# DecodeGenetics/Ratatosk

Measured on AMD Instinct MI355X. Metric: corrected long-read bases/sec, higher is better.
Workload: dtype u64

## Files before the change

### include/ratatosk_hip.h

```cpp
#ifndef RATATOSK_HIP_H
#define RATATOSK_HIP_H

#include <stdint.h>

#ifdef __cplusplus
extern "C" {
#endif

#define RTK_OK 0
#define RTK_ERR_IO (-1)
#define RTK_ERR_FORMAT (-2)
#define RTK_ERR_ARG (-3)
#define RTK_ERR_NO_DEVICE (-4)
#define RTK_ERR_DEVICE (-5)
#define RTK_ERR_UNSUPPORTED (-6)

typedef struct rtk_graph rtk_graph;
typedef struct rtk_batch rtk_batch;

typedef struct rtk_opts {
    uint64_t insert_sz;
    uint64_t min_cov_vertices;
    uint64_t max_len_weak_region1;
    uint64_t max_km_cov;
    double weak_region_len_factor;
    double large_k_factor;
    double min_score;
    int32_t max_qual;
    int32_t out_qual;
    double min_confidence_snp_corr;
    int32_t long_read_correct;
    int32_t force_unres_snp_corr;
    uint64_t max_len_weak_region2;
    int32_t a2_exclusive;
    int32_t a3_strand_order;
    int32_t d1_desc;
    uint32_t struct_size;
} rtk_opts;

typedef struct rtk_graph_info {
    uint64_t n_unitigs, n_kmers, n_bases, n_colour_ids, n_global_sets;
    uint64_t table_slots, hbm_bytes;
    uint64_t max_km_cov_top;
    int32_t k, device;
} rtk_graph_info;

typedef struct rtk_stats {
    double ms_total, ms_lookup_exact, ms_mask, ms_lookup_inexact, ms_seeds, ms_regions, ms_correct, ms_stitch;
    uint64_t n_windows, n_probes_exact, n_probes_inexact, n_hits_inexact, n_regions, n_region_items, n_arena_overflow;
    uint64_t n_expand, n_colour_elem, n_path_base, n_align, n_align_cells;
    uint64_t in_bases, out_bases;
    uint64_t cyc_colour, cyc_paths, cyc_consensus, cyc_total, cyc_myers, cyc_sets , cyc_tostring, cyc_pathqual;
    uint64_t n_slots_exact, n_slots_inexact;
    uint64_t cyc_walk, n_moves;
    double ms_lanes;
    uint64_t n_lane_regions, n_lane_handed;
    double ms_phase;
    uint64_t n_phase_skipped;
    uint64_t n_trim_stored, n_trim_column, n_trim_fallback, n_consensus_resumed, n_consensus_swept;
    uint64_t n_fa_linked_run, n_fa_linked_skipped, n_fa_linked_entries;
    uint64_t n_strand2_run, n_strand2_skipped, n_strand2_audit_mismatch;
    uint64_t n_park_walked, n_park_deferred;
    uint64_t n_colours_small, n_colours_wide, n_colours_bits, n_colours_general, n_colours_audit_mismatch;
    uint64_t n_colours_declined_fit;
} rtk_stats;

int rtk_graph_load(const char* unitig_fasta_gz, const char* rtsk, int k, int n_threads, rtk_graph** out);
#define RTK_LOAD_DEVICE_TABLES 1u
int rtk_graph_load2(const char* unitig_fasta_gz, const char* rtsk, int k, int n_threads, uint32_t flags, rtk_graph** out);

int rtk_graph_upload(rtk_graph* g, int device);

int rtk_graph_shell(int k, rtk_graph** out);
int rtk_graph_n_buffers(const rtk_graph* g);
int rtk_graph_buffer(rtk_graph* g, int idx, void** dev_ptr, uint64_t* bytes);
int rtk_graph_alloc_buffers(rtk_graph* g, int device, const uint64_t* bytes, int n, const rtk_graph_info* info);
int rtk_graph_adopt_device(rtk_graph* g);
int rtk_graph_attach_buffers(rtk_graph* g, int device, void* const* dev_ptrs, const uint64_t* bytes, int n, const rtk_graph_info* info);
int rtk_graph_buffer_bytes(const rtk_graph* g, uint64_t* bytes, int n);
int rtk_graph_move_buffer(rtk_graph* g, int idx, void* dev_ptr, uint64_t bytes);
int rtk_graph_host_buffer(const rtk_graph* g, int idx, const void** p, uint64_t* bytes);
int rtk_graph_download_buffer(const rtk_graph* g, int idx, void* host_dst, uint64_t bytes);

int rtk_n_devices(void);
int rtk_device_memory(int device, uint64_t* free_bytes, uint64_t* total_bytes);
int rtk_graph_clone_to_device(const rtk_graph* src, int device, rtk_graph** out);

int rtk_graph_get_info(const rtk_graph* g, rtk_graph_info* info);
void rtk_graph_free(rtk_graph* g);
long long rtk_graph_strip_annotations(rtk_graph* g);

int rtk_reserve_scratch(int device, uint32_t max_read_len);
int rtk_reserve_second_pass(int device, uint32_t n_tickets, uint64_t phase_bytes, uint64_t region_bytes);
int rtk_graph_reserve_batches(rtk_graph* g, uint32_t n_batches, uint64_t bases_per_batch, uint32_t reads_per_batch, int with_qualities, uint64_t raw_bases_per_batch);

int rtk_opts_default(const rtk_graph* g, rtk_opts* opts);

int rtk_correct_batch(rtk_graph* g, const rtk_opts* opts, uint32_t n, const char* const* seq, const char* const* qual,
                      const uint32_t* len, char** out_seq, char** out_qual, uint32_t* out_len);
int rtk_coalesce_stats(rtk_graph* g, uint64_t* n_groups, uint64_t* n_tickets);

int rtk_batch_create(rtk_graph* g, uint32_t n, const char* const* seq, const char* const* qual, const uint32_t* len, rtk_batch** out);
int rtk_batch_create2(rtk_graph* g, uint32_t n, const char* const* seq, const char* const* qual, const uint32_t* len,
                      const char* const* raw, const uint32_t* raw_len, rtk_batch** out);
int rtk_batch_run(rtk_batch* b, const rtk_opts* opts);
int rtk_batch_run_seeds(rtk_batch* b, const rtk_opts* opts);
int rtk_batch_run_regions(rtk_batch* b, const rtk_opts* opts);
int rtk_batch_fetch(rtk_batch* b, char** out_seq, char** out_qual, uint32_t* out_len);
int rtk_batch_fetch_view(rtk_batch* b, const char** pool, const uint64_t** off, const uint32_t** len);
int rtk_batch_get_stats(const rtk_batch* b, rtk_stats* stats);
void rtk_batch_free(rtk_batch* b);


int rtk_lookup_exact(rtk_graph* g, const char* seq, uint32_t len, int64_t* hits);

int rtk_fix_snps(rtk_graph* g, const char* seq, uint32_t len, char* out);

int rtk_seeds(rtk_graph* g, const rtk_opts* opts, const char* seq, uint32_t len,
              uint64_t* n_solid, int64_t* solid, uint64_t* n_weak, int64_t* weak, uint64_t cap);

int rtk_batch_fetch_seeds(rtk_batch* b, uint32_t read, uint64_t* n_solid, int64_t* solid, uint64_t* n_weak, int64_t* weak, uint64_t cap);

int rtk_myers_batch(uint32_t n, const char* const* query, const uint32_t* qlen, const char* const* target, const uint32_t* tlen,
                    const int32_t* k, const int32_t* mode, int want_path, int use_iupac,
                    int32_t* dist, int32_t* n_loc, int32_t* end_locs, uint32_t cap_locs, char* cigar, uint32_t cap_cigar);

int rtk_myers_batch_waves(uint32_t n, const char* const* query, const uint32_t* qlen, const char* const* target, const uint32_t* tlen,
                          const int32_t* k, const int32_t* mode, int want_path, int use_iupac,
                          int32_t* dist, int32_t* n_loc, int32_t* end_locs, uint32_t cap_locs, char* cigar, uint32_t cap_cigar, int waves);

#define RTK_MYERS_MODE_SHW_BY_COLUMN 3
#define RTK_MYERS_MODE_NW_PREFIX 4
#define RTK_MYERS_MODE_NW_PREFIX_LAST 5
void rtk_myers_column_last_routes(uint64_t* column_route, uint64_t* fallback);

int rtk_myers_batch_lanes(uint32_t n, const char* const* query, const uint32_t* qlen, const char* const* target, const uint32_t* tlen,
                          const int32_t* k, const int32_t* mode, int want_path, int use_iupac,
                          int32_t* dist, int32_t* n_loc, int32_t* end_locs, uint32_t cap_locs, char* cigar, uint32_t cap_cigar);
void rtk_myers_lanes_last_routes(uint64_t* lane_route, uint64_t* wave_route);

int rtk_index_count_kmers(int device, int k, const char* const* files, int n_files, uint32_t min_count, int n_threads, uint64_t** solid, uint64_t* n_solid);
int rtk_index_unitigs(int device, int k, const uint64_t* solid, uint64_t n_solid, char** seq_pool, uint64_t** seq_off, uint64_t** seeds, uint64_t* n_unitigs,
                      uint64_t** left, uint64_t* n_left);

int rtk_index_colour_begin(int device, int k, const char* seq_pool, const uint64_t* seq_off, uint64_t n_unitigs, void** job);
int rtk_index_colour_chunk(void* job, const char* chars, uint64_t n_chars, const uint64_t* starts, const uint32_t* ids, uint32_t n_reads);
int rtk_index_colour_end(void* job, uint64_t** events, uint64_t* n_events, uint64_t** cov);
int rtk_index_colour_chunk_q(void* job, const char* chars, const unsigned char* quals, unsigned char q_min, uint64_t n_chars, const uint64_t* starts, const uint32_t* ids,
                             uint32_t n_reads);
int rtk_index_colour_cov(void* job, uint64_t** cov);
int rtk_index_colour_end_subsampled(void* job, const uint8_t* bin_of_unitig, const uint8_t* forced_candidate, const uint8_t* bin_is_sampled, uint32_t n_bins, uint32_t mcv,
                                    double rate, uint64_t seed, uint64_t** events, uint64_t* n_events, uint64_t* n_events_before, uint64_t* n_ids_before, uint64_t* n_ids_after);
int rtk_index_subsample_events(int device, const uint64_t* events, uint64_t n_events, uint32_t n_unitigs, const uint8_t* bin_of_unitig, const uint8_t* forced_candidate,
                               const uint8_t* bin_is_sampled, uint32_t n_bins, uint32_t mcv, double rate, uint64_t seed, uint64_t* events_out, uint64_t* n_out,
                               uint64_t* n_ids_before, uint64_t* n_ids_after);
int rtk_index_colour_merge(void* job, uint64_t* n_events_before, uint64_t* n_events_after, uint64_t* n_ids_before, uint64_t* n_ids_after);
int rtk_index_colour_merge_classes(void* job, uint64_t* classes_above_one, uint64_t* largest);
int rtk_index_merge_events(int device, const uint64_t* events, uint64_t n_events, uint32_t n_unitigs, uint64_t* events_out, uint64_t* n_out, uint64_t* n_ids_before,
                           uint64_t* n_ids_after);

#define RTK_SNP_FIRST_PER_SITE 1u
int rtk_index_snp_candidates(int device, int k, const char* seq_pool, const uint64_t* seq_off, uint64_t n_unitigs, const uint8_t* searched, uint32_t flags,
                             uint64_t** cand, uint64_t* n_cand);
int rtk_index_snp_plan(int device, int k, const uint64_t* seq_off, uint64_t n_unitigs, const uint8_t* searched, uint64_t room, uint32_t* passes,
                       uint64_t* need_one_pass, uint64_t* need_min);

int rtk_index_cover_begin(int device, int k, const char* seq_pool, const uint64_t* seq_off, uint64_t n_unitigs, const uint8_t* low_bits, void** job);
int rtk_index_cover_chunk(void* job, const char* chars, uint64_t n_chars, const uint64_t* starts, const uint32_t* seq_numbers, const uint64_t* first_positions, uint32_t n_seqs);
int rtk_index_cover_end(void* job, uint64_t** crossings, uint64_t* n);

int rtk_rescue_begin(int device, int k, const uint64_t* lr, uint64_t n_lr, const uint64_t* sr, uint64_t n_sr, uint32_t min_positions, void** job);
int rtk_rescue_chunk(void* job, const char* chars, uint64_t n_chars, const uint64_t* starts, uint32_t n_reads, unsigned char* keep);
int rtk_rescue_end(void* job, uint64_t* n_positions_probed, uint64_t* n_hits);

#define RTK_SETS_UNION 0
#define RTK_SETS_INTER 1
#define RTK_SETS_DIFF 2
#define RTK_SETS_INTER_COUNT 3
#define RTK_SETS_SORT_PAIRS 4
#define RTK_SETS_RADIX_U32 5
#define RTK_SETS_RADIX_PAIRS_U32 6
#define RTK_SETS_BM_LOWEST 7
#define RTK_SETS_BM8_LOWEST 8
#define RTK_SETS_RADIX_TAGGED 9
#define RTK_SETS_COLOUR_UNIVERSE 10
#define RTK_SETS_OK 0
// ... 18 lines not shown
```

### ratatosk_amd/api.py

```python
import ctypes as C
import os

_HERE = os.path.dirname(os.path.abspath(__file__))
LIB_PATH = os.environ.get("RTK_LIB_OVERRIDE") or os.path.join(_HERE, "libratatosk_hip.so")


class RtkError(RuntimeError):
    pass


class RtkOpts(C.Structure):
    _fields_ = [("insert_sz", C.c_uint64), ("min_cov_vertices", C.c_uint64), ("max_len_weak_region1", C.c_uint64),
                ("max_km_cov", C.c_uint64), ("weak_region_len_factor", C.c_double), ("large_k_factor", C.c_double),
                ("min_score", C.c_double), ("max_qual", C.c_int32), ("out_qual", C.c_int32), ("min_confidence_snp_corr", C.c_double),
                ("long_read_correct", C.c_int32), ("force_unres_snp_corr", C.c_int32), ("max_len_weak_region2", C.c_uint64),
                ("a2_exclusive", C.c_int32), ("a3_strand_order", C.c_int32), ("d1_desc", C.c_int32), ("struct_size", C.c_uint32)]


class RtkGraphInfo(C.Structure):
    _fields_ = [("n_unitigs", C.c_uint64), ("n_kmers", C.c_uint64), ("n_bases", C.c_uint64), ("n_colour_ids", C.c_uint64),
                ("n_global_sets", C.c_uint64), ("table_slots", C.c_uint64), ("hbm_bytes", C.c_uint64), ("max_km_cov_top", C.c_uint64),
                ("k", C.c_int32), ("device", C.c_int32)]


class RtkStats(C.Structure):
    _fields_ = [(n, C.c_double) for n in ("ms_total", "ms_lookup_exact", "ms_mask", "ms_lookup_inexact", "ms_seeds", "ms_regions", "ms_correct", "ms_stitch")] + \
               [(n, C.c_uint64) for n in ("n_windows", "n_probes_exact", "n_probes_inexact", "n_hits_inexact", "n_regions", "n_region_items", "n_arena_overflow",
                                         "n_expand", "n_colour_elem", "n_path_base", "n_align", "n_align_cells", "in_bases", "out_bases",
                                         "cyc_colour", "cyc_paths", "cyc_consensus", "cyc_total", "cyc_myers", "cyc_sets", "cyc_tostring", "cyc_pathqual", "n_slots_exact", "n_slots_inexact", "cyc_walk", "n_moves")] + \
               [("ms_lanes", C.c_double), ("n_lane_regions", C.c_uint64), ("n_lane_handed", C.c_uint64), ("ms_phase", C.c_double), ("n_phase_skipped", C.c_uint64)] + \
               [(n, C.c_uint64) for n in ("n_trim_stored", "n_trim_column", "n_trim_fallback", "n_consensus_resumed", "n_consensus_swept",
                                         "n_fa_linked_run", "n_fa_linked_skipped", "n_fa_linked_entries",
                                         "n_strand2_run", "n_strand2_skipped", "n_strand2_audit_mismatch",
                                         "n_park_walked", "n_park_deferred",
                                         "n_colours_small", "n_colours_wide", "n_colours_bits", "n_colours_general", "n_colours_audit_mismatch", "n_colours_declined_fit")]

    def as_dict(self):
        return {n: getattr(self, n) for n, _ in self._fields_}


_libs = {}


os.environ.setdefault("GPU_MAX_HW_QUEUES", "16")


def load_library(path=None):
    path = path or LIB_PATH
    if path in _libs:
        return _libs[path]
    if not os.path.exists(path):
        raise RtkError("%s is missing: build it with `python -c 'import __graft_entry__ as g; g.build()'` (make -C ratatosk_amd/csrc)" % path)
    L = C.CDLL(path)
    L.rtk_last_error.restype = C.c_char_p
    L.rtk_version.restype = C.c_char_p
    L.rtk_graph_load.argtypes = [C.c_char_p, C.c_char_p, C.c_int, C.c_int, C.POINTER(C.c_void_p)]
    L.rtk_graph_load2.argtypes = [C.c_char_p, C.c_char_p, C.c_int, C.c_int, C.c_uint32, C.POINTER(C.c_void_p)]
    L.rtk_graph_move_buffer.argtypes = [C.c_void_p, C.c_int, C.c_void_p, C.c_uint64]
    L.rtk_graph_host_buffer.argtypes = [C.c_void_p, C.c_int, C.POINTER(C.c_void_p), C.POINTER(C.c_uint64)]
    L.rtk_graph_download_buffer.argtypes = [C.c_void_p, C.c_int, C.c_void_p, C.c_uint64]
    L.rtk_graph_upload.argtypes = [C.c_void_p, C.c_int]
    L.rtk_graph_shell.argtypes = [C.c_int, C.POINTER(C.c_void_p)]
    L.rtk_graph_n_buffers.argtypes = [C.c_void_p]
    L.rtk_graph_buffer.argtypes = [C.c_void_p, C.c_int, C.POINTER(C.c_void_p), C.POINTER(C.c_uint64)]
    L.rtk_graph_alloc_buffers.argtypes = [C.c_void_p, C.c_int, C.POINTER(C.c_uint64), C.c_int, C.POINTER(RtkGraphInfo)]
    L.rtk_graph_adopt_device.argtypes = [C.c_void_p]
    L.rtk_graph_buffer_bytes.argtypes = [C.c_void_p, C.POINTER(C.c_uint64), C.c_int]
    L.rtk_graph_get_info.argtypes = [C.c_void_p, C.POINTER(RtkGraphInfo)]
    L.rtk_graph_free.argtypes = [C.c_void_p]
    L.rtk_opts_default.argtypes = [C.c_void_p, C.POINTER(RtkOpts)]
    L.rtk_correct_batch.argtypes = [C.c_void_p, C.POINTER(RtkOpts), C.c_uint32, C.POINTER(C.c_char_p), C.POINTER(C.c_char_p), C.POINTER(C.c_uint32),
                                    C.POINTER(C.c_void_p), C.POINTER(C.c_void_p), C.POINTER(C.c_uint32)]
    L.rtk_batch_create.argtypes = [C.c_void_p, C.c_uint32, C.POINTER(C.c_char_p), C.POINTER(C.c_char_p), C.POINTER(C.c_uint32), C.POINTER(C.c_void_p)]
    L.rtk_batch_create2.argtypes = [C.c_void_p, C.c_uint32, C.POINTER(C.c_char_p), C.POINTER(C.c_char_p), C.POINTER(C.c_uint32),
                                    C.POINTER(C.c_char_p), C.POINTER(C.c_uint32), C.POINTER(C.c_void_p)]
    L.rtk_batch_run.argtypes = [C.c_void_p, C.POINTER(RtkOpts)]
    L.rtk_graph_strip_annotations.restype = C.c_longlong
    L.rtk_graph_strip_annotations.argtypes = [C.c_void_p]
    L.rtk_batch_run_seeds.argtypes = [C.c_void_p, C.POINTER(RtkOpts)]
    L.rtk_batch_run_regions.argtypes = [C.c_void_p, C.POINTER(RtkOpts)]
    L.rtk_batch_fetch.argtypes = [C.c_void_p, C.POINTER(C.c_void_p), C.POINTER(C.c_void_p), C.POINTER(C.c_uint32)]
    L.rtk_batch_fetch_view.argtypes = [C.c_void_p, C.POINTER(C.c_char_p), C.POINTER(C.POINTER(C.c_uint64)), C.POINTER(C.POINTER(C.c_uint32))]
    L.rtk_n_devices.restype = C.c_int
    L.rtk_device_memory.argtypes = [C.c_int, C.POINTER(C.c_uint64), C.POINTER(C.c_uint64)]
    L.rtk_graph_clone_to_device.argtypes = [C.c_void_p, C.c_int, C.POINTER(C.c_void_p)]
    L.rtk_batch_get_stats.argtypes = [C.c_void_p, C.POINTER(RtkStats)]
    L.rtk_batch_free.argtypes = [C.c_void_p]
    L.rtk_lookup_exact.argtypes = [C.c_void_p, C.c_char_p, C.c_uint32, C.POINTER(C.c_int64)]
# ... 234 lines not shown
            c = cig.raw[i * cap_cig:(i + 1) * cap_cig].split(b"\0", 1)[0].decode()
        out.append((dist[i], el, c))
    return out


def _u64_array(a):
    if hasattr(a, "ctypes"):
        import numpy as np
        arr = np.ascontiguousarray(a, dtype=np.uint64)
        return arr, arr.ctypes.data_as(C.POINTER(C.c_uint64)), int(arr.size)
    arr = (C.c_uint64 * max(1, len(a)))(*[int(x) for x in a])
    return arr, arr, len(a)


def rescue_reads(lr_kmers, sr_kmers, seqs, k=31, min_positions=31, device=0, stats=None, lib_path=None):
    L = load_library(lib_path)
    if L.rtk_api_revision() < 9:
        raise RtkError("%s is of interface revision %d: the rescue entries came with revision 9" % (L._name, L.rtk_api_revision()))
    keep_lr, p_lr, n_lr = _u64_array(lr_kmers)
    keep_sr, p_sr, n_sr = _u64_array(sr_kmers)
    job = C.c_void_p()

    def check(rc):
        if rc != 0:
            raise RtkError("rtk error %d: %s" % (rc, L.rtk_last_error().decode()))

    check(L.rtk_rescue_begin(device, k, p_lr, n_lr, p_sr, n_sr, min_positions, C.byref(job)))
    out = []
    try:
        bs = [_b(s) for s in seqs]
        i = 0
        while i < len(bs):
            j, size = i, 0
            while j < len(bs) and (j == i or (size + len(bs[j]) + 1 <= (48 << 20) and j - i < (2 << 20))):
                size += len(bs[j]) + 1; j += 1
            starts, at = (C.c_uint64 * (j - i))(), 0
            for r in range(i, j):
                starts[r - i] = at; at += len(bs[r]) + 1
            chars = b"\n".join(bs[i:j]) + b"\n"
            keep = (C.c_ubyte * (j - i))()
            check(L.rtk_rescue_chunk(job, chars, len(chars), starts, j - i, keep))
            out.extend(bool(x) for x in keep)
            i = j
    except Exception:
        L.rtk_rescue_end(job, None, None)
        raise
    probed, hits = C.c_uint64(), C.c_uint64()
    check(L.rtk_rescue_end(job, C.byref(probed), C.byref(hits)))
    if stats is not None:
        stats["n_positions_probed"], stats["n_hits"] = probed.value, hits.value
    return out


MODE_SHW_BY_COLUMN, MODE_NW_PREFIX, MODE_NW_PREFIX_LAST = 3, 4, 5


def myers_column_last_routes(lib_path=None):
    L = load_library(lib_path)
    a, b = C.c_uint64(), C.c_uint64()
    L.rtk_myers_column_last_routes.argtypes = [C.POINTER(C.c_uint64), C.POINTER(C.c_uint64)]; L.rtk_myers_column_last_routes.restype = None
    L.rtk_myers_column_last_routes(C.byref(a), C.byref(b))
    return a.value, b.value


def myers_lanes_last_routes(lib_path=None):
    L = load_library(lib_path)
    a, b = C.c_uint64(), C.c_uint64()
    L.rtk_myers_lanes_last_routes.argtypes = [C.POINTER(C.c_uint64), C.POINTER(C.c_uint64)]; L.rtk_myers_lanes_last_routes.restype = None
    L.rtk_myers_lanes_last_routes(C.byref(a), C.byref(b))
    return a.value, b.value


SETS_UNION, SETS_INTER, SETS_DIFF, SETS_INTER_COUNT, SETS_SORT_PAIRS, SETS_RADIX_U32, SETS_RADIX_PAIRS_U32, SETS_BM_LOWEST, SETS_BM8_LOWEST, SETS_RADIX_TAGGED, SETS_COLOUR_UNIVERSE = range(11)
SETS_OK, SETS_NOT_IN_BUILD, SETS_DECLINED = 0, 1, 2


def sets_batch(problems, lib_path=None):
    import numpy as np
    L = load_library(lib_path)
    if L.rtk_api_revision() < 10:
        raise RtkError("%s is of interface revision %d: rtk_sets_batch came with revision 10" % (L._name, L.rtk_api_revision()))
    n = len(problems)
    keep, off = [], [0]
    ops = (C.c_uint32 * max(1, n))(); na = (C.c_uint32 * max(1, n))(); nb = (C.c_uint32 * max(1, n))(); sc = (C.c_uint32 * max(1, n))()
    pa = (C.POINTER(C.c_uint32) * max(1, n))(); pb = (C.POINTER(C.c_uint32) * max(1, n))()
    for i, (op, a, b, scalar) in enumerate(problems):
        if op == SETS_SORT_PAIRS:
            a = np.ascontiguousarray(a, dtype="<u8"); b = np.ascontiguousarray(b, dtype="<u8")
            count_a, count_b, a, b = int(a.size), int(b.size), a.view("<u4"), b.view("<u4")
        else:
            a = np.ascontiguousarray(a, dtype=np.uint32); b = np.ascontiguousarray(b, dtype=np.uint32)
            count_a, count_b = int(a.size), int(b.size)
        keep.append((a, b))
        ops[i], na[i], nb[i], sc[i] = op, count_a, count_b, scalar
        pa[i] = a.ctypes.data_as(C.POINTER(C.c_uint32)); pb[i] = b.ctypes.data_as(C.POINTER(C.c_uint32))
        need = {SETS_UNION: count_a + count_b, SETS_INTER: count_a, SETS_DIFF: count_a, SETS_INTER_COUNT: 0, SETS_SORT_PAIRS: 4 * count_a, SETS_RADIX_U32: count_a,
                SETS_RADIX_PAIRS_U32: 2 * count_a, SETS_BM_LOWEST: min(scalar, count_b), SETS_BM8_LOWEST: min(scalar, count_b),
                SETS_RADIX_TAGGED: 2 * count_a, SETS_COLOUR_UNIVERSE: 2 + count_a + 2 * count_b * max(1, (count_a + 63) // 64)}.get(op, 0)
        off.append(off[-1] + need)
    out = np.zeros(max(1, off[-1]), dtype=np.uint32)
    offs = (C.c_uint64 * (n + 1))(*off)
    out_n = (C.c_uint32 * max(1, n))(); res = (C.c_uint32 * max(1, n))(); st = (C.c_uint32 * max(1, n))()
    rc = L.rtk_sets_batch(n, ops, pa, na, pb, nb, sc, out.ctypes.data_as(C.POINTER(C.c_uint32)), offs, out_n, res, st)
    if rc != 0:
        raise RtkError("rtk error %d: %s" % (rc, L.rtk_last_error().decode()))
    ret = []
    for i, (op, _, _, _) in enumerate(problems):
# ... 250 lines not shown
```

### ratatosk_amd/csrc/hip/rtk_device.hip

```cpp
#include <algorithm>
#include <atomic>
#include <chrono>
#include <cmath>
#include <cstdio>
#include <cstring>
#include <map>
#include <memory>
#include <condition_variable>
#include <mutex>
#include <string>
#include <thread>
#include <vector>

#include "../../../include/ratatosk_hip.h"
#include "../host/flat_graph.hpp"
#include "rtk_graph_tables.h"
#include "rtk_mem.h"
#include "rtk_myers.h"
#include "rtk_myers_lane.h"
#include "rtk_types.h"
#include "rtk_wave.h"

#ifdef RTK_SIM
thread_local int rtk_sim_block_id = 0;
// ... 404 lines not shown
            if (rtk_lane() == 0) hitmap[tile] = bal;
#endif
        }
    }
    if (n_probes_out) {
        const int tot = rtk_wave_sum(static_cast<int>(probes)), tots = rtk_wave_sum(static_cast<int>(slots));
        if (rtk_lane() == 0) { if (tot) rtk_atomic_add(reinterpret_cast<unsigned long long*>(n_probes_out), static_cast<unsigned long long>(tot)); if (tots) rtk_atomic_add(reinterpret_cast<unsigned long long*>(n_probes_out) + 11, static_cast<unsigned long long>(tots)); }
    }
}

static int default_grid() {
#ifdef RTK_SIM
    return 64;
#else
    return 256 * 16;
#endif
}

extern "C" int rtk_lookup_exact(rtk_graph* g, const char* seq, uint32_t len, int64_t* hits) {
    if (!g || !seq || !hits) return rtk_fail(RTK_ERR_ARG, "rtk_lookup_exact: null argument");
    if (!g->on_device) return rtk_fail(RTK_ERR_NO_DEVICE, "rtk_lookup_exact: graph is not resident on a device (call rtk_graph_upload)");
    try {
        rtk_set_device(g->device);
        std::string up(seq, len);
        for (size_t i = 0; i < up.size(); ++i) up[i] = static_cast<char>(toupper(static_cast<unsigned char>(up[i])));
        char* dseq = static_cast<char*>(rtk_dmalloc(len + 64));
        uint64_t* droff = static_cast<uint64_t*>(rtk_dmalloc(16));
        uint64_t* dhits = static_cast<uint64_t*>(rtk_dmalloc(8ull * (len + 1)));
        const uint64_t roff[2] = {0, len};
        rtk_h2d(dseq, up.data(), len); rtk_h2d(droff, roff, 16);
        rtk_launch(k_lookup_exact, default_grid(), 0, g->dview, static_cast<const char*>(dseq), static_cast<const uint64_t*>(droff), 1u, static_cast<uint64_t>(len), default_grid(), dhits, static_cast<uint64_t*>(nullptr), static_cast<uint64_t*>(nullptr));
        rtk_dsync();
        std::vector<uint64_t> h(len + 1);
        rtk_d2h(h.data(), dhits, 8ull * len);
        const uint32_t nw = len >= static_cast<uint32_t>(g->info.k) ? len - g->info.k + 1 : 0;
        for (uint32_t i = 0; i < nw; ++i) hits[i] = (h[i] == RTK_NO_HIT) ? -1 : static_cast<int64_t>(h[i]);
        rtk_dfree(dseq); rtk_dfree(droff); rtk_dfree(dhits);
    } catch (const std::exception& e) { return rtk_fail(RTK_ERR_DEVICE, e.what()); }
    return RTK_OK;
}

RTK_FN void rtk_myers_column_item(const MyersScratch& sc, const MyersProb& p, uint32_t i, const char* q, const char* t, int use_iupac, int32_t* dist, int32_t* n_loc, int32_t* end_locs,
                                  uint32_t cap_locs, uint8_t* moves_out, uint32_t* n_moves_out, uint32_t cap_moves, uint32_t* status) {
    const int m = static_cast<int>(p.qlen), n = static_cast<int>(p.tlen); const bool iupac = use_iupac != 0;
    uint32_t route = 2, nm = 0;
    MyersResult r;
    if (p.mode == RTK_MYERS_MODE_SHW_BY_COLUMN) {
        if (rtk_myers_shw_by_column(sc, t, n, q, m, iupac, 0, 0, &r, nullptr)) route = 1;
        else r = rtk_myers_distance(sc, q, m, t, n, -1, RTK_MODE_SHW, iupac);
        if (cap_locs > 0) end_locs[static_cast<uint64_t>(i) * cap_locs] = r.first;
        if (r.nloc > 1 && static_cast<uint32_t>(r.nloc) <= cap_locs) end_locs[static_cast<uint64_t>(i) * cap_locs + (r.nloc - 1)] = r.last;
        n_loc[i] = r.nloc;
    } else {
        const int k = p.k; const bool last_only = p.mode == RTK_MYERS_MODE_NW_PREFIX_LAST;
        int at = 0, last = -1;
        if (k > 0 && rtk_myers_shw_by_column(sc, q, m, t, n, iupac, 1, k, &r, &at)) {
            const long long W = (k + 63) >> 6;
            if (static_cast<uint32_t>(k) <= sc.r_cap && static_cast<uint32_t>(k + n) <= sc.mv_cap && (2LL * 8 + 4) * W * n + 8LL * n < 1024 * 1024) {
                if (last_only) last = rtk_myers_last_move(sc, k, n, n, at);
                else rtk_myers_walk(sc, k, n, n, at, &nm);
                r.dist = at; route = 1;
            }
        }
        if (route != 1) {
            if (k > 0 && n > 0) r = rtk_myers_path(sc, q, k, t, n, RTK_MODE_NW, iupac, &nm);
            else r = rtk_myers_distance(sc, q, k, t, n, -1, RTK_MODE_NW, iupac);
            if (last_only) { rtk_sync(); last = nm ? static_cast<int>(rtk_ld(sc.moves.get() + (nm - 1u))) : -1; nm = 0; }
        }
        if (cap_locs > 0) end_locs[static_cast<uint64_t>(i) * cap_locs] = last_only ? last : n - 1;
        n_loc[i] = 1;
    }
    dist[i] = r.dist;
    if (nm <= cap_moves) rtk_wcopy(moves_out + static_cast<uint64_t>(i) * cap_moves, sc.moves, nm);
    n_moves_out[i] = nm;
    status[i] = *sc.overflow | (route << 16);
}

RTK_FN void rtk_myers_batch_item(const MyersScratch& sc, const MyersProb& p, uint32_t i, const char* pool, int want_path, int use_iupac, int32_t* dist, int32_t* n_loc, int32_t* end_locs, uint32_t cap_locs,
                                 uint8_t* moves_out, uint32_t* n_moves_out, uint32_t cap_moves, uint32_t* status) {
    *sc.overflow = 0;
    const char* q = pool + p.q_off; const char* t = pool + p.t_off;
    if (p.mode >= RTK_MYERS_MODE_SHW_BY_COLUMN) { rtk_myers_column_item(sc, p, i, q, t, use_iupac, dist, n_loc, end_locs, cap_locs, moves_out, n_moves_out, cap_moves, status); return; }
    const MyersResult r = rtk_myers_distance(sc, q, static_cast<int>(p.qlen), t, static_cast<int>(p.tlen), p.k, p.mode, use_iupac != 0, cap_locs ? end_locs + static_cast<uint64_t>(i) * cap_locs : nullptr, static_cast<int>(cap_locs));
    dist[i] = r.dist; n_loc[i] = r.nloc;
    uint32_t nm = 0;
    if (want_path && r.dist >= 0 && p.qlen > 0 && p.tlen > 0) {
        if (p.k < 0 && p.mode != RTK_MODE_HW) {
            const MyersResult r2 = rtk_myers_path(sc, q, static_cast<int>(p.qlen), t, static_cast<int>(p.tlen), p.mode, use_iupac != 0, &nm);
            if (r2.dist != r.dist || r2.first != r.first) *sc.overflow = 3;
        } else
        rtk_myers_alignment(sc, q, static_cast<int>(p.qlen), t, r.first + 1, r.dist, use_iupac != 0, &nm);
        if (nm <= cap_moves) rtk_wcopy(moves_out + static_cast<uint64_t>(i) * cap_moves, sc.moves, nm);
    }
    n_moves_out[i] = nm;
    status[i] = *sc.overflow;
}

RTK_GLOBAL void k_myers_batch(const MyersProb* probs, uint32_t n, const char* pool, int want_path, int use_iupac, char* scratch, uint64_t scratch_stride, ScratchCfg cfg,
                              int grid, int32_t* dist, int32_t* n_loc, int32_t* end_locs, uint32_t cap_locs, uint8_t* moves_out, uint32_t* n_moves_out, uint32_t cap_moves, uint32_t* status, unsigned long long* prof) {
#ifdef RTK_SIM
    const MyersScratch sc = scratch_carve(scratch + static_cast<uint64_t>(RTK_BLOCK_ID) * scratch_stride, cfg);
#else
    __shared__ MyersScratch sc;
    sc = scratch_carve(scratch + static_cast<uint64_t>(RTK_BLOCK_ID) * scratch_stride, cfg);
    __syncthreads();
#endif
    for (uint32_t i = static_cast<uint32_t>(RTK_BLOCK_ID); i < n; i += static_cast<uint32_t>(grid))
        rtk_myers_batch_item(sc, probs[i], i, pool, want_path, use_iupac, dist, n_loc, end_locs, cap_locs, moves_out, n_moves_out, cap_moves, status);
    if (prof && rtk_lane() == 0) { rtk_atomic_add(prof + 0, sc.hb_total.get()); rtk_atomic_add(prof + 1, sc.hb_pass.get()); rtk_atomic_add(prof + 2, sc.hb_split.get()); rtk_atomic_add(prof + 3, sc.hb_leaf.get()); rtk_atomic_add(prof + 4, sc.walk_cycles.get()); }
}

#ifndef RTK_SIM
void rtk_launch_myers_batch_waves(int grid, int waves, const MyersProb* probs, uint32_t n, const char* pool, int want_path, int use_iupac, char* scratch, uint64_t scratch_stride, const ScratchCfg& cfg,
                                  int32_t* dist, int32_t* n_loc, int32_t* end_locs, uint32_t cap_locs, uint8_t* moves_out, uint32_t* n_moves_out, uint32_t cap_moves, uint32_t* status, unsigned long long* prof);
#endif
static thread_local uint64_t g_col_routes[2] = {0, 0};
extern "C" void rtk_myers_column_last_routes(uint64_t* column_route, uint64_t* fallback) { if (column_route) *column_route = g_col_routes[0]; if (fallback) *fallback = g_col_routes[1]; }
extern "C" int rtk_myers_batch(uint32_t n, const char* const* query, const uint32_t* qlen, const char* const* target, const uint32_t* tlen,
                               const int32_t* k, const int32_t* mode, int want_path, int use_iupac,
                               int32_t* dist, int32_t* n_loc, int32_t* end_locs, uint32_t cap_locs, char* cigar, uint32_t cap_cigar) {
    return rtk_myers_batch_waves(n, query, qlen, target, tlen, k, mode, want_path, use_iupac, dist, n_loc, end_locs, cap_locs, cigar, cap_cigar, 1);
}
extern "C" int rtk_myers_batch_waves(uint32_t n, const char* const* query, const uint32_t* qlen, const char* const* target, const uint32_t* tlen,
                                     const int32_t* k, const int32_t* mode, int want_path, int use_iupac,
                                     int32_t* dist, int32_t* n_loc, int32_t* end_locs, uint32_t cap_locs, char* cigar, uint32_t cap_cigar, int waves) {
    if (waves > 16) return rtk_fail(RTK_ERR_ARG, "rtk_myers_batch_waves: at most 16 waves per workgroup");
    if (!query || !qlen || !target || !tlen || !k || !mode || !dist || !n_loc || (!end_locs && cap_locs)) return rtk_fail(RTK_ERR_ARG, "rtk_myers_batch: null argument");
    if (rtk_device_count() <= 0) return rtk_fail(RTK_ERR_NO_DEVICE, "rtk_myers_batch: no HIP device visible (no CPU fallback)");
    if (n == 0) return RTK_OK;
    try {
        std::vector<MyersProb> probs(n);
        std::string pool;
        uint32_t max_q = 1, max_t = 1;
        for (uint32_t i = 0; i < n; ++i) {
            probs[i].q_off = pool.size(); pool.append(query[i], qlen[i]);
            probs[i].t_off = pool.size(); pool.append(target[i], tlen[i]);
            probs[i].qlen = qlen[i]; probs[i].tlen = tlen[i]; probs[i].k = k[i]; probs[i].mode = mode[i];
            if (mode[i] == RTK_MODE_HW && want_path) return rtk_fail(RTK_ERR_UNSUPPORTED, "rtk_myers_batch: HW path alignment is not on the hot path");
            if (mode[i] < 0 || mode[i] > RTK_MYERS_MODE_NW_PREFIX_LAST || (mode[i] > RTK_MODE_HW && waves > 1)) return rtk_fail(RTK_ERR_ARG, "rtk_myers_batch: unknown mode (the test-only modes 3 to 5 run on one wave)");
            if ((mode[i] == RTK_MYERS_MODE_SHW_BY_COLUMN && k[i] >= 0) || (mode[i] >= RTK_MYERS_MODE_NW_PREFIX && (k[i] < 0 || static_cast<uint32_t>(k[i]) > qlen[i])))
                return rtk_fail(RTK_ERR_ARG, "rtk_myers_batch: mode 3 takes k < 0, modes 4 and 5 a query row 0 <= k <= qlen");
            max_q = std::max(max_q, qlen[i]); max_t = std::max(max_t, tlen[i]);
        }
        for (uint32_t i = 0; i < n; ++i) if (mode[i] > RTK_MODE_HW) { max_q = max_t = std::max(max_q, max_t); break; }
        ScratchCfg cfg;
        cfg.w_cap = (max_q + 63) / 64 + 1; cfg.t_cap = max_t + 64; cfg.r_cap = max_q + 64; cfg.mv_cap = max_q + max_t + 64;
        cfg.tb_cap_words = std::max<uint64_t>(4ull * 52429 + 64, 4ull * cfg.w_cap + 64);
        const int grid = static_cast<int>(std::min<uint32_t>(n, static_cast<uint32_t>(default_grid() / 4 > 0 ? default_grid() / 4 : 1)));
        const uint64_t stride = scratch_bytes(cfg) + (waves > 1 ? static_cast<uint64_t>((waves < RTK_LEAF_WAVES ? waves : RTK_LEAF_WAVES) - 1) * scratch_bytes(rtk_leaf_cfg()) : 0ull);
        const uint32_t cap_moves = want_path ? (max_q + max_t + 8) : 1;
        struct Held { std::vector<void*> v; void* get(uint64_t bytes) { v.push_back(nullptr); v.back() = rtk_dmalloc(bytes); return v.back(); } void release() { for (void* p : v) if (p) rtk_dfree(p); v.clear(); } ~Held() { release(); } } held;
        char* dpool = static_cast<char*>(held.get(pool.size() + 64));
        MyersProb* dprobs = static_cast<MyersProb*>(held.get(sizeof(MyersProb) * n));
        char* dscr = static_cast<char*>(held.get(stride * grid));
        int32_t* ddist = static_cast<int32_t*>(held.get(4ull * n)); int32_t* dnloc = static_cast<int32_t*>(held.get(4ull * n));
        int32_t* dlocs = static_cast<int32_t*>(held.get(4ull * n * cap_locs + 8)); uint32_t* dst = static_cast<uint32_t*>(held.get(4ull * n));
        uint8_t* dmoves = static_cast<uint8_t*>(held.get(static_cast<uint64_t>(n) * cap_moves + 8)); uint32_t* dnm = static_cast<uint32_t*>(held.get(4ull * n));
        rtk_h2d(dpool, pool.data(), pool.size()); rtk_h2d(dprobs, probs.data(), sizeof(MyersProb) * n);
        unsigned long long* dprof = nullptr;
        if (rtk_knob_myers_prof()) { dprof = static_cast<unsigned long long*>(rtk_dmalloc(64)); const unsigned long long z[8] = {0, 0, 0, 0, 0, 0, 0, 0}; rtk_h2d(dprof, z, 64); }
#ifndef RTK_SIM
        if (waves > 1) rtk_launch_myers_batch_waves(grid, waves, static_cast<const MyersProb*>(dprobs), n, static_cast<const char*>(dpool), want_path, use_iupac, dscr, stride, cfg, ddist, dnloc, dlocs, cap_locs, dmoves, dnm, cap_moves, dst, dprof);
        else
#endif
        { RtkTimer tk; const bool timed = rtk_knob_myers_time() && waves <= 1; if (timed) tk.start(0);
          rtk_launch(k_myers_batch, grid, 0, static_cast<const MyersProb*>(dprobs), n, static_cast<const char*>(dpool), want_path, use_iupac, dscr, stride, cfg, grid, ddist, dnloc, dlocs, cap_locs, dmoves, dnm, cap_moves, dst, dprof);
          if (timed) { tk.stop(0); rtk_dsync(); fprintf(stderr, "[rtk myers time] one wave per problem: %u problems, %d waves, kernel %.3f ms\n", n, grid, tk.elapsed()); } }
        if (dprof) { rtk_dsync(); unsigned long long pc[8]; rtk_d2h(pc, dprof, 64); rtk_dfree(dprof);
            fprintf(stderr, "[rtk myers prof] waves %d: Hirschberg driver %.3g cycles (half passes %.3g, columns + split %.3g, leaf tracebacks %.3g of which walks %.3g)\n", waves, double(pc[0]), double(pc[1]), double(pc[2]), double(pc[3]), double(pc[4])); }
        rtk_dsync();
        std::vector<uint32_t> st(n), nm(n);
        rtk_d2h(dist, ddist, 4ull * n); rtk_d2h(n_loc, dnloc, 4ull * n); if (cap_locs) rtk_d2h(end_locs, dlocs, 4ull * n * cap_locs);
        rtk_d2h(st.data(), dst, 4ull * n); rtk_d2h(nm.data(), dnm, 4ull * n);
        int rc = RTK_OK;
        g_col_routes[0] = 0; g_col_routes[1] = 0;
        for (uint32_t i = 0; i < n; ++i) {
            if (st[i] & 0xFFFFu) rc = rtk_fail(RTK_ERR_DEVICE, "rtk_myers_batch: scratch capacity exceeded on device");
            if (mode[i] > RTK_MODE_HW) ++g_col_routes[(st[i] >> 16) == 1u ? 0 : 1];
        }
        if (want_path && cigar && rc == RTK_OK) {
            std::vector<uint8_t> mv(static_cast<size_t>(n) * cap_moves);
            rtk_d2h(mv.data(), dmoves, mv.size());
            static const char code[4] = {'M', 'I', 'D', 'M'};
            for (uint32_t i = 0; i < n; ++i) {
                std::string c;
                const uint8_t* a = &mv[static_cast<size_t>(i) * cap_moves];
                for (uint32_t x = 0; x < nm[i];) { uint32_t y = x; while (y < nm[i] && code[a[y]] == code[a[x]]) ++y; c += std::to_string(y - x); c.push_back(code[a[x]]); x = y; }
                if (c.size() + 1 > cap_cigar) { rc = rtk_fail(RTK_ERR_ARG, "rtk_myers_batch: cigar buffer too small"); break; }
                memcpy(cigar + static_cast<size_t>(i) * cap_cigar, c.c_str(), c.size() + 1);
            }
        }
        held.release();
        return rc;
    } catch (const std::exception& e) { return rtk_fail(RTK_ERR_DEVICE, e.what()); }
// ... 278 lines not shown
```

### ratatosk_amd/csrc/hip/rtk_knobs.h

```cpp
#ifndef RTK_KNOBS_H
#define RTK_KNOBS_H

#include <stdint.h>
#include <stdlib.h>
#include <string.h>
#include <algorithm>

inline bool rtk_env_set(const char* name) { return getenv(name) != nullptr; }
inline bool rtk_env_is1(const char* name) { const char* e = getenv(name); return e && e[0] == '1'; }
inline int rtk_env_int(const char* name, int dflt) { const char* e = getenv(name); return e ? atoi(e) : dflt; }
inline int rtk_env_pos_int(const char* name, int dflt) { const int v = rtk_env_int(name, 0); return v > 0 ? v : dflt; }
inline uint64_t rtk_env_u64(const char* name, uint64_t dflt) { const char* e = getenv(name); return e ? strtoull(e, nullptr, 10) : dflt; }
inline bool rtk_env_eq(const char* name, const char* value) { const char* e = getenv(name); return e && !strcmp(e, value); }

inline bool rtk_knob_trace() { return rtk_env_set("RTK_TRACE"); }
inline int rtk_knob_trace_class(int dflt) { return rtk_env_int("RTK_TRACE_CLASS", dflt); }
inline bool rtk_knob_lane_cost() { return rtk_env_set("RTK_LANE_COST"); }
inline bool rtk_knob_myers_prof() { return rtk_env_set("RTK_MYERS_PROF"); }
inline bool rtk_knob_myers_time() { return rtk_env_set("RTK_MYERS_TIME"); }
inline bool rtk_knob_index_trace() { return rtk_env_set("RTK_INDEX_TRACE"); }
inline bool rtk_knob_load_trace() { return rtk_env_set("RTK_LOAD_TRACE"); }

inline uint32_t rtk_knob_mask_seg() { return static_cast<uint32_t>(rtk_env_u64("RTK_MASK_SEG", 8192)); }
inline int rtk_knob_seed_waves() { return rtk_env_pos_int("RTK_SEED_WAVES", 4096); }
inline bool rtk_knob_inexact_enum() { return rtk_env_is1("RTK_INEXACT_ENUM"); }
inline bool rtk_knob_test_tiny_scratch() { return rtk_env_set("RTK_TEST_TINY_SCRATCH"); }
inline int rtk_knob_a2_exclusive() { return rtk_env_eq("RTK_A2_XOR", "union") ? 0 : (rtk_env_eq("RTK_A2_XOR", "exclusive-ids") ? 2 : 1); }
inline int rtk_knob_a3_strand_order() { return rtk_env_eq("RTK_A3_ORDER", "strand") ? 1 : 0; }
inline int rtk_knob_d1_desc() { return rtk_env_eq("RTK_D1_ORDER", "desc") ? 1 : 0; }

inline bool rtk_knob_phase_align_all() { return rtk_env_is1("RTK_PHASE_ALIGN_ALL"); }
inline uint32_t rtk_knob_phase_long() { return static_cast<uint32_t>(rtk_env_u64("RTK_PHASE_LONG", 24576)); }
inline int rtk_knob_phase_lwaves() { return std::max(1, std::min(16, rtk_env_int("RTK_PHASE_LWAVES", 4))); }
inline int rtk_knob_phase_pgrid() { return rtk_env_int("RTK_PHASE_PGRID", 1024); }
inline int rtk_knob_phase_lgrid() { return rtk_env_int("RTK_PHASE_LGRID", 192); }
inline int rtk_knob_phase_mgrid() { return rtk_env_int("RTK_PHASE_MGRID", 768); }

inline bool rtk_knob_lane_max_gap_set() { return rtk_env_set("RTK_LANE_MAX_GAP"); }
inline uint32_t rtk_knob_lane_max_gap() { return static_cast<uint32_t>(rtk_env_u64("RTK_LANE_MAX_GAP", 0)); }
inline int rtk_knob_lane_waves() { return rtk_env_pos_int("RTK_LANE_WAVES", 1024); }
inline bool rtk_knob_lane_serial() { return rtk_env_is1("RTK_LANE_SERIAL"); }
inline int rtk_knob_lane_round() { return rtk_env_int("RTK_LANE_ROUND", 64); }
inline bool rtk_knob_compact() { return rtk_env_is1("RTK_COMPACT"); }
inline int rtk_knob_region_waves() { return rtk_env_pos_int("RTK_REGION_WAVES", 4096); }
inline int rtk_knob_p2_rgrid() { return rtk_env_int("RTK_P2_RGRID", 512); }
inline bool rtk_knob_fa_linked_always() { return rtk_env_is1("RTK_FA_LINKED_ALWAYS"); }
inline bool rtk_knob_strand2_always() { return rtk_env_is1("RTK_STRAND2_ALWAYS"); }
inline bool rtk_knob_strand2_audit() { return rtk_env_is1("RTK_STRAND2_AUDIT"); }
inline uint32_t rtk_knob_colours_route() { return rtk_env_eq("RTK_COLOURS_ROUTE", "bits") ? 1u : (rtk_env_eq("RTK_COLOURS_ROUTE", "general") ? 2u : 0u); }
inline uint32_t rtk_knob_colours_audit() { return rtk_env_is1("RTK_COLOURS_AUDIT") ? (rtk_env_is1("RTK_TEST_COLOURS_FAULT") ? 3u : 1u) : 0u; }
inline bool rtk_knob_park_eager() { return rtk_env_is1("RTK_PARK_EAGER"); }
inline bool rtk_knob_test_coalesce_fail() { return rtk_env_set("RTK_TEST_COALESCE_FAIL"); }

inline uint64_t rtk_knob_lane_auto_bases() { static const uint64_t v = rtk_env_u64("RTK_LANE_AUTO_BASES", 512ull << 20); return v; }
inline uint64_t rtk_knob_half_slab_bases() { static const uint64_t v = rtk_env_u64("RTK_HALF_SLAB_BASES", 8ull << 20); return v; }
inline int rtk_knob_half_waves() { static const int v = std::min(rtk_env_pos_int("RTK_HALF_WAVES", 2048), 2048); return v; }
inline uint64_t rtk_knob_coalesce_bases() { static const uint64_t v = rtk_env_u64("RTK_COALESCE_BASES", 16ull << 20); return v; }
inline long rtk_knob_coalesce_wait_us() { static const long v = [] { const char* e = getenv("RTK_COALESCE_WAIT_US"); return e ? atol(e) : 1500L; }(); return v; }
inline uint32_t rtk_knob_coalesce_split() { static const uint32_t v = static_cast<uint32_t>(rtk_env_pos_int("RTK_COALESCE_SPLIT", 2)); return v; }

inline uint64_t rtk_knob_index_cap(uint64_t dflt) { return rtk_env_u64("RTK_INDEX_CAP", dflt); }
inline uint64_t rtk_knob_index_chunk(uint64_t dflt) { const uint64_t v = rtk_env_u64("RTK_INDEX_CHUNK", 0); return v >= 1024 ? v : dflt; }
inline int rtk_knob_index_keep_text() { return rtk_env_int("RTK_INDEX_KEEP_TEXT", -1); }
inline uint64_t rtk_knob_index_events(uint64_t dflt) { return rtk_env_u64("RTK_INDEX_EVENTS", dflt); }
inline uint64_t rtk_knob_index_cover_cap(uint64_t dflt) { return rtk_env_u64("RTK_INDEX_COVER_CAP", dflt); }
inline uint64_t rtk_knob_index_snp_mem(uint64_t dflt) { return std::min(dflt, rtk_env_u64("RTK_INDEX_SNP_MEM", dflt)); }
inline uint32_t rtk_knob_index_snp_passes() { return static_cast<uint32_t>(std::min<uint64_t>(rtk_env_u64("RTK_INDEX_SNP_PASSES", 0), 0xFFFFFFFFull)); }
inline uint64_t rtk_knob_hx_part_keys(uint64_t dflt) { return rtk_env_u64("RTK_HX_PART_KEYS", dflt); }

inline int rtk_knob_sim_devices() { return std::max(1, rtk_env_int("RTK_SIM_DEVICES", 1)); }


#endif
```

### ratatosk_amd/csrc/hip/rtk_myers.h

```cpp
#ifndef RTK_MYERS_H
#define RTK_MYERS_H

#include "rtk_wave.h"

#define RTK_MODE_NW 0
#define RTK_MODE_SHW 1
#define RTK_MODE_HW 2

struct MyersScratch {
    U<uint64_t*> peq;
    U<uint32_t> w_cap;
    U<int8_t*> carry;
    U<int32_t*> colscore;
    U<uint32_t> t_cap;
    U<uint64_t*> tb;
    U<uint64_t> tb_cap_words;
    U<int32_t*> rowL;
    U<int32_t*> rowR;
    U<uint32_t> r_cap;
    U<uint8_t*> moves;
    U<uint8_t*> moves_tmp;
    U<uint32_t> mv_cap;
    U<int32_t*> hstack;
    UL<uint32_t*> overflow;
// ... 178 lines not shown
}
#endif

#ifndef RTK_SIM
struct SweepStat { int final_score, best, first, last, cnt; bool plain; int at_score; };
__device__ __forceinline__ void rtk_last_column_stat(uint64_t pv, uint64_t mv, int B, int m, int n, int at, SweepStat& st) {
    const int lane = rtk_lane();
    const int row0 = B * lane;
    int rows = m - row0; rows = rows < 0 ? 0 : (rows > B ? B : rows);
    const uint64_t mask = rows >= 64 ? ~0ull : ((1ull << rows) - 1ull);
    pv &= mask; mv &= mask;
    int total;
    int v = n + rtk_wave_excl_scan(rtk_popc(pv) - rtk_popc(mv), &total);
    int best = 0x7fffffff, first = -1, last = -1, cnt = 0, atv = 0;
    for (int b = 0; b < rows; ++b) {
        v += static_cast<int>((pv >> b) & 1ull) - static_cast<int>((mv >> b) & 1ull);
        const bool lt = v < best, eq = v == best;
        best = lt ? v : best; first = lt ? row0 + b : first; last = (lt || eq) ? row0 + b : last; cnt = lt ? 1 : (cnt + (eq ? 1 : 0));
        atv = (row0 + b + 1 == at) ? v : atv;
    }
    int gb = best;
    for (int o = 32; o > 0; o >>= 1) { const int x = __shfl_xor(gb, o, 64); gb = x < gb ? x : gb; }
    const uint64_t has = rtk_ballot(cnt > 0 && best == gb);
    st.best = gb; st.first = __shfl(first, rtk_ffs(has) - 1, 64); st.last = __shfl(last, 63 - __builtin_clzll(has), 64);
    st.cnt = rtk_wave_sum((cnt > 0 && best == gb) ? cnt : 0);
    st.at_score = (at <= 0) ? n : __shfl(atv, (at - 1) / B, 64);
}
template <int STORE, int COLUMN = 0>
__device__ __forceinline__ SweepStat rtk_myers_fast(const char* __restrict__ qp, int m, const char* __restrict__ tp, int n, int top_h, bool iupac, uint64_t* __restrict__ tb, int at = 0) {
    SweepStat st; st.final_score = m; st.best = 0x7fffffff; st.first = -1; st.last = -1; st.cnt = 0; st.plain = true; st.at_score = 0;
    const int lane = rtk_lane();
    const int W = (m + 63) >> 6, last_bit = (m - 1) & 63;
    const int w = lane;
    const bool has_word = lane < W;
    uint64_t eqA = 0, eqC = 0, eqG = 0, eqT = 0;
    if (has_word) {
        const int lim = (m - 64 * w) < 64 ? (m - 64 * w) : 64;
        uint64_t qw[8];
        for (int j = 0; j < 8; ++j) { uint64_t x = 0; if (8 * j < lim) __builtin_memcpy(&x, qp + 64 * w + 8 * j, 8); qw[j] = x; }
        for (int i = 0; i < lim; ++i) {
            const unsigned char qc = static_cast<unsigned char>((qw[i >> 3] >> (8 * (i & 7))) & 0xFFull);
            uint32_t bm;
            if (qc == 'A') bm = 1u; else if (qc == 'C') bm = 2u; else if (qc == 'G') bm = 4u; else if (qc == 'T') bm = 8u;
            else bm = rtk_eq_classes(rtk_cls(qc), iupac) & 0xFu;
            eqA |= static_cast<uint64_t>(bm & 1u) << i; eqC |= static_cast<uint64_t>((bm >> 1) & 1u) << i;
            eqG |= static_cast<uint64_t>((bm >> 2) & 1u) << i; eqT |= static_cast<uint64_t>((bm >> 3) & 1u) << i;
        }
    }
    const int bit = (w == W - 1) ? last_bit : 63;
    uint64_t Pv = ~0ull, Mv = 0ull;
    int hout_prev = 0; unsigned tc_prev = 0;
    int score = m;
    int best = 0x7fffffff, first = -1, last = -1, cnt = 0, fin = m;
    const int steps = n + W - 1;
    for (int c0 = 0; c0 < steps; c0 += 64) {
        const int cj = c0 + lane;
        int my_t = 'A';
        if (cj < n) my_t = static_cast<int>(static_cast<unsigned char>(tp[cj]));
        if (rtk_ballot(!(my_t == 'A' || my_t == 'C' || my_t == 'G' || my_t == 'T')) != 0ull) { st.plain = false; return st; }
        asm volatile("" : "+v"(my_t));
        const int lim = (steps - c0) < 64 ? (steps - c0) : 64;
        for (int j = 0; j < lim; ++j) {
            const int s = c0 + j;
            const unsigned in_t = static_cast<unsigned>(__builtin_amdgcn_readlane(my_t, j));
            const unsigned mine = static_cast<unsigned>(hout_prev + 1) | (tc_prev << 8);
            const unsigned got = static_cast<unsigned>(__builtin_amdgcn_update_dpp(static_cast<int>(static_cast<unsigned>(top_h + 1) | (in_t << 8)), static_cast<int>(mine), 0x138, 0xF, 0xF, false));
            const int hin = static_cast<int>(got & 0xFFu) - 1;
            const unsigned tc = got >> 8;
            const unsigned sel = (tc >> 1) & 3u;
            const uint64_t Eq = (sel & 2u) ? ((sel & 1u) ? eqG : eqT) : ((sel & 1u) ? eqC : eqA);
            uint64_t nPv = Pv, nMv = Mv, Ph, Mh;
            const int hout = rtk_myers_step(nPv, nMv, Eq, hin, bit, Ph, Mh);
            const int col = s - lane;
            const bool active = has_word && col >= 0 && col < n;
            if (STORE) { if (active) { rtk_tb_put(tb + 4ull * RTK_TB(col, w, n), nPv, nMv, Ph, Mh); } }
            Pv = active ? nPv : Pv; Mv = active ? nMv : Mv;
            hout_prev = active ? hout : hout_prev;
            score += (active && lane == W - 1) ? hout : 0;
            tc_prev = tc;
            const int tcol = s - (W - 1);
            if (!COLUMN && tcol >= 0) {
                const int sv = __builtin_amdgcn_readlane(score, W - 1);
                fin = sv;
                if (sv < best) { best = sv; first = tcol; last = tcol; cnt = 1; }
                else if (sv == best) { last = tcol; ++cnt; }
            }
        }
    }
    if (COLUMN) { rtk_last_column_stat(has_word ? Pv : 0ull, has_word ? Mv : 0ull, 64, m, n, at, st); return st; }
    st.final_score = fin; st.best = best; st.first = first; st.last = last; st.cnt = cnt;
    return st;
}
#endif
#ifndef RTK_SIM
RTK_DEV int rtk_myers_step32(uint32_t& Pv, uint32_t& Mv, uint32_t Eq, int hin, int bit, uint32_t& Ph_out, uint32_t& Mh_out) {
    const uint32_t pv = Pv, mv = Mv;
    const uint32_t Xv = Eq | mv;
    Eq |= static_cast<uint32_t>(hin) >> 31;
    const uint32_t Xh = (((Eq & pv) + pv) ^ pv) | Eq;
    uint32_t Ph = mv | ~(Xh | pv);
    uint32_t Mh = pv & Xh;
    Ph_out = Ph; Mh_out = Mh;
    const int hout = static_cast<int>((Ph >> bit) & 1u) - static_cast<int>((Mh >> bit) & 1u);
    Ph = (Ph << 1) | (hin > 0 ? 1u : 0u); Mh = (Mh << 1) | (static_cast<uint32_t>(hin) >> 31);
    Pv = Mh | ~(Xv | Ph);
    Mv = Ph & Xv;
    return hout;
}

template <int STORE, int TRACK>
__device__ __forceinline__ SweepStat rtk_myers_fast32(const char* __restrict__ qp, int m, const char* __restrict__ tp, int n, int top_h, bool iupac, uint64_t* __restrict__ tb, int at = 0) {
    SweepStat st; st.final_score = m; st.best = 0x7fffffff; st.first = -1; st.last = -1; st.cnt = 0; st.plain = true; st.at_score = 0;
    const int lane = rtk_lane();
    const int W = (m + 31) >> 5, W64 = (m + 63) >> 6, last_bit = (m - 1) & 31;
    const int w = lane;
    const bool has_word = lane < W;
    uint32_t eqA = 0, eqC = 0, eqG = 0, eqT = 0;
    if (has_word) {
        const int lim = (m - 32 * w) < 32 ? (m - 32 * w) : 32;
        uint64_t qw[4];
        for (int j = 0; j < 4; ++j) { uint64_t x = 0; if (8 * j < lim) __builtin_memcpy(&x, qp + 32 * w + 8 * j, 8); qw[j] = x; }
        uint32_t p1 = 0, p2 = 0, done = 0;
        for (int j = 0; j < 8; ++j) {
            if (4 * j >= lim) break;
            const uint32_t x = static_cast<uint32_t>(qw[j >> 1] >> (32 * (j & 1)));
            const uint32_t b1 = (x >> 1) & 0x01010101u, b2 = (x >> 2) & 0x01010101u;
            const uint32_t b12 = b1 & b2, b2n = b2 & ~b1;
            const uint32_t recon = 0x41414141u + (b1 << 1) + (b12 << 2) + (b2n << 4) + (b2n << 1) + b2n;
            if (x != recon || 4 * j + 4 > lim) continue;
            const uint32_t n1 = (b1 & 1u) | ((b1 >> 7) & 2u) | ((b1 >> 14) & 4u) | ((b1 >> 21) & 8u);
            const uint32_t n2 = (b2 & 1u) | ((b2 >> 7) & 2u) | ((b2 >> 14) & 4u) | ((b2 >> 21) & 8u);
            p1 |= n1 << (4 * j); p2 |= n2 << (4 * j); done |= 0xFu << (4 * j);
        }
        eqA = ~p1 & ~p2 & done; eqC = p1 & ~p2 & done; eqT = ~p1 & p2 & done; eqG = p1 & p2 & done;
        if (done != ((lim >= 32) ? ~0u : ((1u << lim) - 1u))) {
            for (int i = 0; i < lim; ++i) {
                if ((done >> i) & 1u) continue;
                const unsigned char qc = static_cast<unsigned char>((qw[i >> 3] >> (8 * (i & 7))) & 0xFFull);
                uint32_t bm;
                if (qc == 'A') bm = 1u; else if (qc == 'C') bm = 2u; else if (qc == 'G') bm = 4u; else if (qc == 'T') bm = 8u;
                else bm = rtk_eq_classes(rtk_cls(qc), iupac) & 0xFu;
                eqA |= (bm & 1u) << i; eqC |= ((bm >> 1) & 1u) << i; eqG |= ((bm >> 2) & 1u) << i; eqT |= ((bm >> 3) & 1u) << i;
            }
        }
    }
    const int bit = (w == W - 1) ? last_bit : 31;
    uint32_t Pv = ~0u, Mv = 0u;
    int hout_prev = 0; uint32_t m1_prev = 0, m2_prev = 0;
    int score = m;
    int vbest = 0x7fffffff, vfirst = -1, vlast = -1, vcnt = 0;
    const int steps = n + W - 1;
    RtkTbHalf* const tbh = reinterpret_cast<RtkTbHalf*>(tb) + 2ull * RTK_TB(0, w >> 1, n) + (w & 1);
#define RTK_STEP32(MASKED)                                                                                                                   \
    {                                                                                                                                        \
        const int s = c0 + j;                                                                                                                \
        const int in_t = __builtin_amdgcn_readlane(my_t, j);                                                                                 \
         \
         \
        const int hin = __builtin_amdgcn_update_dpp(top_h, hout_prev, 0x138, 0xF, 0xF, false);                                              \
        const uint32_t m1 = static_cast<uint32_t>(__builtin_amdgcn_update_dpp(__builtin_amdgcn_sbfe(in_t, 1, 1), static_cast<int>(m1_prev), 0x138, 0xF, 0xF, false)); \
        const uint32_t m2 = static_cast<uint32_t>(__builtin_amdgcn_update_dpp(__builtin_amdgcn_sbfe(in_t, 2, 1), static_cast<int>(m2_prev), 0x138, 0xF, 0xF, false)); \
        const uint32_t lo_ = (eqC & m1) | (eqA & ~m1), hi_ = (eqG & m1) | (eqT & ~m1);                                                       \
        const uint32_t Eq = (hi_ & m2) | (lo_ & ~m2);                                                                                        \
        uint32_t nPv = Pv, nMv = Mv, Ph, Mh;                                                                                                 \
        const int hout = rtk_myers_step32(nPv, nMv, Eq, hin, bit, Ph, Mh);                                                                   \
        const int col = s - lane;                                                                                                            \
        if (MASKED) {                                                                                                                        \
            const bool active = has_word && col >= 0 && col < n;                                                                             \
            if (STORE) { if (active) { RtkTbHalf hv; hv.pv = nPv; hv.mv = nMv; hv.ph = Ph; hv.mh = Mh; tbh[2ull * static_cast<uint64_t>(col)] = hv; } } \
            Pv = active ? nPv : Pv; Mv = active ? nMv : Mv;                                                                                  \
            hout_prev = active ? hout : hout_prev;                                                                                           \
            score += active ? hout : 0;                                                                                                      \
        } else {                                                                                                                             \
            if (STORE) { if (has_word) { RtkTbHalf hv; hv.pv = nPv; hv.mv = nMv; hv.ph = Ph; hv.mh = Mh; tbh[2ull * static_cast<uint64_t>(col)] = hv; } } \
            Pv = nPv; Mv = nMv; hout_prev = hout; score += hout;                                                                             \
        }                                                                                                                                    \
        m1_prev = m1; m2_prev = m2;                                                                                                          \
        if (TRACK == 1) {                                                                                                                    \
            const int tcol = s - (W - 1);                                                                                                    \
            if (!(MASKED) || tcol >= 0) {  \
                const bool lt_ = score < vbest, eq_ = score == vbest;                                                                        \
                vbest = lt_ ? score : vbest; vfirst = lt_ ? tcol : vfirst; vlast = (lt_ || eq_) ? tcol : vlast; vcnt = lt_ ? 1 : (vcnt + (eq_ ? 1 : 0)); \
            }                                                                                                                                \
        }                                                                                                                                    \
    }
    int nxt_t = 'A';
    if (lane < n) nxt_t = static_cast<int>(static_cast<unsigned char>(tp[lane]));
    for (int c0 = 0; c0 < steps; c0 += 64) {
        int my_t = nxt_t;
        { const int cn = c0 + 64 + lane; nxt_t = 'A'; if (cn < n) nxt_t = static_cast<int>(static_cast<unsigned char>(tp[cn])); }
        if (rtk_ballot(!(my_t == 'A' || my_t == 'C' || my_t == 'G' || my_t == 'T')) != 0ull) { st.plain = false; return st; }
        asm volatile("" : "+v"(my_t));
        const int lim = (steps - c0) < 64 ? (steps - c0) : 64;
        int j_fill = (W - 1) - c0; j_fill = j_fill < 0 ? 0 : (j_fill > lim ? lim : j_fill);
        int j_full = n - c0; j_full = j_full < j_fill ? j_fill : (j_full > lim ? lim : j_full);
        int j = 0;
        for (; j < j_fill; ++j) RTK_STEP32(1)
        for (; j < j_full; ++j) RTK_STEP32(0)
        for (; j < lim; ++j) RTK_STEP32(1)
    }
#undef RTK_STEP32
    st.final_score = __builtin_amdgcn_readlane(score, W - 1);
    if (TRACK == 2) rtk_last_column_stat(has_word ? Pv : 0u, has_word ? Mv : 0u, 32, m, n, at, st);
    if (TRACK == 1) { st.best = __builtin_amdgcn_readlane(vbest, W - 1); st.first = __builtin_amdgcn_readlane(vfirst, W - 1); st.last = __builtin_amdgcn_readlane(vlast, W - 1); st.cnt = __builtin_amdgcn_readlane(vcnt, W - 1); }
    return st;
}

template <int STORE, int TRACK>
__device__ __forceinline__ SweepStat rtk_myers_fast_any(const char* __restrict__ qp, int m, const char* __restrict__ tp, int n, int top_h, bool iupac, uint64_t* __restrict__ tb, int at = 0) {
    if (m <= 2048) return rtk_myers_fast32<STORE, TRACK>(qp, m, tp, n, top_h, iupac, tb, at);
    return rtk_myers_fast<STORE, TRACK == 2 ? 1 : 0>(qp, m, tp, n, top_h, iupac, tb, at);
}
#endif


#define RTK_BAND_FULL (1 << 29)
#define RTK_BAND_INF 0x3fffffff
#define RTK_RING_MAX_BAND 4000
struct RtkBand { int dlo, dhi; };
RTK_HD RtkBand rtk_band_full() { RtkBand b; b.dlo = -RTK_BAND_FULL; b.dhi = RTK_BAND_FULL; return b; }
RTK_HD RtkBand rtk_band_nw(int m, int n, int k) {
    const int d = n - m, ad = d < 0 ? -d : d;
    const int h = k > ad ? (k - ad) / 2 : 0;
    RtkBand b; b.dlo = (d < 0 ? d : 0) - h; b.dhi = (d > 0 ? d : 0) + h; return b;
}
RTK_HD bool rtk_band_is_full(const RtkBand& b, int m, int n) { return b.dlo <= -m && b.dhi >= n; }
RTK_HD int rtk_band_clo(int w, int dlo, int gran) { const long long c = 64LL * ((w / gran) * gran) + dlo; return c < 0 ? 0 : static_cast<int>(c); }
RTK_HD int rtk_band_chi(int w, int W, int n, int dhi, int gran) { int wl = (w / gran) * gran + gran - 1; if (wl > W - 1) wl = W - 1; const long long c = 64LL * wl + 63 + dhi; return c > n - 1 ? n - 1 : static_cast<int>(c); }
RTK_HD int rtk_band_words(int m, int n, int dlo) { const int W = (m + 63) >> 6; const long long r = static_cast<long long>(n) - 1 - dlo; if (r < 0) return 0; const long long w = (r >> 6) + 1; return w < W ? static_cast<int>(w) : W; }
RTK_HD int rtk_band_gran(int m, int dlo, int dhi) { return (((m + 63) >> 6) > 64 && (dhi - dlo) <= RTK_RING_MAX_BAND) ? 1 : 64; }
RTK_HD int rtk_band_guess(int m, int n) {
    const int d = n - m, ad = d < 0 ? -d : d, mn = m < n ? m : n;
    int g = ad + (mn / 8 > 64 ? mn / 8 : 64);
    if (g < RTK_RING_MAX_BAND - 100) g = RTK_RING_MAX_BAND - 100;
    return g < m + n ? g : m + n;
}

struct RtkGangCtx { const char* q; const char* t; char* stage; uint64_t* peq; uint64_t* fin; int32_t* nodes; int n_nodes, iupac; };
struct RtkCoopJob { const char* qp; const char* tp; int m, n, qrev, trev, top_h, iupac; uint64_t* fin_pv; uint64_t* fin_mv; int8_t* carry; int32_t* colscore; int dlo, dhi, ring; uint64_t* peq4; };
#ifndef RTK_SIM
__device__ __forceinline__ int rtk_coop_ld(const int* p) { return __builtin_amdgcn_readfirstlane(__hip_atomic_load(p, __ATOMIC_RELAXED, __HIP_MEMORY_SCOPE_WORKGROUP)); }
__device__ __forceinline__ void rtk_coop_st(int* p, int v) { if (rtk_lane() == 0) __hip_atomic_store(p, v, __ATOMIC_RELAXED, __HIP_MEMORY_SCOPE_WORKGROUP); }
__device__ __forceinline__ unsigned char rtk_job_qc(const char* __restrict__ qp, int m, int qrev, int i) { return static_cast<unsigned char>(qrev ? qp[m - 1 - i] : qp[i]); }
__device__ __forceinline__ void rtk_myers_eq4(const char* __restrict__ qp, int m, int qrev, int w, bool iupac, uint64_t& eqA, uint64_t& eqC, uint64_t& eqG, uint64_t& eqT) {
    eqA = 0; eqC = 0; eqG = 0; eqT = 0;
    const int lim = (m - 64 * w) < 64 ? (m - 64 * w) : 64;
    for (int i = 0; i < lim; ++i) {
        const unsigned char qc = rtk_job_qc(qp, m, qrev, 64 * w + i);
        uint32_t bm;
        if (qc == 'A') bm = 1u; else if (qc == 'C') bm = 2u; else if (qc == 'G') bm = 4u; else if (qc == 'T') bm = 8u;
        else bm = rtk_eq_classes(rtk_cls(qc), iupac) & 0xFu;
        eqA |= static_cast<uint64_t>(bm & 1u) << i; eqC |= static_cast<uint64_t>((bm >> 1) & 1u) << i;
        eqG |= static_cast<uint64_t>((bm >> 2) & 1u) << i; eqT |= static_cast<uint64_t>((bm >> 3) & 1u) << i;
    }
// ... 541 lines not shown
    rtk_myers_pass(sc, rtk_seq(q, m), rtk_seq(t, n), mode == RTK_MODE_HW ? 0 : 1, iupac, 0, nullptr, nullptr);
    if (mode == RTK_MODE_NW) {
        const int d = sc.colscore[n - 1];
        if (k >= 0 && d > k) return r;
        r.dist = d; r.first = r.last = n - 1; r.nloc = 1;
        if (locs_out && cap > 0) locs_out[0] = n - 1;
        return r;
    }
    int best = 0x7fffffff;
    for (int j = rtk_lane(); j < n; j += RTK_WAVE) { const int v = sc.colscore[j]; best = v < best ? v : best; }
#ifndef RTK_SIM
    for (int o = 32; o > 0; o >>= 1) { const int v = __shfl_xor(best, o, 64); best = v < best ? v : best; }
#endif
    const bool pseudo = (m & 63) != 0;
    if (pseudo && m < best) best = m;
    if (k >= 0 && best > k) return r;
    r.dist = best;
    int cnt = 0, first = 0x7fffffff, last = -2;
    if (pseudo && m == best) { cnt = 1; first = -1; last = -1; if (locs_out && cap > 0) locs_out[0] = -1; }
    for (int j0 = 0; j0 < n; j0 += RTK_WAVE) {
        const int j = j0 + rtk_lane();
        const bool hit = (j < n) && (sc.colscore[j] == best);
        const uint64_t b = rtk_ballot(hit);
        if (b) {
            const int lo = j0 + rtk_ffs(b) - 1;
            const int hi = j0 + 63 - __builtin_clzll(b);
            if (lo < first) first = lo;
            if (hi > last) last = hi;
            if (locs_out) {
                const int my = cnt + rtk_popc(b & ((1ull << rtk_lane()) - 1ull));
                if (hit && my < cap) locs_out[my] = j;
            }
            cnt += rtk_popc(b);
        }
    }
    rtk_sync();
    r.first = first; r.last = last; r.nloc = cnt;
    return r;
}

RTK_FN bool rtk_myers_shw_by_column(const MyersScratch& sc_, const char* corr_, int m_, const char* raw_, int n_, bool iupac_, int store_, int at_, MyersResult* out_, int* at_score_) {
    const MyersScratch& sc = *rtk_u(&sc_); RTK_ASSUME_LDS(&sc); const char* corr = rtk_u(corr_); const char* raw = rtk_u(raw_);
    const int m = rtk_u(m_), n = rtk_u(n_), store = rtk_u(store_), at = rtk_u(at_); const bool iupac = rtk_u(iupac_);
    MyersResult* out = rtk_u(out_); int* at_score = rtk_u(at_score_);
    const long long W = (m + 63) >> 6;
    if (m <= 0 || n <= 0 || m > 4096 || static_cast<uint32_t>((n + 63) >> 6) > sc.w_cap || static_cast<uint32_t>(m) > sc.t_cap) return false;
    if (static_cast<uint32_t>(W) > sc.w_cap || static_cast<uint32_t>(n) > sc.t_cap) return false;
    if (store && static_cast<uint64_t>(4 * W * n) > sc.tb_cap_words) return false;
    if (store) { MyersScratch& msc = const_cast<MyersScratch&>(sc); msc.tb_gen = rtk_ld(&msc.tb_gen) + 1u; }
    int best, first, last, cnt, atv;
#ifdef RTK_SIM
    for (int j = 0; j < n; ++j) { const char ch = raw[j]; if (!(ch == 'A' || ch == 'C' || ch == 'G' || ch == 'T')) return false; }
    uint64_t* fin = new uint64_t[2 * W];
    rtk_myers_pass(sc, rtk_seq(corr, m), rtk_seq(raw, n), 1, iupac, store, fin, fin + W);
    best = 0x7fffffff; first = -1; last = -1; cnt = 0; atv = n;
    for (int i = 0, v = n; i < m; ++i) {
        v += static_cast<int>((fin[i >> 6] >> (i & 63)) & 1ull) - static_cast<int>((fin[W + (i >> 6)] >> (i & 63)) & 1ull);
        if (v < best) { best = v; first = last = i; cnt = 1; } else if (v == best) { last = i; ++cnt; }
        if (i + 1 == at) atv = v;
    }
    delete[] fin;
#else
    const SweepStat st = store ? rtk_myers_fast_any<1, 2>(corr, m, raw, n, 1, iupac, rtk_ld(&sc.tb), at) : rtk_myers_fast_any<0, 2>(corr, m, raw, n, 1, iupac, nullptr, at);
    rtk_sync();
    if (!st.plain) return false;
    best = st.best; first = st.first; last = st.last; cnt = st.cnt; atv = st.at_score;
#endif
    MyersResult r; const int colbest = best; const bool pseudo = (n & 63) != 0;
    if (pseudo && n < best) best = n;
    r.dist = best;
    if (pseudo && n == best) { r.first = -1; r.last = (colbest == best) ? last : -1; r.nloc = 1 + ((colbest == best) ? cnt : 0); }
    else { r.first = first; r.last = last; r.nloc = cnt; }
    *out = r;
    if (at_score) *at_score = atv;
    return true;
}

RTK_FN void rtk_myers_walk(const MyersScratch& sc_, int m_, int n_, int ncols_, int cur_, uint32_t* n_moves_) {
    const MyersScratch& sc = *rtk_u(&sc_); RTK_ASSUME_LDS(&sc); uint32_t* n_moves = rtk_u(n_moves_);
    const int m = rtk_u(m_), n = rtk_u(n_), ncols = rtk_u(ncols_);
    int cur = rtk_u(cur_);
    const unsigned long long tw0 = rtk_clock(); unsigned n_rel = 0, n_sc = 0;
    int i = m, j = n;
    uint32_t nt = 0;
    uint8_t* tmp = rtk_ld(&sc.moves_tmp);
    const uint32_t cap = rtk_ld(&sc.mv_cap);
    uint64_t* const tbp = rtk_ld(&sc.tb);
#ifndef RTK_SIM
    const int lane = rtk_lane();
    int w_cur = -1, c_hi = -1;
    uint64_t e0 = 0, e1 = 0, e2 = 0, e3 = 0;
#define RTK_RL64(v, l) ((static_cast<uint64_t>(static_cast<uint32_t>(__builtin_amdgcn_readlane(static_cast<int>((v) >> 32), (l)))) << 32) | static_cast<uint32_t>(__builtin_amdgcn_readlane(static_cast<int>((v) & 0xFFFFFFFFull), (l))))
#endif
    while (i > 0 && j > 0) {
        const int r = i - 1, c = j - 1, w = r >> 6, b = r & 63;
#ifdef RTK_SIM
        uint64_t a0, a1, a2, a3; rtk_tb_get(tbp + 4ull * RTK_TB(c, w, ncols), a0, a1, a2, a3);
        uint64_t l0 = 0, l1 = 0;
        if (c > 0) { uint64_t l2, l3; rtk_tb_get(tbp + 4ull * RTK_TB(c - 1, w, ncols), l0, l1, l2, l3); }
#else
        if (w != w_cur || c > c_hi || c_hi - c > 62) {
            c_hi = c; w_cur = w; ++n_rel;
            const int col = c - lane;
            if (col >= 0) rtk_tb_get(tbp + 4ull * RTK_TB(col, w, ncols), e0, e1, e2, e3);
        }
        const int li = c_hi - c;
        {
            const uint64_t up = RTK_RL64(e0, li) & ~RTK_RL64(e1, li);
            if ((up >> b) & 1ull) {
                const uint64_t nup = ~(up << (63 - b));
                const int run = nup ? __builtin_clzll(nup) : 64;
                if (lane < run) tmp[cap - (nt + 1u + static_cast<uint32_t>(lane))] = 1;
                i -= run; cur -= run; nt += static_cast<uint32_t>(run);
                continue;
            }
        }
        {
            const int l = lane - li;
            const int vd_ = static_cast<int>((e0 >> b) & 1ull) - static_cast<int>((e1 >> b) & 1ull);
            const int hd_ = static_cast<int>((e2 >> b) & 1ull) - static_cast<int>((e3 >> b) & 1ull);
            const bool isleft = l >= 0 && (c - l) >= 0 && vd_ != 1 && hd_ == 1;
            const uint64_t nleft = ~(rtk_ballot(isleft) >> li);
            const int run = nleft ? __builtin_ctzll(nleft) : 64;
            if (run > 0) {
                if (l >= 0 && l < run) tmp[cap - (nt + 1u + static_cast<uint32_t>(l))] = 2;
                j -= run; cur -= run; nt += static_cast<uint32_t>(run);
// ... 12 lines not shown
            const bool isdiag = valid && vd_ != 1 && hd_ != 1;
            const uint64_t dm = rtk_ballot(isdiag) >> li;
            const uint64_t ndm = ~dm;
            const int run = ndm ? __builtin_ctzll(ndm) : 64;
            if (run > 0) {
                const bool mine = l >= 0 && l < run;
                const bool mism = (hd_ + vdl) != 0;
                const uint64_t mm = rtk_ballot(mine && mism);
                if (mine) tmp[cap - (nt + 1u + static_cast<uint32_t>(l))] = mism ? 3 : 0;
                cur -= rtk_popc(mm); i -= run; j -= run; nt += static_cast<uint32_t>(run);
                continue;
            }
        }
        ++n_sc;
        const uint64_t a0 = RTK_RL64(e0, li), a1 = RTK_RL64(e1, li), a2 = RTK_RL64(e2, li), a3 = RTK_RL64(e3, li);
        const uint64_t l0 = RTK_RL64(e0, li + 1), l1 = RTK_RL64(e1, li + 1);
#endif
        const int vd = static_cast<int>((a0 >> b) & 1ull) - static_cast<int>((a1 >> b) & 1ull);
        const int hd = static_cast<int>((a2 >> b) & 1ull) - static_cast<int>((a3 >> b) & 1ull);
        uint8_t mv;
        if (vd == 1) { mv = 1; --i; cur -= 1; }
        else if (hd == 1) { mv = 2; --j; cur -= 1; }
        else {
            const int left = cur - hd;
            int diag;
            if (c == 0) diag = i - 1;
            else diag = left - (static_cast<int>((l0 >> b) & 1ull) - static_cast<int>((l1 >> b) & 1ull));
            mv = (diag == cur) ? 0 : 3;
            --i; --j; cur = diag;
        }
        ++nt; tmp[cap - nt] = mv;
    }
    const unsigned long long tw1 = rtk_clock();
    if (i > 0) { rtk_wfill(tmp + (cap - nt - static_cast<uint32_t>(i)), 1, static_cast<uint64_t>(i)); nt += static_cast<uint32_t>(i); i = 0; }
    if (j > 0) { rtk_wfill(tmp + (cap - nt - static_cast<uint32_t>(j)), 2, static_cast<uint64_t>(j)); nt += static_cast<uint32_t>(j); j = 0; }
    rtk_sync();
    rtk_wcopy(rtk_ld(&sc.moves) + *n_moves, tmp + (cap - nt), nt);
    *n_moves += nt;
    { MyersScratch& msc = const_cast<MyersScratch&>(sc); msc.walk_cycles += rtk_clock() - tw0; msc.walk_moves += nt; msc.walk_reloads += n_rel; msc.walk_scalar += n_sc; msc.walk_calls += 1; msc.walk_tail_cycles += rtk_clock() - tw1; }
}

RTK_DEV uint8_t rtk_myers_last_move(const MyersScratch& sc_, int m_, int n_, int ncols_, int cur_) {
    const MyersScratch& sc = *rtk_u(&sc_); RTK_ASSUME_LDS(&sc);
    const int m = rtk_u(m_), n = rtk_u(n_), ncols = rtk_u(ncols_), cur = rtk_u(cur_);
    const uint64_t* const tbp = rtk_ld(&sc.tb);
    const int r = m - 1, c = n - 1, w = r >> 6, b = r & 63;
    uint64_t a0, a1, a2, a3; rtk_tb_get(tbp + 4ull * RTK_TB(c, w, ncols), a0, a1, a2, a3);
    if (static_cast<int>((a0 >> b) & 1ull) - static_cast<int>((a1 >> b) & 1ull) == 1) return 1;
    const int hd = static_cast<int>((a2 >> b) & 1ull) - static_cast<int>((a3 >> b) & 1ull);
    if (hd == 1) return 2;
    int diag = m - 1;
    if (c > 0) { uint64_t l0, l1, l2, l3; rtk_tb_get(tbp + 4ull * RTK_TB(c - 1, w, ncols), l0, l1, l2, l3); diag = cur - hd - (static_cast<int>((l0 >> b) & 1ull) - static_cast<int>((l1 >> b) & 1ull)); }
    return (diag == cur) ? 0 : 3;
}

RTK_FN void rtk_myers_traceback(const MyersScratch& sc_, MySeq q_, MySeq t_, bool iupac_, uint32_t* n_moves_) {
    const MyersScratch& sc = *rtk_u(&sc_); RTK_ASSUME_LDS(&sc); uint32_t* n_moves = rtk_u(n_moves_); const bool iupac = rtk_u(iupac_);
    MySeq q, t; q.p = rtk_u(q_.p); q.n = rtk_u(q_.n); q.rev = rtk_u(q_.rev); t.p = rtk_u(t_.p); t.n = rtk_u(t_.n); t.rev = rtk_u(t_.rev);
    const int m = q.n, n = t.n;
    int cur;
#ifndef RTK_SIM
    SweepStat fst; fst.plain = false;
    if (m <= 4096 && !q.rev && !t.rev) fst = rtk_myers_fast_any<1, 0>(q.p, m, t.p, n, 1, iupac, rtk_ld(&sc.tb));
    if (fst.plain) { cur = fst.final_score; rtk_sync(); }
    else
#endif
    { rtk_myers_pass(sc, q, t, 1, iupac, 1, nullptr, nullptr); cur = rtk_ld(rtk_ld(&sc.colscore) + (n - 1)); }
    rtk_myers_walk(sc, m, n, n, cur, n_moves);
}
RTK_FN void rtk_myers_column(const uint64_t* fin_pv_, const uint64_t* fin_mv_, int m_, int n_, int32_t* out_, int dlo_, int dhi_, int gran_) {
    const uint64_t* fin_pv = rtk_u(fin_pv_); const uint64_t* fin_mv = rtk_u(fin_mv_); const int m = rtk_u(m_), n = rtk_u(n_); int32_t* out = rtk_u(out_);
    const int dlo = rtk_u(dlo_), dhi = rtk_u(dhi_), gran = rtk_u(gran_);
    const int W = (m + 63) >> 6, Wa = rtk_band_words(m, n, dlo);
    for (int w0 = 0, base = n; w0 < W; w0 += RTK_WAVE) {
        const int w = w0 + rtk_lane();
        int delta = 0;
        uint64_t pv = 0, mv = 0;
        const bool have = w < Wa;
        if (have) {
            pv = fin_pv[w]; mv = fin_mv[w];
            const int rows = (m - 64 * w) < 64 ? (m - 64 * w) : 64;
            const uint64_t mask = rows == 64 ? ~0ull : ((1ull << rows) - 1ull);
            pv &= mask; mv &= mask;
            delta = rtk_popc(pv) - rtk_popc(mv);
        }
        int total;
        const int excl = rtk_wave_excl_scan(delta, &total);
        if (w < W) {
            const int rows = (m - 64 * w) < 64 ? (m - 64 * w) : 64;
            if (have && rtk_band_chi(w, W, n, dhi, gran) == n - 1) {
                int v = base + excl;
                for (int b = 0; b < rows; ++b) { v += static_cast<int>((pv >> b) & 1ull) - static_cast<int>((mv >> b) & 1ull); out[64 * w + b] = v; }
            } else for (int b = 0; b < rows; ++b) out[64 * w + b] = RTK_BAND_INF;
        }
        base += total;
    }
    rtk_sync();
}

#ifndef RTK_SIM
#include "rtk_myers_lvl.h"
#endif
#if defined(RTK_MULTIWAVE) && !defined(RTK_SIM)
__device__ __noinline__ void rtk_myers_leaf_item(RtkCoop* st, int wave, int x) {
    int32_t* const L = reinterpret_cast<int32_t*>(rtk_u(reinterpret_cast<unsigned long long>(st->llist)));
    const char* const q = reinterpret_cast<const char*>(rtk_u(reinterpret_cast<unsigned long long>(st->lq)));
// ... 231 lines not shown
```

### ratatosk_amd/csrc/hip/rtk_pipeline.inc

```
#include "rtk_seeds.h"
#include "rtk_region.h"
#include "rtk_region_enum.h"
#include "rtk_region_lane.h"
#ifdef RTK_SIM
thread_local RlEnv rl_env; thread_local uint32_t rl_lst[RL_S_N * RL_STRIDE]; thread_local uint64_t rl_peq_all[RL_NSYM * RL_MAXW * RL_STRIDE];
#endif
#include "rtk_phasing.h"
#include "rtk_fixsnps.h"
#ifndef RTK_SIM
#include "rtk_phase_long.h"
#endif

RTK_GLOBAL void k_set_ctx(LaunchCtx* out, GraphView g, OptsView o, BatchView bv, RegionBatch rb) {
    if (RTK_BLOCK_ID == 0 && rtk_lane() == 0) { out->g = g; out->o = o; out->bv = bv; out->rb = rb; }
}

#ifdef RTK_SIM
#define RTK_SEED_SCRATCH(sc, expr) const SeedScratch sc = (expr)
#else
#define RTK_SEED_SCRATCH(sc, expr) __shared__ SeedScratch sc; sc = (expr); __syncthreads()
#endif
RTK_GLOBAL void k_mask(const LaunchCtx* L, BatchView bv, const uint64_t* items, uint32_t n_items, uint32_t seg_w, char* scratch, uint64_t stride, SeedScratchCfg cfg, int grid) {
    RTK_SEED_SCRATCH(sc, seed_scratch_carve(scratch + static_cast<uint64_t>(RTK_BLOCK_ID) * stride, cfg));
    for (uint32_t it = static_cast<uint32_t>(RTK_BLOCK_ID); it < n_items; it += static_cast<uint32_t>(grid)) {
// ... 44 lines not shown
    rtk_graph* g = nullptr;
    uint32_t n = 0; uint64_t n_bases = 0;
    std::vector<uint64_t> roff;
    std::vector<std::pair<void*, uint64_t> > owned;
    BatchView bv;
    rtk_stats stats;
    RegionBatch rb;
    bool seeded = false, ran = false;
    rtk_stream_t stream = 0; bool has_stream = false;
    void (*on_region_slab)(void*) = nullptr; void* on_region_slab_arg = nullptr;
    rtk_stream_t stream2 = 0; bool has_stream2 = false; rtk_event_t ev[2];
    rtk_stream_t lane_stream() { if (!has_stream2) { stream2 = rtk_stream_create_high(); ev[0] = rtk_event_create(); ev[1] = rtk_event_create(); has_stream2 = true; } return stream2; }
    RtkTimer t_all;
    void* h_out = nullptr; uint64_t h_out_bytes = 0; std::vector<uint64_t> h_off; std::vector<uint32_t> h_sl, h_ql;
    char* d_raw = nullptr; uint64_t* d_raw_off = nullptr; uint64_t raw_bases = 0; uint32_t raw_max_len = 0; bool has_raw = false, phased = false, snps_fixed = false;
    uint64_t* d_mask_items = nullptr; uint32_t n_mask_items = 0, mask_seg = 0;
    LaunchCtx* d_ctx = nullptr;
    LaunchCtx* ctx() { if (!d_ctx) d_ctx = alloc<LaunchCtx>(1); return d_ctx; }
    void alloc_arrays() {
        bv.hits = alloc<uint64_t>(n_bases + 64);
        bv.hitmap = alloc<uint64_t>(n_bases / 64 + 4);
        bv.masked = alloc<char>(n_bases + 64);
        bv.wdesc = alloc<uint64_t>(n_bases + 64);
        bv.ipool_cap = std::max<uint64_t>(4096, n_bases / 2) + 4096ull * 4096ull;
        bv.ipool = alloc<uint64_t>(2 * bv.ipool_cap);
        bv.ipool_top = alloc<unsigned long long>(1);
        bv.s_pos = alloc<uint32_t>(n_bases + 64); bv.n_solid = alloc<uint32_t>(n);
        bv.wk_cap = std::max<uint64_t>(4096, n_bases / 2); bv.wk_pos = alloc<uint32_t>(bv.wk_cap); bv.wk_hit = alloc<uint64_t>(bv.wk_cap); bv.wk_top = alloc<unsigned long long>(1);
        bv.w_off = alloc<uint64_t>(n); bv.w_cnt = alloc<uint32_t>(n);
        bv.status = alloc<uint32_t>(n); bv.counters = alloc<unsigned long long>(RTK_CNT_TOTAL);
    }
    rtk_batch() { memset(&bv, 0, sizeof(bv)); memset(&stats, 0, sizeof(stats)); memset(&rb, 0, sizeof(rb)); }
    char* arena = nullptr; uint64_t arena_bytes = 0, arena_top = 0;
    void arena_reserve(uint64_t bytes) { if (arena || !bytes) return; uint64_t got = 0; arena = static_cast<char*>(g->pool_take(bytes, &got)); owned.push_back(std::make_pair(static_cast<void*>(arena), got)); arena_bytes = got; arena_top = 0; }
    template <class T> T* alloc(uint64_t count) {
        const uint64_t bytes = (sizeof(T) * (count ? count : 1) + 255ull) & ~255ull;
        if (arena && arena_top + bytes <= arena_bytes) { T* p = reinterpret_cast<T*>(arena + arena_top); arena_top += bytes; return p; }
        uint64_t got = 0; void* p = g->pool_take(bytes, &got); owned.push_back(std::make_pair(p, got)); return static_cast<T*>(p);
    }
    ~rtk_batch() { if (has_stream2) { try { rtk_ssync(stream2); } catch (...) {} rtk_stream_destroy(stream2); rtk_event_destroy(ev[0]); rtk_event_destroy(ev[1]); } if (has_stream) { try { rtk_ssync(stream); } catch (...) {} rtk_stream_destroy(stream); } if (g) { if (h_out) g->stage_give(h_out, h_out_bytes); for (size_t i = 0; i < owned.size(); ++i) g->pool_give(owned[i].first, owned[i].second); graph_release(g); } }
};

static bool opts_ok(const rtk_opts* o) { return o->struct_size == static_cast<uint32_t>(sizeof(rtk_opts)); }
static OptsView opts_view(const rtk_opts* o) {
    OptsView v;
    v.insert_sz = static_cast<uint32_t>(o->insert_sz); v.min_cov_vertices = static_cast<uint32_t>(o->min_cov_vertices);
    v.max_len_weak_region1 = static_cast<uint32_t>(o->max_len_weak_region1); v.max_km_cov = static_cast<uint32_t>(o->max_km_cov > 0xFFFFFFFFull ? 0xFFFFFFFFull : o->max_km_cov);
    v.weak_region_len_factor = o->weak_region_len_factor; v.large_k_factor = o->large_k_factor; v.min_score = o->min_score; v.max_qual = o->max_qual; v.out_qual = o->out_qual; v.min_confidence_snp_corr = o->min_confidence_snp_corr;
    v.a2_exclusive = (o->a2_exclusive == 2) ? 2u : (o->a2_exclusive ? 1u : 0u); v.a3_strand_order = o->a3_strand_order ? 1u : 0u; v.d1_desc = o->d1_desc ? 1u : 0u;
    v.fa_linked_always = rtk_knob_fa_linked_always() ? 1u : 0u;
    v.strand2_mode = rtk_knob_strand2_always() ? 1u : (rtk_knob_strand2_audit() ? 2u : 0u);
    v.colours_mode = rtk_knob_colours_route() | (rtk_knob_colours_audit() << 2);
    v.park_eager = rtk_knob_park_eager() ? 1u : 0u;
    v.long_read_correct = o->long_read_correct ? 1 : 0; v.max_len_weak_region2 = static_cast<uint32_t>(o->max_len_weak_region2 > 0xFFFFFFFFull ? 0xFFFFFFFFull : o->max_len_weak_region2);
    return v;
}

static uint32_t mask_seg() { const uint32_t unit = 64u * RTK_WAVE; uint32_t v = rtk_knob_mask_seg(); v = (v + unit - 1) / unit * unit; return v ? v : unit; }

static uint64_t rtk_batch_arena_bytes(uint64_t n_bases, uint64_t n, bool with_qual, uint64_t raw_bases) {
    return 66ull * n_bases + (with_qual ? 2ull * n_bases : 0ull) + 2ull * raw_bases + 640ull * n + (300ull << 20);
}
static thread_local uint64_t t_arena_extra = 0;
static uint64_t rtk_second_pass_extra(uint64_t n_bases, uint64_t raw_bases) { return 42ull * n_bases + 2ull * raw_bases + (64ull << 20); }
extern "C" int rtk_graph_reserve_batches(rtk_graph* g, uint32_t n_batches, uint64_t bases_per_batch, uint32_t reads_per_batch, int with_qualities, uint64_t raw_bases_per_batch) {
    if (!g) return rtk_fail(RTK_ERR_ARG, "rtk_graph_reserve_batches: null argument");
    if (!g->on_device) return rtk_fail(RTK_ERR_NO_DEVICE, "rtk_graph_reserve_batches: graph is not resident on a device");
#ifdef RTK_SIM
    (void)n_batches; (void)bases_per_batch; (void)reads_per_batch; (void)with_qualities; (void)raw_bases_per_batch; return RTK_OK;
#else
    std::vector<std::pair<void*, uint64_t> > held; int rc = RTK_OK;
    try {
        rtk_set_device(g->device);
        const uint64_t want = rtk_batch_arena_bytes(bases_per_batch, reads_per_batch, with_qualities != 0, 0) + (raw_bases_per_batch ? rtk_second_pass_extra(bases_per_batch, raw_bases_per_batch) : 0ull);
        for (uint32_t i = 0; i < n_batches; ++i) {
            size_t fr = 0, tot = 0;
            if (hipMemGetInfo(&fr, &tot) != hipSuccess || static_cast<uint64_t>(fr) < want + static_cast<uint64_t>(tot) / 8) { rc = rtk_fail(RTK_ERR_DEVICE, "rtk_graph_reserve_batches: not all reserved (less than an eighth of the device memory would stay free)"); break; }
            uint64_t got = 0; void* p = g->pool_take(want, &got); held.push_back(std::make_pair(p, got));
        }
    } catch (const std::exception& e) { rc = rtk_fail(RTK_ERR_DEVICE, std::string("rtk_graph_reserve_batches: ") + e.what()); }
    for (size_t j = 0; j < held.size(); ++j) g->pool_give(held[j].first, held[j].second);
    try {
        std::vector<std::pair<void*, uint64_t> > hh;
        const uint64_t in_b = bases_per_batch * (with_qualities ? 2ull : 1ull) + 16ull * reads_per_batch + (1ull << 16), out_b = 2ull * (bases_per_batch + bases_per_batch / 8) + 8;
        for (uint32_t i = 0; i < n_batches; ++i) {
            uint64_t got = 0; void* p = g->stage_take(in_b, &got); hh.push_back(std::make_pair(p, got));
            p = g->stage_take(out_b, &got); hh.push_back(std::make_pair(p, got));
            if (raw_bases_per_batch) { p = g->stage_take(raw_bases_per_batch + 64, &got); hh.push_back(std::make_pair(p, got)); }
        }
        for (size_t j = 0; j < hh.size(); ++j) g->stage_give(hh[j].first, hh[j].second);
    } catch (const std::exception& e) { if (rc == RTK_OK) rc = rtk_fail(RTK_ERR_DEVICE, std::string("rtk_graph_reserve_batches: ") + e.what()); }
    return rc;
#endif
}

extern "C" int rtk_batch_create(rtk_graph* g, uint32_t n, const char* const* seq, const char* const* qual, const uint32_t* len, rtk_batch** out) {
    if (!g || !seq || !len || !out) return rtk_fail(RTK_ERR_ARG, "rtk_batch_create: null argument");
    bool have_qual = qual != nullptr;
    for (uint32_t i = 0; have_qual && i < n; ++i) have_qual = qual[i] != nullptr || len[i] == 0;
    if (!g->on_device) return rtk_fail(RTK_ERR_NO_DEVICE, "rtk_batch_create: graph is not resident on a device (call rtk_graph_upload); there is no CPU fallback");
    try {
        rtk_set_device(g->device);
        std::unique_ptr<rtk_batch> b(new rtk_batch());
        b->g = g; b->n = n; g->refs.fetch_add(1);
        b->stream = rtk_stream_create(); b->has_stream = true;
        b->roff.assign(n + 1, 0);
// ... 389 lines not shown
```

### ratatosk_amd/csrc/hip/rtk_pipeline_run.inc

```

RTK_GLOBAL void k_enum(const LaunchCtx* L, BatchView bv, int grid) {
#ifdef RTK_SIM
    unsigned char comp_tab[256];
#else
    __shared__ unsigned char comp_tab[256];
#endif
    for (uint32_t c = static_cast<uint32_t>(rtk_lane()); c < 256u; c += RTK_WAVE) comp_tab[c] = static_cast<unsigned char>(rtk_comp(static_cast<char>(c)));
    rtk_sync();
    for (uint32_t ri = static_cast<uint32_t>(RTK_BLOCK_ID); ri < bv.n_reads; ri += static_cast<uint32_t>(grid)) rtk_enum_regions(L->g, L->bv, L->rb, bv.order[ri], comp_tab);
}

RTK_DEV bool rtk_region_is_heavy(const BatchView& bv, const RegionDesc& rd) {
    if (rd.kind == RTK_RG_GAP) { const uint32_t* sp = bv.s_pos + bv.roff[rd.read]; return (sp[rd.i_solid + 1] - sp[rd.i_solid]) >= 160u; }
    return rd.kind == RTK_RG_HEAD || rd.kind == RTK_RG_TAIL;
}
RTK_DEV bool rtk_gap_is_easy(const GraphView& g, const OptsView& o, const BatchView& bv, const RegionDesc& rd, bool* shortcut, UMap* ua_out, uint32_t* len_unitig_km_out, uint32_t* min_pos_out) {
    const uint64_t base = bv.roff[rd.read]; const uint32_t* sp = bv.s_pos + base; const uint32_t k = static_cast<uint32_t>(g.k);
    const uint32_t pa = sp[rd.i_solid], pb = sp[rd.i_solid + 1];
    const UMap ua = rtk_unpack_hit(bv.hits[base + pa]), ub = rtk_unpack_hit(bv.hits[base + pb]);
    *shortcut = false;
    bool same = (ua.unitig == ub.unitig) && (ua.strand == ub.strand);
    if (same && !(g.flags[ua.unitig] & RTK_F_SHORT_CYCLE)) {
        const uint32_t min_pos = ua.dist < ub.dist ? ua.dist : ub.dist, max_pos = ua.dist < ub.dist ? ub.dist : ua.dist;
        const uint32_t len_query_km = pb - pa, len_unitig_km = max_pos - min_pos;
// ... 257 lines not shown
        RTK_PAIR_REGION();
#ifdef RTK_PROF
        {
            const uint64_t* ht = reinterpret_cast<const uint64_t*>(g.ht.get()); const uint64_t nsl = g.ht_slots ? g.ht_slots : 1;
            uint64_t x = (idx * 0x9E3779B97F4A7C15ull) ^ (static_cast<uint64_t>(RTK_BLOCK_ID) << 20);
            unsigned long long t0_ = rtk_clock();
            for (int q = 0; q < 4; ++q) { x = rtk_u(ht[2ull * ((x >> 7) % nsl)]) + x * 0x9E3779B97F4A7C15ull + q; }
            unsigned long long t1_ = rtk_clock();
            uint64_t y = x & 7ull;
            for (int q = 0; q < 4; ++q) { y = (rtk_u(g.uoff[y & 63ull]) + y) & 63ull; }
            unsigned long long t2_ = rtk_clock();
            volatile uint64_t* slab = reinterpret_cast<volatile uint64_t*>(sc->str[RTK_STR_PROBE].get());
            slab[rtk_lane()] = y + x; const uint64_t z = slab[(rtk_lane() + 1) & 63];
            unsigned long long t3_ = rtk_clock() + (z & 1ull);
            sc->prof[RTK_LAP_PROBE_COLD] += t1_ - t0_; sc->prof[RTK_LAP_PROBE_WARM] += t2_ - t1_; sc->prof[RTK_LAP_PROBE_SLAB] += t3_ - t2_; sc->prof[RTK_LAP_PROBE_SAMPLES] += 1; sc->prof_t = rtk_clock();
        }
#endif
        const unsigned long long t0 = rtk_clock();
        const unsigned long long exp0 = RTK_HIST_GET(*sc, RTK_H_DFS_RUNNING);
        rtk_region_program(c, rd);
        { const unsigned long long dt = rtk_clock() - t0; sc->cnt[RTK_RC_CYC_TOTAL] += dt;
#if !defined(RTK_SIM)
          if (trace_class < -1) { ++n_mine; if (dt > dt_max) { dt_max = dt; idx_of_max = idx; } }
#endif
          int hb = RTK_GAP_CLASS_HEAD_TAIL;
          if (rd->kind == RTK_RG_GAP) { const uint32_t* sp = bv.s_pos + bv.roff[rd->read]; const uint32_t gl = sp[rd->i_solid + 1] - sp[rd->i_solid]; hb = rtk_gap_class(gl); }
          else if (rd->kind != RTK_RG_HEAD && rd->kind != RTK_RG_TAIL) hb = -1;
          if (hb >= 0) { RTK_HIST_ADD(*sc, RTK_H_CYCLES + hb, dt); RTK_HIST_ADD(*sc, RTK_H_REGIONS + hb, 1); RTK_HIST_ADD(*sc, RTK_H_DFS + hb, RTK_HIST_GET(*sc, RTK_H_DFS_RUNNING) - exp0); } }
        rd->status = *sc->overflow;
        if (*sc->overflow && rtk_lane() == 0) {
            rtk_atomic_add(rb.n_overflow, 1ull);
            if (stolen) { const unsigned long long at = rtk_atomic_add(rb.n_heavy.get() + 4, 1ull); rb.horder[at] = ri; }
        }
    }
#if !defined(RTK_SIM)
    if (trace_class < -1 && rtk_lane() == 0) {
        const unsigned long long wall1 = wall_clock64();
        atomicMax(reinterpret_cast<unsigned long long*>(bv.counters + RTK_CNT_WAVE_TRACE + 0), dt_max); atomicMax(reinterpret_cast<unsigned long long*>(bv.counters + RTK_CNT_WAVE_TRACE + 1), ~wall0); atomicMax(reinterpret_cast<unsigned long long*>(bv.counters + RTK_CNT_WAVE_TRACE + 2), wall1);
        rtk_atomic_add(bv.counters + RTK_CNT_WAVE_TRACE + 3, wall1 - wall0); rtk_atomic_add(bv.counters + RTK_CNT_WAVE_TRACE + 4, 1ull);
        if (dt_max > 0 && atomicMax(reinterpret_cast<unsigned long long*>(bv.counters + RTK_CNT_WAVE_TRACE + 5), dt_max) < dt_max) bv.counters[RTK_CNT_WAVE_TRACE + 6] = idx_of_max;
        atomicMax(reinterpret_cast<unsigned long long*>(bv.counters + RTK_CNT_WAVE_TRACE + 7), n_mine);
    }
#endif
    if (rtk_lane() == 0) {
        rtk_atomic_add(bv.counters + RTK_CNT_EXPAND, sc->cnt[RTK_RC_EXPAND]); rtk_atomic_add(bv.counters + RTK_CNT_COLOUR, sc->cnt[RTK_RC_COLOUR]); rtk_atomic_add(bv.counters + RTK_CNT_PATHBASE, sc->cnt[RTK_RC_PATHBASE]);
        rtk_atomic_add(bv.counters + RTK_CNT_ALIGN, sc->cnt[RTK_RC_ALIGN]); rtk_atomic_add(bv.counters + RTK_CNT_CELLS, sc->cnt[RTK_RC_CELLS]);
        for (int i = 0; i < 6; ++i) rtk_atomic_add(bv.counters + RTK_CNT_CYC + i, sc->cnt[RTK_RC_CYC_COLOUR + i]);
        rtk_atomic_add(bv.counters + RTK_CNT_CYC_SETS, sc->cnt[RTK_RC_CYC_PATHREC]); rtk_atomic_add(bv.counters + RTK_CNT_CYC_TOSTRING, sc->cnt[RTK_RC_CYC_TOSTRING]); rtk_atomic_add(bv.counters + RTK_CNT_CYC_PATHQUAL, sc->cnt[RTK_RC_CYC_PATHQUAL]); rtk_atomic_add(bv.counters + RTK_CNT_WALK_CYCLES, sc->my.walk_cycles); rtk_atomic_add(bv.counters + RTK_CNT_WALK_MOVES, sc->my.walk_moves); rtk_atomic_add(bv.counters + RTK_CNT_WALK_RELOADS, sc->my.walk_reloads); rtk_atomic_add(bv.counters + RTK_CNT_WALK_SCALAR, sc->my.walk_scalar); rtk_atomic_add(bv.counters + RTK_CNT_WALK_CALLS, sc->my.walk_calls); rtk_atomic_add(bv.counters + RTK_CNT_WALK_TAIL, sc->my.walk_tail_cycles); rtk_atomic_add(bv.counters + RTK_CNT_CYC_DFS, sc->cnt[RTK_RC_CYC_DFS]); rtk_atomic_add(bv.counters + RTK_CNT_CYC_COLOUR_OK, sc->cnt[RTK_RC_CYC_COLOUR_OK]);
        for (int i = 0; i < RTK_FINE_N; ++i) rtk_atomic_add(bv.counters + RTK_CNT_FINE + i, sc->fine[i]);
        for (int i = RTK_RC_TRIM_STORED; i < RTK_RC_FA_LINKED_RUN; ++i) rtk_atomic_add(bv.counters + RTK_CNT_ROUTES + (i - RTK_RC_TRIM_STORED), sc->cnt[i]);
        for (int i = RTK_RC_FA_LINKED_RUN; i < RTK_RC_STRAND2_RUN; ++i) rtk_atomic_add(bv.counters + RTK_CNT_FA_LINKED + (i - RTK_RC_FA_LINKED_RUN), sc->cnt[i]);
        for (int i = RTK_RC_STRAND2_RUN; i < RTK_RC_PARK_WALKED; ++i) rtk_atomic_add(bv.counters + RTK_CNT_STRAND2 + (i - RTK_RC_STRAND2_RUN), sc->cnt[i]);
        for (int i = RTK_RC_PARK_WALKED; i < RTK_RC_COLOURS_SMALL; ++i) rtk_atomic_add(bv.counters + RTK_CNT_PARK + (i - RTK_RC_PARK_WALKED), sc->cnt[i]);
        for (int i = RTK_RC_COLOURS_SMALL; i < RTK_RC_N; ++i) rtk_atomic_add(bv.counters + RTK_CNT_COLOURS + (i - RTK_RC_COLOURS_SMALL), sc->cnt[i]);
        for (int i = 0; i < RTK_H_N; ++i) rtk_atomic_add(bv.counters + RTK_CNT_HIST + i, static_cast<unsigned long long>(RTK_HIST_GET(*sc, i)));
#ifdef RTK_PROF
        for (int i = 0; i < RTK_LAP_N; ++i) rtk_atomic_add(bv.counters + RTK_CNT_PROF + i, static_cast<unsigned long long>(sc->prof[i]));
#endif
    }
}

RTK_GLOBAL void k_stitch(const LaunchCtx* L, BatchView bv, int grid) {
    for (uint32_t ri = static_cast<uint32_t>(RTK_BLOCK_ID); ri < bv.n_reads; ri += static_cast<uint32_t>(grid)) rtk_stitch_offsets(L->bv, L->rb, bv.order[ri]);
}
RTK_GLOBAL void k_stitch_copy(const LaunchCtx* L, uint64_t n_regions, int grid) {
    for (uint64_t c0 = static_cast<uint64_t>(RTK_BLOCK_ID) * RTK_WAVE; c0 < n_regions; c0 += static_cast<uint64_t>(grid) * RTK_WAVE) rtk_stitch_copy(L->rb, c0, n_regions);
}

static bool region_compact() { return rtk_knob_compact(); }
static int region_waves_that_fit(uint64_t stride, uint64_t held, bool trace) {
    int w = rtk_knob_region_waves();
#ifndef RTK_SIM
    size_t fr = 0, tot = 0;
    if (hipMemGetInfo(&fr, &tot) == hipSuccess && stride) {
        const uint64_t room = (static_cast<uint64_t>(fr) + held) / 10 * 7;
        if (trace) fprintf(stderr, "[rtk trace] region work areas: %.1f GB free + %.1f GB held of %.1f GB, %d waves x %.1f MB wanted\n", fr / 1073741824.0, held / 1073741824.0, tot / 1073741824.0, w, stride / 1048576.0);
        if (static_cast<uint64_t>(w) * stride > room) { uint64_t f = room / stride / 256 * 256; if (f < 512) f = 512; if (f < static_cast<uint64_t>(w)) w = static_cast<int>(f); }
    }
#else
    (void)stride; (void)held; (void)trace;
#endif
    return w;
}

static RegionScratchCfg region_cfg(uint32_t max_len_exact, int attempt) {
    RegionScratchCfg c;
    uint32_t max_len = 131072u; while (max_len < max_len_exact) max_len <<= 1;
    if (attempt == 0 && rtk_knob_test_tiny_scratch()) {
        c.str_cap = 2048; c.my.w_cap = c.str_cap / 64 + 2; c.my.t_cap = c.str_cap; c.my.r_cap = c.str_cap; c.my.mv_cap = 2 * c.str_cap;
        c.my.tb_cap_words = 4ull * 52429 + 64; c.set_cap = 64; c.um_cap = 8; c.list_cap = 64; c.memo_cap = 16; c.bm_words = max_len / 64 + 8; c.arena_cap = 8192;
        return c;
    }
    if (region_compact()) {
        if (attempt == 0) {
            c.str_cap = 65536; c.my.w_cap = c.str_cap / 64 + 2; c.my.t_cap = c.str_cap; c.my.r_cap = c.str_cap; c.my.mv_cap = 2 * c.str_cap;
            c.my.tb_cap_words = 4ull * 8192 + 64; c.set_cap = 4096; c.um_cap = 512; c.list_cap = 1024; c.memo_cap = 512; c.bm_words = c.str_cap / 64 + 8; c.arena_cap = 128u << 10;
            return c;
        }
        attempt -= 1;
    }
    const uint32_t scale = 1u << (3 * attempt);
    c.str_cap = std::max<uint32_t>(65536u, (5u * max_len) / 2u + 1024u) * scale;
    c.my.w_cap = c.str_cap / 64 + 2; c.my.t_cap = c.str_cap; c.my.r_cap = c.str_cap; c.my.mv_cap = 2 * c.str_cap;
    c.my.tb_cap_words = std::max<uint64_t>(4ull * 52429 + 64, 4ull * c.my.w_cap + 64);
    c.set_cap = 16384u * scale; c.um_cap = 2048u * scale; c.list_cap = 4096u * scale; c.memo_cap = 2048u * scale;
    c.bm_words = max_len / 64 + 8; c.arena_cap = (1ull << 20) * scale;
    return c;
// ... 283 lines not shown
        const unsigned long long* h = cnt + RTK_CNT_HIST;
        fprintf(stderr, "[rtk trace] k_regions by size class (share of region time, regions, avg kcycles, second-strand share, DFS calls per region):");
        for (int i = 0; i < RTK_GAP_CLASSES; ++i) {
            const unsigned long long cyc = h[RTK_H_CYCLES + i], n = h[RTK_H_REGIONS + i];
            if (n) fprintf(stderr, " [%s %.3f n=%llu %.0fk bw=%.2f dfs=%.1f]", hn[i], double(cyc) / total, n, 1e-3 * double(cyc) / double(n), double(h[RTK_H_STRAND2 + i]) / double(n),
                           double(h[RTK_H_DFS + i]) / double(n));
        }
        fprintf(stderr, "\n");
    }
    {
        static const char* const fine_names[RTK_FINE_N] = {
            "colour: class unions", "fixAmbiguity: path alignment", "fixAmbiguity: walk of the moves",
            "fixAmbiguity: linked alleles (k-mer lookups)", "fixAmbiguity: apply", "colour small: bit vectors (or array: shared_with(all))",
            "colour small: classes + selection (or array: set ops)", "region: side lists", "region: trim alignment", "region: fixAmbiguity",
            "consensus: merge logic", "paths: explore_paths outside DFS", "colour: small path (cycles)", "colour: 4096-bit path (cycles)",
            "colour: small path calls / total cycles", "colour: 4096-bit path calls / total cycles"};
        const unsigned long long* f = cnt + RTK_CNT_FINE;
        fprintf(stderr, "[rtk trace] chooseColors calls: small path %llu, 4096-bit path %llu; fixAmbiguity calls %llu, of which left by the all-confident way out %llu\n",
                f[RTK_FINE_COL_S_CALLS], f[RTK_FINE_COL_B_CALLS], f[RTK_FINE_FA_CALLS], f[RTK_FINE_FA_ALL_CONFIDENT]);
        fprintf(stderr, "[rtk trace] k_regions fine shares:");
        for (int i = 0; i < RTK_FINE_N; ++i) if (f[i]) fprintf(stderr, " [%s %.3f]", fine_names[i], double(f[i]) / total);
        fprintf(stderr, "\n");
    }
#ifdef RTK_LANE_PROF
    {
        static const char* const ln[RL_NPROF] = {
            "driver", "side lists", "chooseColors", "search glue", "dfs walk", "colour_ok", "to_string", "peq build", "sweep", "walk",
            "path records", "path qual", "select", "amb collect", "fixAmbiguity", "assemble", "trim", "revcomp", "consensus", "emit",
            "idle at round end", "colours: universe", "colours: rows", 0};
        static_assert(RL_NPROF == RTK_CNT_LANE_PROF2 - RTK_CNT_LANE_PROF, "counter map: the lane profile has RL_NPROF slots");
        const unsigned long long* p1 = cnt + RTK_CNT_LANE_PROF; const unsigned long long* p2 = cnt + RTK_CNT_LANE_PROF2;
        unsigned long long tot = 0; for (int i = 0; i < RL_NPROF; ++i) tot += p1[i];
        fprintf(stderr, "[rtk trace] k_regions_lanes lap profile (%.3g lane cycles):", double(tot));
        for (int i = 0; i < RL_NPROF; ++i) if (p1[i] && ln[i]) fprintf(stderr, " [%s %.4f]", ln[i], double(p1[i]) / double(tot ? tot : 1));
        fprintf(stderr, "\n");
        unsigned long long tw = 0; for (int i = 0; i < RL_NPROF; ++i) tw += p2[i];
        fprintf(stderr, "[rtk trace] k_regions_lanes wave-time estimate by slot (share of %.3g, lanes together):", double(tw) / 64.0);
        for (int i = 0; i < RL_NPROF; ++i)
            if (p2[i] && ln[i]) fprintf(stderr, " [%s %.4f x%.1f]", ln[i], double(p2[i]) / double(tw ? tw : 1), 64.0 * double(p1[i]) / double(p2[i]));
        fprintf(stderr, "\n");
    }
#endif
    fprintf(stderr, "[rtk trace] k_regions shares of %.3g wave cycles: colour %.3f paths %.3f consensus %.3f myers %.3f sets %.3f tostring %.3f pathqual %.3f "
                    "walk %.3f\n",
            double(cnt[RTK_CNT_CYC_TOTAL]), share(RTK_CNT_CYC_COLOUR), share(RTK_CNT_CYC_PATHS), share(RTK_CNT_CYC_CONSENSUS), share(RTK_CNT_CYC_MYERS),
            share(RTK_CNT_CYC_SETS),
            share(RTK_CNT_CYC_TOSTRING), share(RTK_CNT_CYC_PATHQUAL), share(RTK_CNT_WALK_CYCLES));
    fprintf(stderr, "[rtk trace] k_regions cycle shares: DFS bookkeeping %.3f (of which colour checks %.3f)\n", share(RTK_CNT_CYC_DFS), share(RTK_CNT_CYC_COLOUR_OK));
    fprintf(stderr, "[rtk trace] trims: by column %llu (of which stored %llu), by the distance call %llu, cycles %.3g; consensus calls: forward alignment resumed %llu, swept %llu\n",
            cnt[RTK_CNT_ROUTES + 0] + cnt[RTK_CNT_ROUTES + 1], cnt[RTK_CNT_ROUTES + 0], cnt[RTK_CNT_ROUTES + 2], double(cnt[RTK_CNT_FINE + RTK_FINE_TRIM]), cnt[RTK_CNT_ROUTES + 3], cnt[RTK_CNT_ROUTES + 4]);
    fprintf(stderr, "[rtk trace] fixAmbiguity linked-allele searches: run %llu, skipped %llu, entries produced %llu, cycles %.3g\n", cnt[RTK_CNT_FA_LINKED + 0], cnt[RTK_CNT_FA_LINKED + 1],
            cnt[RTK_CNT_FA_LINKED + 2], double(cnt[RTK_CNT_FINE + RTK_FINE_FA_LINKED]));
    fprintf(stderr, "[rtk trace] second strand of gap regions: run %llu, skipped %llu (the forward result decides), audit mismatches %llu\n", cnt[RTK_CNT_STRAND2 + 0], cnt[RTK_CNT_STRAND2 + 1], cnt[RTK_CNT_STRAND2 + 2]);
    fprintf(stderr, "[rtk trace] stored sweeps of the forward trims: walked for a consensus %llu, never walked %llu\n", cnt[RTK_CNT_PARK + 0], cnt[RTK_CNT_PARK + 1]);
    fprintf(stderr, "[rtk trace] colour selections answered by: small %llu, wide %llu, bits %llu, general %llu; audit mismatches %llu; handed on by the register program for room %llu\n", cnt[RTK_CNT_COLOURS + 0], cnt[RTK_CNT_COLOURS + 1], cnt[RTK_CNT_COLOURS + 2],
            cnt[RTK_CNT_COLOURS + 3], cnt[RTK_CNT_COLOURS + 4], cnt[RTK_CNT_COLOURS + 5]);
    fprintf(stderr, "[rtk trace] walks %llu moves %llu reloads %llu scalar steps %llu cycles %.3g tail cycles %.3g\n", cnt[RTK_CNT_WALK_CALLS], cnt[RTK_CNT_WALK_MOVES],
            cnt[RTK_CNT_WALK_RELOADS], cnt[RTK_CNT_WALK_SCALAR], double(cnt[RTK_CNT_WALK_CYCLES]), double(cnt[RTK_CNT_WALK_TAIL]));
}

static void region_stats(RegionRun& R, const unsigned long long* cnt) {
    rtk_batch* b = R.b; rtk_stats& st = b->stats;
    st.cyc_colour = cnt[RTK_CNT_CYC_COLOUR]; st.cyc_paths = cnt[RTK_CNT_CYC_PATHS]; st.cyc_consensus = cnt[RTK_CNT_CYC_CONSENSUS]; st.cyc_total = cnt[RTK_CNT_CYC_TOTAL];
    st.cyc_myers = cnt[RTK_CNT_CYC_MYERS]; st.cyc_sets = cnt[RTK_CNT_CYC_SETS]; st.cyc_tostring = cnt[RTK_CNT_CYC_TOSTRING]; st.cyc_pathqual = cnt[RTK_CNT_CYC_PATHQUAL];
    st.cyc_walk = cnt[RTK_CNT_WALK_CYCLES]; st.n_moves = cnt[RTK_CNT_WALK_MOVES];
    st.n_slots_exact = cnt[RTK_CNT_SLOTS_EXACT]; st.n_slots_inexact = cnt[RTK_CNT_SLOTS_INEXACT];
    st.ms_regions = R.t_enum.elapsed() + (R.n_regions ? R.t_easy.elapsed() : 0.0);
    st.ms_lanes = R.lanes_on ? R.t_lanes.elapsed() : 0.0;
    st.ms_correct = R.ms_reg + ((R.lanes_on && !R.lanes_beside) ? st.ms_lanes : 0.0);
    st.n_lane_handed = cnt[RTK_CNT_LANE_HANDED]; st.n_lane_regions = cnt[RTK_CNT_LANE_HANDED] + cnt[RTK_CNT_LANE_DONE];
    st.n_trim_stored = cnt[RTK_CNT_ROUTES + 0]; st.n_trim_column = cnt[RTK_CNT_ROUTES + 1]; st.n_trim_fallback = cnt[RTK_CNT_ROUTES + 2];
    st.n_consensus_resumed = cnt[RTK_CNT_ROUTES + 3]; st.n_consensus_swept = cnt[RTK_CNT_ROUTES + 4];
    st.n_fa_linked_run = cnt[RTK_CNT_FA_LINKED + 0]; st.n_fa_linked_skipped = cnt[RTK_CNT_FA_LINKED + 1]; st.n_fa_linked_entries = cnt[RTK_CNT_FA_LINKED + 2];
    st.n_strand2_run = cnt[RTK_CNT_STRAND2 + 0]; st.n_strand2_skipped = cnt[RTK_CNT_STRAND2 + 1]; st.n_strand2_audit_mismatch = cnt[RTK_CNT_STRAND2 + 2];
    st.n_park_walked = cnt[RTK_CNT_PARK + 0]; st.n_park_deferred = cnt[RTK_CNT_PARK + 1];
    st.n_colours_small = cnt[RTK_CNT_COLOURS + 0]; st.n_colours_wide = cnt[RTK_CNT_COLOURS + 1]; st.n_colours_bits = cnt[RTK_CNT_COLOURS + 2]; st.n_colours_general = cnt[RTK_CNT_COLOURS + 3];
    st.n_colours_audit_mismatch = cnt[RTK_CNT_COLOURS + 4]; st.n_colours_declined_fit = cnt[RTK_CNT_COLOURS + 5];
    st.ms_stitch = R.t_st.elapsed(); st.ms_total = b->t_all.elapsed();
    st.n_windows = b->n_bases;
    st.n_probes_exact = cnt[RTK_CNT_PROBES_EXACT]; st.n_probes_inexact = cnt[RTK_CNT_PROBES_INEXACT]; st.n_hits_inexact = cnt[RTK_CNT_HITS_INEXACT];
    st.n_regions = R.n_regions; st.n_region_items = R.n_regions; st.n_arena_overflow = R.n_ovf_total;
    st.n_expand = cnt[RTK_CNT_EXPAND]; st.n_colour_elem = cnt[RTK_CNT_COLOUR]; st.n_path_base = cnt[RTK_CNT_PATHBASE];
    st.n_align = cnt[RTK_CNT_ALIGN]; st.n_align_cells = cnt[RTK_CNT_CELLS];
    st.in_bases = b->n_bases; st.out_bases = R.out_top / 2;
}

extern "C" int rtk_batch_run_regions(rtk_batch* b, const rtk_opts* opts) {
    int rc = batch_precheck(b, opts, "rtk_batch_run_regions");
    if (rc) return rc;
    if (!b->seeded) return rtk_fail(RTK_ERR_ARG, "rtk_batch_run_regions: rtk_batch_run_seeds has not completed for this batch");
    if (opts->long_read_correct && !b->bv.qual.get())
        return rtk_fail(RTK_ERR_ARG, "rtk_batch_run_regions: the second pass (long_read_correct) needs a batch created with quality strings");
    rtk_graph* g = b->g;
    try {
        rtk_set_device(g->device);
        RegionRun R = {};
        R.b = b; R.g = g; R.ov = opts_view(opts); R.sm = b->stream; R.own_slab = opts->long_read_correct != 0;
        R.hold.g = g; R.hold.what = -1; R.slab.g = g;
        R.trace = rtk_knob_trace(); R.w0 = std::chrono::steady_clock::now();
        for (uint32_t i = 0; i < b->n; ++i) R.max_len = std::max<uint32_t>(R.max_len, static_cast<uint32_t>(b->roff[i + 1] - b->roff[i]));
        R.grid = default_grid();
        region_alloc(R);
        region_lane_class(R);
        R.lap("alloc");
        region_enumerate(R);
        R.lap("enum");
        region_easy(R);
        region_lanes(R);
        region_take_areas(R);
        rc = region_attempts(R);
        if (rc) return rc;
        R.hold.release();
        R.lap("regions");
        rc = region_stitch(R);
        if (rc) return rc;
        unsigned long long cnt[RTK_CNT_TOTAL]; rtk_d2h_s(cnt, b->bv.counters, sizeof(cnt), R.sm);
        if (R.trace) region_trace_report(cnt);
        region_stats(R, cnt);
        R.lap("done");
        if (b->h_out) { g->stage_give(b->h_out, b->h_out_bytes); b->h_out = nullptr; }
        b->ran = true; b->seeded = false;
    } catch (const std::exception& e) { return rtk_fail(RTK_ERR_DEVICE, e.what()); }
    return RTK_OK;
}

extern "C" int rtk_batch_run(rtk_batch* b, const rtk_opts* opts) {
    const int rc = rtk_batch_run_seeds(b, opts);
    return rc ? rc : rtk_batch_run_regions(b, opts);
// ... 252 lines not shown
```

### ratatosk_amd/csrc/hip/rtk_region.h

```cpp
#ifndef RTK_REGION_H
#define RTK_REGION_H

#include "rtk_region_types.h"
#include "rtk_region_paths.h"
#include "rtk_sim_census.h"
#include "rtk_region_align.h"
#include "rtk_ambiguity.h"
#include "rtk_region_search.h"
#include "rtk_colours.h"
#include "rtk_region_result.h"
#include "rtk_consensus.h"

RTK_DEV int rtk_bifrost_code(char ch) { const int x = (ch & 4) >> 1; return x + ((x ^ (ch & 2)) >> 1); }

template <class Cond, class Fn>
RTK_DEV void rtk_scan_anchor_runs(const Anchors& a, int64_t start, int step, Cond in_range, Fn fn) {
    uint32_t prev_unitig = RTK_NONE32; bool first = true;
    for (int64_t b = 0;; b += RTK_WAVE) {
        const int64_t x = start + static_cast<int64_t>(step) * (b + rtk_lane());
        bool ok = false; UMap um = rtk_um_empty();
        if (x >= 0 && x < static_cast<int64_t>(a.n)) { ok = in_range(rtk_an_pos(a, static_cast<uint32_t>(x))); if (ok) um = rtk_an_um(a, static_cast<uint32_t>(x)); }
        const uint64_t okm = rtk_ballot(ok);
        const int lead = (~okm == 0ull) ? RTK_WAVE : (rtk_ffs(~okm) - 1);
        if (lead == 0) break;
// ... 307 lines not shown
            rtk_correct_region(c, s_bw, L, so_r, we_r, i_solid_rev, i_weak_rev, nullptr, bw, q_fw);
            if (rtk_failed(s)) return;
            rtk_rc_reverse_complement(s, bw, s.bm[RTK_BM_RC_TMP], s.rbuf[RTK_RB_RC_TMP]);
            rtk_app(s, out_s, &osl, bw.seq, bw.seq_len >= k ? bw.seq_len - k : bw.seq_len);
            rtk_app(s, out_q, &oql, bw.qual, bw.qual_len >= k ? bw.qual_len - k : bw.qual_len);
        } else { rtk_app(s, out_s, &osl, s_fw, so.pos[0]); app_q(0, so.pos[0], q_min); }
    } else if (kind == RTK_RG_GAP) {
        const uint32_t i = rtk_u(rd->i_solid), prev_pos = rtk_u(rd->prev_pos);
        const uint32_t pa = rtk_u(so.pos[i]), pb = rtk_u(so.pos[i + 1]);
        const UMap ua = rtk_u(rtk_an_um(so, i)), ub = rtk_u(rtk_an_um(so, i + 1));
        const uint32_t i_weak = rtk_u(rtk_an_first_ge(we, 0, we.n, pa));
        bool isUncorrected = false;
        bool sameUnitig = (ua.unitig == ub.unitig) && (ua.strand == ub.strand);
        if (lrc && has_min_qual(pa, pb + k)) isUncorrected = true;
        else if (sameUnitig && !(c.g.flags[ua.unitig] & RTK_F_SHORT_CYCLE)) {
            const uint32_t min_pos = ua.dist < ub.dist ? ua.dist : ub.dist, max_pos = ua.dist < ub.dist ? ub.dist : ua.dist;
            const uint32_t len_query_km = pb - pa, len_unitig_km = max_pos - min_pos;
            uint64_t mn, mx; rtk_min_max_len(len_unitig_km, c.o.weak_region_len_factor, &mn, &mx);
            sameUnitig = sameUnitig && ((ua.strand && (ua.dist < ub.dist)) || (!ua.strand && (ua.dist > ub.dist)));
            sameUnitig = sameUnitig && (len_query_km >= mn) && (len_query_km <= mx);
            RTK_PL(s, RTK_LAP_DRIVER_DISPATCH);
            if (sameUnitig) {
                UMap sub = ua; sub.dist = min_pos; sub.len = len_unitig_km + 1;
                const uint32_t sl = rtk_ums_to_string(c, &sub, 1, s.str[RTK_STR_CAND]); if (sl == 0xFFFFFFFFu) return;
                rtk_app(s, out_s, &osl, s_fw + prev_pos, pa - prev_pos);
                rtk_app(s, out_s, &osl, s.str[RTK_STR_CAND], sl >= k ? sl - k : sl);
                if (lrc) {
                    const uint32_t buff = (sl >= 2 * k) ? k : (sl - k);
                    rtk_app(s, out_q, &oql, q_fw + prev_pos, pa - prev_pos + buff);
                    if (sl - buff - k > 0) rtk_app_fill(s, out_q, &oql, q_max, sl - buff - k);
                } else rtk_app_fill(s, out_q, &oql, q_max, (pa - prev_pos) + (sl - k));
                RTK_PL(s, RTK_LAP_DRIVER_SAME_UNITIG);
            } else isUncorrected = true;
        } else if (pb >= pa + k) {
            RTK_PL(s, RTK_LAP_DRIVER_DISPATCH);
            rtk_correct_region(c, s_fw, L, so, we, i, i_weak, nullptr, fw, q_fw, true);
            if (rtk_failed(s)) return;
            const uint32_t l_solid = pa - prev_pos;
            auto emit_minus_k = [&](const char* seq, uint32_t sl, const char* q, uint32_t ql) {
                const uint32_t ts = l_solid + sl, tq = l_solid + ql;
                const uint32_t ks = ts >= k ? ts - k : ts, kq = tq >= k ? tq - k : tq;
                rtk_app(s, out_s, &osl, s_fw + prev_pos, ks < l_solid ? ks : l_solid); if (ks > l_solid) rtk_app(s, out_s, &osl, seq, ks - l_solid);
                app_q(prev_pos, kq < l_solid ? kq : l_solid, q_max); if (kq > l_solid) rtk_app(s, out_q, &oql, q, kq - l_solid);
            };
            const uint32_t s2_mode = rtk_u(c.o.strand2_mode);
            const bool skippable = !fw.is_corrected && s2_mode != 1u && rtk_strand2_skippable(c, fw, s_fw, pa, pb, so, i, we, i_weak);
            if (fw.is_corrected) emit_minus_k(fw.seq, fw.seq_len, fw.qual, fw.qual_len);
            else if (skippable && s2_mode == 0u) {
                s.cnt[RTK_RC_STRAND2_SKIPPED] += 1;
                s.cnt[RTK_RC_CONS_RESUMED] += 1;
                emit_minus_k(fw.seq, fw.seq_len, fw.qual, fw.qual_len);
            } else {
                s.cnt[skippable ? RTK_RC_STRAND2_SKIPPED : RTK_RC_STRAND2_RUN] += 1;
                rtk_park_walk(c);
                auto audit = [&](const char* seq, uint32_t sl, const char* q, uint32_t ql) {
                    if (skippable && !(sl == fw.seq_len && ql == fw.qual_len && rtk_str_equal(seq, fw.seq, sl) && rtk_str_equal(q, fw.qual, ql))) s.cnt[RTK_RC_STRAND2_AUDIT_MISMATCH] += 1;
                };
                const uint32_t i_solid_bw = so.n - i - 2;
                uint32_t i_weak_bw = we.n - i_weak;
                i_weak_bw = rtk_an_first_gt(we_r, 0, i_weak_bw, rtk_an_pos(so_r, i_solid_bw));
                RTK_PL(s, RTK_LAP_DRIVER_STRAND2);
                { const uint32_t gl_ = pb - pa; RTK_HIST_ADD(s, RTK_H_STRAND2 + rtk_gap_class(gl_), 1); }
                rtk_correct_region(c, s_bw, L, so_r, we_r, i_solid_bw, i_weak_bw, &fw, bw, q_bw);
                if (rtk_failed(s)) return;
                RTK_PL(s, RTK_LAP_DRIVER_STRAND2);
                rtk_rc_reverse_complement(s, bw, s.bm[RTK_BM_RC_TMP], s.rbuf[RTK_RB_RC_TMP]);
                if (bw.is_corrected) {
                    audit(bw.seq, bw.seq_len, bw.qual, bw.qual_len);
                    emit_minus_k(bw.seq, bw.seq_len, bw.qual, bw.qual_len);
                } else {
                    const uint32_t ref_len = pb - pa + k;
                    uint32_t& csl = s.loc.len[RTK_LEN_CONS_SEQ]; uint32_t& cql = s.loc.len[RTK_LEN_CONS_QUAL]; csl = 0; cql = 0;
                    const unsigned long long tc0 = rtk_clock();
                    const bool ok = rtk_generate_consensus(c, &fw, &bw, s_fw + pa, ref_len, c.o.weak_region_len_factor, s.rbuf[RTK_RB_CONS_SEQ], &csl, s.rbuf[RTK_RB_CONS_QUAL], &cql);
                    s.cnt[RTK_RC_CYC_CONSENSUS] += rtk_clock() - tc0;
                    RTK_PL(s, RTK_LAP_CONS_FINAL);
                    if (rtk_failed(s)) return;
                    if (!ok || csl == 0) {
                        csl = 0; cql = 0;
                        rtk_app(s, s.rbuf[RTK_RB_CONS_SEQ], &csl, s_fw + pa, ref_len);
                        if (lrc) rtk_app(s, s.rbuf[RTK_RB_CONS_QUAL], &cql, q_fw + pa, ref_len);
                        else { rtk_app_fill(s, s.rbuf[RTK_RB_CONS_QUAL], &cql, q_max, k); rtk_app_fill(s, s.rbuf[RTK_RB_CONS_QUAL], &cql, q_min, pb - pa); }
                    }
                    audit(s.rbuf[RTK_RB_CONS_SEQ], csl, s.rbuf[RTK_RB_CONS_QUAL], cql);
                    emit_minus_k(s.rbuf[RTK_RB_CONS_SEQ], csl, s.rbuf[RTK_RB_CONS_QUAL], cql);
                }
            }
        } else isUncorrected = true;
        if (isUncorrected) {
            rtk_app(s, out_s, &osl, s_fw + prev_pos, pb - prev_pos);
            if (lrc) rtk_app(s, out_q, &oql, q_fw + prev_pos, pb - prev_pos);
            else {
                rtk_app_fill(s, out_q, &oql, q_max, pa - prev_pos);
                if (pb < pa + k) rtk_app_fill(s, out_q, &oql, q_max, pb - pa);
                else { rtk_app_fill(s, out_q, &oql, q_max, k); rtk_app_fill(s, out_q, &oql, q_min, pb - pa - k); }
            }
        }
    } else if (kind == RTK_RG_TAIL) {
        const uint32_t i = rd->i_solid, prev_pos = rd->prev_pos;
        const uint32_t pa = so.pos[i];
        const uint32_t i_weak = rtk_an_first_ge(we, 0, we.n, pa);
        if (lrc && has_min_qual(pa, L)) {
            rtk_app(s, out_s, &osl, s_fw + prev_pos, L - prev_pos); rtk_app(s, out_q, &oql, q_fw + prev_pos, L - prev_pos);
        } else {
            rtk_correct_region(c, s_fw, L, so, we, i, i_weak, nullptr, fw, q_fw);
            if (rtk_failed(s)) return;
            const uint32_t l_solid = pa - prev_pos;
// ... 18 lines not shown
```

### ratatosk_amd/csrc/hip/rtk_region_align.h

```cpp
#ifndef RTK_REGION_ALIGN_H
#define RTK_REGION_ALIGN_H

#include "rtk_region_paths.h"
#include "rtk_sim_census.h"

#ifdef RTK_SIM
#include <assert.h>
#endif

RTK_FN_HOT MyersResult rtk_align(const RCtx& c, const char* q_, uint32_t m_, const char* t_, uint32_t n_, int kk_, int mode_, bool iupac_ = true) {
    RegionScratch& s = *rtk_u(c.sc); const char* q = rtk_u(q_); const char* t = rtk_u(t_);
    const uint32_t m = rtk_u(m_), n = rtk_u(n_); const int kk = rtk_u(kk_), mode = rtk_u(mode_); const bool iupac = rtk_u(iupac_);
    s.cnt[RTK_RC_ALIGN] += 1; s.cnt[RTK_RC_CELLS] += static_cast<unsigned long long>((m + 63) / 64) * n;
    const unsigned long long t0 = rtk_clock();
    rtk_site_note(m, n, kk, false); rtk_pair_note(q, m, t, n);
    const MyersResult r = rtk_myers_distance(s.my, q, static_cast<int>(m), t, static_cast<int>(n), kk, mode, iupac);
    s.cnt[RTK_RC_CYC_MYERS] += rtk_clock() - t0;
    return r;
}

RTK_FN_HOT MyersResult rtk_align_path(const RCtx& c_, const char* q_, uint32_t m_, const char* t_, uint32_t n_, int mode_, uint32_t* n_moves_) {
    const RCtx& c = *rtk_u(&c_); RegionScratch& s = rtk_hdr(c); const char* q = rtk_u(q_); const char* t = rtk_u(t_);
    const uint32_t m = rtk_u(m_), n = rtk_u(n_); const int mode = rtk_u(mode_); uint32_t* n_moves = rtk_u(n_moves_);
    s.cnt[RTK_RC_ALIGN] += (m > 0 && n > 0) ? 2 : 1; s.cnt[RTK_RC_CELLS] += static_cast<unsigned long long>((m + 63) / 64) * n;
    const unsigned long long t0 = rtk_clock();
    rtk_site_note(m, n, -1, true); rtk_pair_note(q, m, t, n);
    const MyersResult r = rtk_myers_path(s.my, q, static_cast<int>(m), t, static_cast<int>(n), mode, true, n_moves);
    s.cnt[RTK_RC_CYC_MYERS] += rtk_clock() - t0;
    return r;
}

RTK_FN void rtk_park_walk(const RCtx& c_) {
    const RCtx& c = *rtk_u(&c_); RegionScratch& s = rtk_hdr(c);
    TrimPark& pk = s.loc.park;
    if (!pk.pending) return;
#ifdef RTK_SIM
    assert(pk.gen == s.my.tb_gen);
#endif
    const unsigned long long t1 = rtk_clock();
    pk.pending = 0;
    uint32_t& nm = pk.nm; nm = 0;
    rtk_myers_walk(s.my, static_cast<int>(pk.len), static_cast<int>(pk.n), static_cast<int>(pk.n), pk.dist, &nm);
    if (nm <= s.str_cap) rtk_wcopy(s.rbuf[RTK_RB_PARK_MOVES], s.my.moves, nm);
    else nm = 0;
    s.cnt[RTK_RC_PARK_WALKED] += 1; s.cnt[RTK_RC_PARK_DEFERRED] -= 1;
    s.cnt[RTK_RC_CYC_MYERS] += rtk_clock() - t1;
}

RTK_FN bool rtk_trim_by_column(const RCtx& c_, const char* raw_, uint32_t n_, const char* corr_, uint32_t m_, bool park_, MyersResult* out_) {
    const RCtx& c = *rtk_u(&c_); RegionScratch& s = rtk_hdr(c); const char* raw = rtk_u(raw_); const char* corr = rtk_u(corr_);
    const uint32_t n = rtk_u(n_), m = rtk_u(m_); const bool park = rtk_u(park_); MyersResult* out = rtk_u(out_);
    const unsigned long long t0 = rtk_clock();
    const bool ok = rtk_myers_shw_by_column(s.my, corr, static_cast<int>(m), raw, static_cast<int>(n), true, park ? 1 : 0, 0, out, nullptr);
    s.cnt[RTK_RC_CYC_MYERS] += rtk_clock() - t0;
    if (!ok) return false;
    s.cnt[RTK_RC_ALIGN] += 1; s.cnt[RTK_RC_CELLS] += static_cast<unsigned long long>((m + 63) / 64) * n;
    RTK_SITE(park ? RTK_SITE_TRIM_STORED : RTK_SITE_TRIM_COLUMN); rtk_site_note(m, n, -1, park); rtk_pair_note(corr, m, raw, n);
    s.cnt[park ? RTK_RC_TRIM_STORED : RTK_RC_TRIM_COLUMN] += 1;
    if (!park) return true;
    s.cnt[RTK_RC_PARK_DEFERRED] += 1;
    const uint32_t keep = (out->first == -1) ? 0u : static_cast<uint32_t>(out->last + 1);
    const long long W = (keep + 63) >> 6;
    if (keep == 0 || keep > s.my.r_cap || keep + n > s.my.mv_cap || !((2LL * 8 + 4) * W * n + 8LL * n < 1024 * 1024)) return true;
    const unsigned long long t1 = rtk_clock();
    TrimPark& pk = s.loc.park;
    pk.nm = 0; pk.len = keep; pk.dist = out->dist; pk.n = n; pk.gen = rtk_ld(&s.my.tb_gen); pk.pending = 1;
    pk.last_move = rtk_myers_last_move(s.my, static_cast<int>(keep), static_cast<int>(n), static_cast<int>(n), out->dist);
    s.cnt[RTK_RC_CYC_MYERS] += rtk_clock() - t1;
    if (rtk_u(c.o.park_eager) || keep + n > s.str_cap) rtk_park_walk(c);
    return true;
}

#endif
```

### ratatosk_amd/csrc/hip/rtk_region_types.h

```cpp
#ifndef RTK_REGION_TYPES_H
#define RTK_REGION_TYPES_H

#include "rtk_myers.h"
#include "rtk_seeds.h"
#include "rtk_types.h"
#include "rtk_wave.h"

struct RegionDesc {
    uint32_t read;
    uint32_t kind;
    uint32_t i_solid;
    uint32_t prev_pos;
    uint64_t seg_off;
    uint32_t seq_len, qual_len;
    uint32_t status;
    uint32_t pad;
};
#define RTK_RG_WHOLE_MAX 0
#define RTK_RG_WHOLE_MIN 1
#define RTK_RG_HEAD 2
#define RTK_RG_GAP 3
#define RTK_RG_TAIL 4
#define RTK_RG_TAIL_COPY 5

// ... 53 lines not shown
    RTK_OVF_AMB = 11,
    RTK_OVF_CONS_STALL = 11,
    RTK_OVF_SEG_POOL = 12,
    RTK_OVF_REPEAT_QUAL = 14
};

enum RtkLap {
    RTK_LAP_DRIVER_DISPATCH = 0, RTK_LAP_DRIVER_SAME_UNITIG = 1, RTK_LAP_REGION_PROLOGUE = 2, RTK_LAP_REGION_SIDE_LISTS = 3, RTK_LAP_REGION_COLOURS = 4,
    RTK_LAP_SEMIWEAK_GLUE = 5, RTK_LAP_PATHS_PROLOGUE = 6, RTK_LAP_EXPLORE_PREFIX = 7, RTK_LAP_DFS_POP = 8, RTK_LAP_DFS_COLOUR_OK = 9,
    RTK_LAP_DFS_T_EXTEND = 10, RTK_LAP_DFS_T_STRING = 11, RTK_LAP_DFS_T_SWEEP = 12, RTK_LAP_DFS_T_COMMIT = 13, RTK_LAP_DFS_NT_EXTEND = 14,
    RTK_LAP_DFS_NT_REST = 15, RTK_LAP_DFS_POST_SCORE = 16, RTK_LAP_DFS_POST_STRING = 17, RTK_LAP_DFS_POST_QUAL = 18, RTK_LAP_DFS_POST_COMMIT = 19,
    RTK_LAP_PATHS_AFTER_EXPLORE = 20, RTK_LAP_PATHS_SELECT = 21, RTK_LAP_SEMIWEAK_MERGE = 22, RTK_LAP_REGION_RESTART = 23, RTK_LAP_REGION_ASSEMBLE = 24,
    RTK_LAP_REGION_FIX_AMBIGUITY = 25, RTK_LAP_REGION_TRIM = 26, RTK_LAP_DRIVER_STRAND2 = 27, RTK_LAP_CONS_ENTRY = 28, RTK_LAP_CONS_FW_PATH = 29,
    RTK_LAP_CONS_BW_PATH = 30, RTK_LAP_CONS_MERGE = 31, RTK_LAP_CONS_FINAL = 32, RTK_LAP_DRIVER_EMIT_PREP = 33, RTK_LAP_DEQUEUE = 34, RTK_LAP_EMIT = 35,
    RTK_LAP_PROBE_COLD = 40, RTK_LAP_PROBE_WARM = 41, RTK_LAP_PROBE_SLAB = 42, RTK_LAP_PROBE_SAMPLES = 43,
    RTK_LAP_N = 48
};
static_assert(RTK_LAP_N == RTK_CNT_PROF_END - RTK_CNT_PROF, "lap slots: the counter map holds one word per slot");

enum RtkSite {
    RTK_SITE_NONE = 0,
    RTK_SITE_SCORE_TERMINAL = 1,
    RTK_SITE_SCORE_REF_IN_PATH = 2,
    RTK_SITE_SCORE_PATH_IN_REF = 3,
    RTK_SITE_PATH_QUAL = 4,
    RTK_SITE_EXPLORE_PREFIX = 5,
    RTK_SITE_SELECT_NT = 6,
    RTK_SITE_RESIZE_BEST = 7,
    RTK_SITE_REPEATS_PATH = 8,
    RTK_SITE_REPEATS_TURN = 9,
    RTK_SITE_SELECT_BFS = 10,
    RTK_SITE_SELECT_PARTIAL_RETRY = 11,
    RTK_SITE_SELECT_PARTIAL = 12,
    RTK_SITE_TRIM_FALLBACK = 13,
    RTK_SITE_CONS_FW = 14, RTK_SITE_CONS_BW = 15, RTK_SITE_CONS_FINAL = 16,
    RTK_SITE_FIX_AMBIGUITY = 17,
    RTK_SITE_TRIM_STORED = 18, RTK_SITE_TRIM_COLUMN = 19
};

enum RtkHist { RTK_H_CYCLES = 0, RTK_H_REGIONS = 8, RTK_H_STRAND2 = 16, RTK_H_DFS = 24, RTK_H_DFS_RUNNING = 31, RTK_H_N = 32 };
enum { RTK_GAP_CLASS_HEAD_TAIL = 7, RTK_GAP_CLASSES = 8 };
static_assert(RTK_H_N == RTK_CNT_HIST_END - RTK_CNT_HIST, "size-class table: the counter map holds one word per slot");
#define rtk_gap_class(gap_len) ((gap_len) < 40 ? 0 : (gap_len) < 64 ? 1 : (gap_len) < 128 ? 2 : (gap_len) < 256 ? 3 : (gap_len) < 512 ? 4 : (gap_len) < 1024 ? 5 : 6)

struct RegionScratchCfg { ScratchCfg my; uint32_t set_cap, um_cap, str_cap, list_cap, memo_cap, bm_words; uint64_t arena_cap; };

struct WPath { U<UMap*> ums; U<char*> qual; U<uint32_t> n, l, qlen; };

struct Anchors { U<const uint32_t*> pos; U<const uint64_t*> hit; U<const uint64_t*> hits_by_pos; U<uint32_t> n, L; U<int> rev; U<int> k; };
struct SideList { uint32_t* u; uint8_t* nb; uint32_t n, cap; };
struct ResCorr { char* seq; char* qual; uint32_t seq_len, qual_len; uint64_t* bm; uint32_t old_len; bool is_corrected; uint32_t n_all; int all_set; };
struct RegionCall { const char* s_read; const char* q_read; uint64_t complete; UMap um1, um2; uint32_t s_len, p1, p2, first_pos, len_weak_region, lw_lo, lw_hi, n_all, n_partial, n_amb, has_end_pt, found_first, lrc; };
struct TrimPark { uint32_t nm, len; int32_t dist; uint32_t n, last_move, pending, gen; };
struct DriverLocals { Anchors an[RTK_AN_N]; ResCorr rc[RTK_RES_N]; SideList side[RTK_SIDE_N]; uint32_t len[RTK_LEN_N]; int best[RTK_BEST_N]; MyersSaved saved; RegionCall call; TrimPark park; MyersResult trim; };

struct RegionScratch {
    MyersScratch my;
    U<uint32_t*> set[RTK_SET_N]; U<uint32_t> set_cap;
    U<char*> arena[RTK_ARENA_N]; U<uint64_t> arena_cap; U<uint64_t> top[RTK_ARENA_N];
    WPath wp[RTK_WP_N]; U<uint32_t> um_cap;
    U<char*> str[RTK_STR_N]; U<uint32_t> str_cap;
    U<char*> rbuf[RTK_RB_N];
    U<uint64_t*> list[RTK_L_N]; U<uint32_t> list_cap;
    U<uint32_t*> memo_u; U<uint8_t*> memo_v; U<uint32_t> memo_cap; U<uint32_t> memo_n;
    U<uint64_t*> bm[RTK_BM_N]; U<uint32_t> bm_words;
    UL<uint32_t*> overflow; U<uint32_t> ovf_word;
    DriverLocals loc;
    U<unsigned long long> cnt[RTK_RC_N];
    U<unsigned long long> fine[RTK_FINE_N];
#ifdef RTK_PROF
    U<unsigned long long> prof[RTK_LAP_N]; U<unsigned long long> prof_t;
#endif
#ifndef RTK_SLIM_HDR
    U<unsigned long long> hist[RTK_H_N];
#endif
};
#ifdef RTK_SLIM_HDR
#define RTK_HIST_ADD(sc, i, v) ((void)0)
#define RTK_HIST_GET(sc, i) 0ull
#else
#define RTK_HIST_ADD(sc, i, v) ((sc).hist[i] += (v))
#define RTK_HIST_GET(sc, i) ((sc).hist[i])
#endif
#ifdef RTK_PROF
#define RTK_PL(sc, i) do { const unsigned long long t_ = rtk_clock(); (sc).prof[i] += t_ - (sc).prof_t; (sc).prof_t = t_; } while (0)
#else
#define RTK_PL(sc, i) ((void)0)
#endif

struct LaunchCtx { GraphView g; OptsView o; BatchView bv; RegionBatch rb; };

struct RCtx {
    const GraphView& g; const OptsView& o; const BatchView& bv; const RegionBatch& rb;
    UL<RegionScratch*> sc;
    U<int> k;
};

RTK_DEV RegionScratch& rtk_hdr(const RCtx& c) { RegionScratch* p = c.sc; RTK_ASSUME_LDS(p); return *p; }

RTK_HD uint64_t region_scratch_bytes(const RegionScratchCfg& c) {
    uint64_t b = scratch_bytes(c.my);
    b += 4ull * RTK_SET_N * c.set_cap + 1ull * RTK_ARENA_N * c.arena_cap + 1ull * RTK_WP_N * (sizeof(UMap) * c.um_cap + c.str_cap) + (1ull * RTK_STR_N + RTK_RB_N) * c.str_cap;
    b += 8ull * RTK_L_N * c.list_cap + 5ull * c.memo_cap + 8ull * RTK_BM_N * c.bm_words + sizeof(RegionScratch) + 1024;
    return (b + 255) / 256 * 256;
}

// ... 37 lines not shown
```

### ratatosk_amd/csrc/hip/rtk_seeds.h

```cpp
#ifndef RTK_SEEDS_H
#define RTK_SEEDS_H

#include "rtk_myers.h"
#include "rtk_sets.h"
#include "rtk_types.h"
#include "rtk_wave.h"

struct OptsView {
    U<uint32_t> insert_sz, min_cov_vertices, max_len_weak_region1, max_km_cov;
    U<double> weak_region_len_factor, large_k_factor, min_score;
    U<int32_t> max_qual, out_qual;
    U<double> min_confidence_snp_corr;
    U<int32_t> long_read_correct;
    U<uint32_t> max_len_weak_region2;
    U<uint32_t> d1_desc;
    U<uint32_t> a3_strand_order;
    U<uint32_t> a2_exclusive;
    U<uint32_t> fa_linked_always;
    U<uint32_t> strand2_mode;
    U<uint32_t> colours_mode;
    U<uint32_t> park_eager;
};

struct BatchView {
    U<uint32_t> n_reads;
    U<uint64_t> n_bases;
    U<const char*> seq;
    U<const char*> qual;
    U<const uint64_t*> roff;
    U<const uint32_t*> order;
    U<uint64_t*> hits;
    U<uint64_t*> hitmap;
    U<char*> masked;
    U<uint64_t*> wdesc;
    U<uint64_t*> ipool;
    U<uint64_t> ipool_cap;
    U<unsigned long long*> ipool_top;
    U<uint32_t*> s_pos;
    U<uint32_t*> n_solid;
    U<uint32_t*> wk_pos;
    U<uint64_t*> wk_hit;
    U<uint64_t> wk_cap;
    U<unsigned long long*> wk_top;
    U<uint64_t*> w_off;
    U<uint32_t*> w_cnt;
    U<uint32_t*> status;
    U<unsigned long long*> counters;
};

struct SeedScratch {
    U<uint32_t*> set[6]; U<uint32_t> set_cap;
    U<uint32_t*> vpos; U<uint64_t*> vcode; U<uint64_t*> vhit; U<uint64_t*> vkey; U<uint64_t*> vidx; U<uint32_t> v_cap;
    U<uint32_t*> gstart; U<uint32_t*> gcnt; U<uint32_t*> gps; U<uint32_t*> gpe; U<uint8_t*> gkeep; U<uint8_t*> vflag;
    U<uint8_t*> sflag;
    U<uint32_t*> overflow;
};


struct SeedScratchCfg { uint32_t set_cap, v_cap, s_cap; };

RTK_HD uint64_t seed_scratch_bytes(const SeedScratchCfg& c) {
    uint64_t b = 0;
    b += 6ull * 4 * c.set_cap;
    b += 4ull * c.v_cap + 8ull * c.v_cap * 2;
    b += 2ull * 8 * (2ull * c.v_cap + 512);
    b += 4ull * 4 * c.v_cap + 2ull * c.v_cap;
    b += c.s_cap; b += 64;
    return (b + 255) / 256 * 256;
}

RTK_HD SeedScratch seed_scratch_carve(char* base, const SeedScratchCfg& c) {
    SeedScratch s; char* p = base;
    s.vcode = reinterpret_cast<uint64_t*>(p); p += 8ull * c.v_cap;
    s.vhit = reinterpret_cast<uint64_t*>(p); p += 8ull * c.v_cap;
// ... 988 lines not shown
```

### ratatosk_amd/csrc/hip/rtk_types.h

```cpp
#ifndef RTK_TYPES_H
#define RTK_TYPES_H

#include <stdint.h>

#if defined(__HIPCC__) && !defined(RTK_SIM)
#include <hip/hip_runtime.h>
#define RTK_HD __host__ __device__ __forceinline__
#else
#define RTK_HD inline
#endif

#if defined(__HIP_DEVICE_COMPILE__) && !defined(RTK_SIM)
template <class T> __device__ __forceinline__ T rtk_u(T v) {
    static_assert(sizeof(T) <= 8, "rtk_u: scalar types only");
    if (sizeof(T) <= 4) {
        uint32_t x = 0; __builtin_memcpy(&x, &v, sizeof(T));
        x = static_cast<uint32_t>(__builtin_amdgcn_readfirstlane(static_cast<int>(x)));
        T r; __builtin_memcpy(&r, &x, sizeof(T)); return r;
    } else {
        uint64_t x = 0; __builtin_memcpy(&x, &v, sizeof(T));
        const uint32_t lo = static_cast<uint32_t>(__builtin_amdgcn_readfirstlane(static_cast<int>(x & 0xFFFFFFFFull)));
        const uint32_t hi = static_cast<uint32_t>(__builtin_amdgcn_readfirstlane(static_cast<int>(x >> 32)));
        x = (static_cast<uint64_t>(hi) << 32) | lo;
        T r; __builtin_memcpy(&r, &x, sizeof(T)); return r;
// ... 93 lines not shown
    x = ((x >> 2) & 0x3333333333333333ull) | ((x & 0x3333333333333333ull) << 2);
    x = ((x >> 4) & 0x0F0F0F0F0F0F0F0Full) | ((x & 0x0F0F0F0F0F0F0F0Full) << 4);
    x = ((x >> 8) & 0x00FF00FF00FF00FFull) | ((x & 0x00FF00FF00FF00FFull) << 8);
    x = ((x >> 16) & 0x0000FFFF0000FFFFull) | ((x & 0x0000FFFF0000FFFFull) << 16);
    x = (x >> 32) | (x << 32);
    return x >> (64 - 2 * k);
}

enum RtkCounterSlot {
    RTK_CNT_WINDOWS = 0, RTK_CNT_PROBES_EXACT = 1, RTK_CNT_PROBES_INEXACT = 2, RTK_CNT_HITS_INEXACT = 3, RTK_CNT_REGIONS = 4, RTK_CNT_ITEMS = 5,
    RTK_CNT_OVERFLOW = 6,
    RTK_CNT_EXPAND = 7, RTK_CNT_COLOUR = 8, RTK_CNT_PATHBASE = 9, RTK_CNT_ALIGN = 10, RTK_CNT_CELLS = 11,
    RTK_CNT_SLOTS_EXACT = 12, RTK_CNT_SLOTS_INEXACT = 13,
    RTK_CNT_EVENTS_END = 14,
    RTK_CNT_SEED_READBACK = 16,
    RTK_CNT_CYC = 16,
    RTK_CNT_CYC_COLOUR = 16, RTK_CNT_CYC_PATHS = 17, RTK_CNT_CYC_CONSENSUS = 18, RTK_CNT_CYC_TOTAL = 19, RTK_CNT_CYC_MYERS = 20, RTK_CNT_CYC_SETS = 21, RTK_CNT_CYC_TOSTRING = 22, RTK_CNT_CYC_PATHQUAL = 23,
    RTK_CNT_CYC_END = 24,
    RTK_CNT_FINALIZE = 24,
    RTK_CNT_FINALIZE_SLOWEST = 31,
    RTK_CNT_FINALIZE_END = 32,
    RTK_CNT_WALK = 32,
    RTK_CNT_WALK_CYCLES = 32, RTK_CNT_WALK_MOVES = 33, RTK_CNT_WALK_RELOADS = 34, RTK_CNT_WALK_SCALAR = 35, RTK_CNT_WALK_CALLS = 36, RTK_CNT_WALK_TAIL = 37,
    RTK_CNT_CYC_DFS = 38, RTK_CNT_CYC_COLOUR_OK = 39,
    RTK_CNT_WALK_END = 40,
    RTK_CNT_FINE = 40,
    RTK_CNT_FINE_END = 56,
    RTK_CNT_HIST = 56,
    RTK_CNT_HIST_END = 88,
    RTK_CNT_PHASE_TRACE = 59,
    RTK_CNT_PHASE_TRACE_END = 64,
    RTK_CNT_FINALIZE_SLOWEST_PHASES = 72,
    RTK_CNT_FINALIZE_SLOWEST_PHASES_END = 79,
    RTK_CNT_PROF = 96,
    RTK_CNT_PROF_END = 144,
    RTK_CNT_WAVE_TRACE = 144,
    RTK_CNT_WAVE_TRACE_END = 152,
    RTK_CNT_LANE_HANDED = 152, RTK_CNT_LANE_DONE = 153,
    RTK_CNT_LANE_END = 154,
    RTK_CNT_ROUTES = 154,
    RTK_CNT_ROUTES_END = 159,
    RTK_CNT_LANE_PROF = 160,
    RTK_CNT_LANE_PROF2 = 184,
    RTK_CNT_LANE_PROF_END = 208,
    RTK_CNT_PHASE_SKIPPED = 210,
    RTK_CNT_FA_LINKED = 211,
    RTK_CNT_FA_LINKED_END = 214,
    RTK_CNT_STRAND2 = 214,
    RTK_CNT_STRAND2_END = 217,
    RTK_CNT_PARK = 217,
    RTK_CNT_PARK_END = 219,
    RTK_CNT_COLOURS = 219,
    RTK_CNT_COLOURS_END = 225,
    RTK_CNT_USED_END = RTK_CNT_COLOURS_END,
    RTK_CNT_TOTAL = (RTK_CNT_USED_END + 31) / 32 * 32
};
static_assert(RTK_CNT_TOTAL == 256, "counter map: the size of the block changed (it is part of what the kernels and the host agree on)");
constexpr bool rtk_cnt_apart(int a, int a_end, int b, int b_end) { return a_end <= b || b_end <= a; }
static_assert(RTK_CNT_EVENTS_END <= RTK_CNT_CYC && RTK_CNT_CYC_END <= RTK_CNT_FINALIZE && RTK_CNT_FINALIZE_END <= RTK_CNT_WALK && RTK_CNT_WALK_END <= RTK_CNT_FINE, "counter map: the event, cycle, finalize and walk ranges overlap");
static_assert(RTK_CNT_FINE_END <= RTK_CNT_HIST && RTK_CNT_HIST_END <= RTK_CNT_PROF && RTK_CNT_PROF_END <= RTK_CNT_WAVE_TRACE && RTK_CNT_WAVE_TRACE_END <= RTK_CNT_LANE_HANDED, "counter map: the trace ranges overlap");
static_assert(RTK_CNT_LANE_END <= RTK_CNT_ROUTES && RTK_CNT_ROUTES_END <= RTK_CNT_LANE_PROF, "counter map: the route counters overlap the lane ranges");
static_assert(RTK_CNT_LANE_END <= RTK_CNT_LANE_PROF && RTK_CNT_LANE_PROF2 - RTK_CNT_LANE_PROF == 24 && RTK_CNT_LANE_PROF_END <= RTK_CNT_PHASE_SKIPPED && RTK_CNT_PHASE_SKIPPED < RTK_CNT_TOTAL, "counter map: the lane ranges overlap");
static_assert(RTK_CNT_PHASE_SKIPPED < RTK_CNT_FA_LINKED && RTK_CNT_FA_LINKED_END <= RTK_CNT_TOTAL, "counter map: the fixAmbiguity counters overlap the phasing slot or leave the block");
static_assert(RTK_CNT_FA_LINKED_END <= RTK_CNT_STRAND2 && RTK_CNT_STRAND2_END <= RTK_CNT_TOTAL, "counter map: the second-strand counters overlap the fixAmbiguity counters or leave the block");
static_assert(RTK_CNT_STRAND2_END <= RTK_CNT_PARK && RTK_CNT_PARK_END <= RTK_CNT_TOTAL, "counter map: the park counters overlap the second-strand counters or leave the block");
static_assert(RTK_CNT_PARK_END <= RTK_CNT_COLOURS && RTK_CNT_COLOURS_END <= RTK_CNT_TOTAL, "counter map: the colour-route counters overlap the park counters or leave the block");
static_assert(rtk_cnt_apart(RTK_CNT_PHASE_TRACE, RTK_CNT_PHASE_TRACE_END, RTK_CNT_FINALIZE_SLOWEST_PHASES, RTK_CNT_FINALIZE_SLOWEST_PHASES_END), "counter map: the two guests of the size-class table overlap");
static_assert(RTK_CNT_HIST <= RTK_CNT_PHASE_TRACE && RTK_CNT_FINALIZE_SLOWEST_PHASES_END <= RTK_CNT_HIST_END, "counter map: the guests of the size-class table left it (update the comment above)");

enum RtkRegionCnt { RTK_RC_EXPAND = 0, RTK_RC_COLOUR = 1, RTK_RC_PATHBASE = 2, RTK_RC_ALIGN = 3, RTK_RC_CELLS = 4,
    RTK_RC_CYC_COLOUR = 5, RTK_RC_CYC_PATHS = 6, RTK_RC_CYC_CONSENSUS = 7, RTK_RC_CYC_TOTAL = 8, RTK_RC_CYC_MYERS = 9, RTK_RC_CYC_SETS = 10,
    RTK_RC_CYC_PATHREC = 11 , RTK_RC_CYC_TOSTRING = 12, RTK_RC_CYC_PATHQUAL = 13, RTK_RC_CYC_DFS = 14, RTK_RC_CYC_COLOUR_OK = 15,
    RTK_RC_TRIM_STORED = 16, RTK_RC_TRIM_COLUMN = 17, RTK_RC_TRIM_FALLBACK = 18, RTK_RC_CONS_RESUMED = 19, RTK_RC_CONS_SWEPT = 20,
    RTK_RC_FA_LINKED_RUN = 21, RTK_RC_FA_LINKED_SKIPPED = 22, RTK_RC_FA_LINKED_ENTRIES = 23,
    RTK_RC_STRAND2_RUN = 24, RTK_RC_STRAND2_SKIPPED = 25, RTK_RC_STRAND2_AUDIT_MISMATCH = 26,
    RTK_RC_PARK_WALKED = 27, RTK_RC_PARK_DEFERRED = 28,
    RTK_RC_COLOURS_SMALL = 29, RTK_RC_COLOURS_WIDE = 30, RTK_RC_COLOURS_BITS = 31, RTK_RC_COLOURS_GENERAL = 32, RTK_RC_COLOURS_AUDIT_MISMATCH = 33, RTK_RC_COLOURS_DECLINED_FIT = 34, RTK_RC_N = 35 };
static_assert(RTK_CNT_ROUTES_END - RTK_CNT_ROUTES == static_cast<int>(RTK_RC_FA_LINKED_RUN) - static_cast<int>(RTK_RC_TRIM_STORED), "counter map: one slot per route counter");
static_assert(RTK_CNT_FA_LINKED_END - RTK_CNT_FA_LINKED == static_cast<int>(RTK_RC_STRAND2_RUN) - static_cast<int>(RTK_RC_FA_LINKED_RUN), "counter map: one slot per fixAmbiguity counter");
static_assert(RTK_CNT_STRAND2_END - RTK_CNT_STRAND2 == static_cast<int>(RTK_RC_PARK_WALKED) - static_cast<int>(RTK_RC_STRAND2_RUN), "counter map: one slot per second-strand counter");
static_assert(RTK_CNT_PARK_END - RTK_CNT_PARK == static_cast<int>(RTK_RC_COLOURS_SMALL) - static_cast<int>(RTK_RC_PARK_WALKED), "counter map: one slot per park counter");
static_assert(RTK_CNT_COLOURS_END - RTK_CNT_COLOURS == static_cast<int>(RTK_RC_N) - static_cast<int>(RTK_RC_COLOURS_SMALL), "counter map: one slot per colour-route counter");
#define RTK_CM_ROUTE 3u
#define RTK_CM_ROUTE_BITS 1u
#define RTK_CM_ROUTE_GENERAL 2u
#define RTK_CM_AUDIT 4u
#define RTK_CM_FAULT 8u
enum RtkRegionFine { RTK_FINE_COL_GENERAL = 0 , RTK_FINE_COL_UNIONS = 0, RTK_FINE_FA_ALIGN = 1, RTK_FINE_FA_WALK = 2, RTK_FINE_FA_LINKED = 3, RTK_FINE_FA_APPLY = 4, RTK_FINE_COL_S_VECTORS = 5, RTK_FINE_COL_S_SELECT = 6,
    RTK_FINE_SIDE_LISTS = 7, RTK_FINE_TRIM = 8, RTK_FINE_FIX_AMBIGUITY = 9, RTK_FINE_FA_CALLS = 10, RTK_FINE_FA_ALL_CONFIDENT = 11, RTK_FINE_COL_S_CYCLES = 12, RTK_FINE_COL_B_CYCLES = 13,
    RTK_FINE_COL_S_CALLS = 14, RTK_FINE_COL_B_CALLS = 15, RTK_FINE_N = 16 };

struct UMap {
    uint32_t unitig;
    uint32_t dist;
    uint32_t len;
    uint32_t strand;
};

RTK_HD UMap rtk_um_empty() { UMap u; u.unitig = RTK_NONE32; u.dist = 0; u.len = 0; u.strand = 1; return u; }
RTK_HD bool rtk_um_is_empty(const UMap& u) { return u.unitig == RTK_NONE32; }
RTK_HD bool rtk_um_eq(const UMap& a, const UMap& b) { return a.unitig == b.unitig && a.dist == b.dist && a.len == b.len && a.strand == b.strand; }

#define RTK_NO_HIT 0xFFFFFFFFFFFFFFFFull
RTK_HD uint64_t rtk_pack_hit(uint32_t unitig, uint32_t dist, uint32_t strand) { return (static_cast<uint64_t>(unitig) << 33) | (static_cast<uint64_t>(dist) << 1) | (strand & 1u); }
RTK_HD UMap rtk_unpack_hit(uint64_t h) { UMap u; u.unitig = static_cast<uint32_t>(h >> 33); u.dist = static_cast<uint32_t>((h >> 1) & 0xFFFFFFFFull); u.len = 1; u.strand = static_cast<uint32_t>(h & 1ull); return u; }

RTK_HD uint64_t rtk_ht_slot(uint64_t hh, uint64_t slots) {
#if defined(__HIP_DEVICE_COMPILE__) && !defined(RTK_SIM)
    return __umul64hi(hh, slots);
#else
    return static_cast<uint64_t>((static_cast<unsigned __int128>(hh) * static_cast<unsigned __int128>(slots)) >> 64);
#endif
}
RTK_HD uint64_t rtk_ht_next(uint64_t i, uint64_t slots) { return i + 1 == slots ? 0 : i + 1; }

RTK_HD uint64_t rtk_find_kmer(const GraphView& g, uint64_t fw, uint32_t* n_probes) {
    const uint64_t rc = rtk_revcomp(fw, g.k);
    const uint64_t can = fw < rc ? fw : rc;
    const uint64_t hh = rtk_hash64(can);
    {
        const uint64_t b1 = (hh >> 12) & g.bf1_mask;
        if (!((g.bf1[b1 >> 6] >> (b1 & 63ull)) & 1ull)) { if (n_probes) *n_probes = 0; return RTK_NO_HIT; }
    }
    {
        const uint64_t bits = (1ull << (hh & 63)) | (1ull << ((hh >> 6) & 63));
        if ((g.bf[(hh >> 32) & g.bf_mask] & bits) != bits) { if (n_probes) *n_probes = 0; return RTK_NO_HIT; }
    }
    uint64_t i = rtk_ht_slot(hh, g.ht_slots);
    uint32_t np = 0;
    while (true) {
        const uint64_t key = g.ht[2 * i];
        ++np;
        if (key == can) {
            const uint64_t v = g.ht[2 * i + 1];
            const uint32_t stored_is_can = static_cast<uint32_t>(v & 1ull), query_is_can = (fw <= rc) ? 1u : 0u;
// ... 80 lines not shown
```

Before: 2.240 billion.

## Keep only last traceback column for parked trim sweeps, re-sweep when walked

The forward trim alignment no longer stores the full Myers traceback table by default. It keeps only the last column's Pv/Mv/Ph/Mh, which is enough to compute the last move. When a parked trim actually has to be walked for a consensus, the sweep is rerun with the full table. This removes the per-cell global stores for trims that are never walked, at the cost of a second sweep for those that are; a knob restores the old table-storing path.

```diff
diff --git a/include/ratatosk_hip.h b/include/ratatosk_hip.h
--- a/include/ratatosk_hip.h
+++ b/include/ratatosk_hip.h
@@ -63,6 +63,7 @@
     uint64_t n_park_walked, n_park_deferred;
     uint64_t n_colours_small, n_colours_wide, n_colours_bits, n_colours_general, n_colours_audit_mismatch;
     uint64_t n_colours_declined_fit;
+    uint64_t n_park_resweeps;
 } rtk_stats;
 
 int rtk_graph_load(const char* unitig_fasta_gz, const char* rtsk, int k, int n_threads, rtk_graph** out);
@@ -132,6 +133,7 @@
 #define RTK_MYERS_MODE_SHW_BY_COLUMN 3
 #define RTK_MYERS_MODE_NW_PREFIX 4
 #define RTK_MYERS_MODE_NW_PREFIX_LAST 5
+#define RTK_MYERS_MODE_NW_PREFIX_LAST_COLUMN 6
 void rtk_myers_column_last_routes(uint64_t* column_route, uint64_t* fallback);
 
 int rtk_myers_batch_lanes(uint32_t n, const char* const* query, const uint32_t* qlen, const char* const* target, const uint32_t* tlen,
diff --git a/ratatosk_amd/api.py b/ratatosk_amd/api.py
--- a/ratatosk_amd/api.py
+++ b/ratatosk_amd/api.py
@@ -33,7 +33,8 @@
                                          "n_fa_linked_run", "n_fa_linked_skipped", "n_fa_linked_entries",
                                          "n_strand2_run", "n_strand2_skipped", "n_strand2_audit_mismatch",
                                          "n_park_walked", "n_park_deferred",
-                                         "n_colours_small", "n_colours_wide", "n_colours_bits", "n_colours_general", "n_colours_audit_mismatch", "n_colours_declined_fit")]
+                                         "n_colours_small", "n_colours_wide", "n_colours_bits", "n_colours_general", "n_colours_audit_mismatch", "n_colours_declined_fit",
+                                         "n_park_resweeps")]
 
     def as_dict(self):
         return {n: getattr(self, n) for n, _ in self._fields_}
@@ -374,7 +375,7 @@
     return out
 
 
-MODE_SHW_BY_COLUMN, MODE_NW_PREFIX, MODE_NW_PREFIX_LAST = 3, 4, 5
+MODE_SHW_BY_COLUMN, MODE_NW_PREFIX, MODE_NW_PREFIX_LAST, MODE_NW_PREFIX_LAST_COLUMN = 3, 4, 5, 6
 
 
 def myers_column_last_routes(lib_path=None):
diff --git a/ratatosk_amd/csrc/hip/rtk_device.hip b/ratatosk_amd/csrc/hip/rtk_device.hip
--- a/ratatosk_amd/csrc/hip/rtk_device.hip
+++ b/ratatosk_amd/csrc/hip/rtk_device.hip
@@ -480,12 +480,13 @@
         if (r.nloc > 1 && static_cast<uint32_t>(r.nloc) <= cap_locs) end_locs[static_cast<uint64_t>(i) * cap_locs + (r.nloc - 1)] = r.last;
         n_loc[i] = r.nloc;
     } else {
-        const int k = p.k; const bool last_only = p.mode == RTK_MYERS_MODE_NW_PREFIX_LAST;
+        const int k = p.k; const bool from_column = p.mode == RTK_MYERS_MODE_NW_PREFIX_LAST_COLUMN, last_only = from_column || p.mode == RTK_MYERS_MODE_NW_PREFIX_LAST;
         int at = 0, last = -1;
-        if (k > 0 && rtk_myers_shw_by_column(sc, q, m, t, n, iupac, 1, k, &r, &at)) {
+        if (k > 0 && rtk_myers_shw_by_column(sc, q, m, t, n, iupac, from_column ? 2 : 1, k, &r, &at)) {
             const long long W = (k + 63) >> 6;
             if (static_cast<uint32_t>(k) <= sc.r_cap && static_cast<uint32_t>(k + n) <= sc.mv_cap && (2LL * 8 + 4) * W * n + 8LL * n < 1024 * 1024) {
-                if (last_only) last = rtk_myers_last_move(sc, k, n, n, at);
+                if (from_column) last = rtk_myers_last_move_column(sc, k);
+                else if (last_only) last = rtk_myers_last_move(sc, k, n, n, at);
                 else rtk_myers_walk(sc, k, n, n, at, &nm);
                 r.dist = at; route = 1;
             }
@@ -565,9 +566,9 @@
             probs[i].t_off = pool.size(); pool.append(target[i], tlen[i]);
             probs[i].qlen = qlen[i]; probs[i].tlen = tlen[i]; probs[i].k = k[i]; probs[i].mode = mode[i];
             if (mode[i] == RTK_MODE_HW && want_path) return rtk_fail(RTK_ERR_UNSUPPORTED, "rtk_myers_batch: HW path alignment is not on the hot path");
-            if (mode[i] < 0 || mode[i] > RTK_MYERS_MODE_NW_PREFIX_LAST || (mode[i] > RTK_MODE_HW && waves > 1)) return rtk_fail(RTK_ERR_ARG, "rtk_myers_batch: unknown mode (the test-only modes 3 to 5 run on one wave)");
+            if (mode[i] < 0 || mode[i] > RTK_MYERS_MODE_NW_PREFIX_LAST_COLUMN || (mode[i] > RTK_MODE_HW && waves > 1)) return rtk_fail(RTK_ERR_ARG, "rtk_myers_batch: unknown mode (the test-only modes 3 to 6 run on one wave)");
             if ((mode[i] == RTK_MYERS_MODE_SHW_BY_COLUMN && k[i] >= 0) || (mode[i] >= RTK_MYERS_MODE_NW_PREFIX && (k[i] < 0 || static_cast<uint32_t>(k[i]) > qlen[i])))
-                return rtk_fail(RTK_ERR_ARG, "rtk_myers_batch: mode 3 takes k < 0, modes 4 and 5 a query row 0 <= k <= qlen");
+                return rtk_fail(RTK_ERR_ARG, "rtk_myers_batch: mode 3 takes k < 0, modes 4 to 6 a query row 0 <= k <= qlen");
             max_q = std::max(max_q, qlen[i]); max_t = std::max(max_t, tlen[i]);
         }
         for (uint32_t i = 0; i < n; ++i) if (mode[i] > RTK_MODE_HW) { max_q = max_t = std::max(max_q, max_t); break; }
diff --git a/ratatosk_amd/csrc/hip/rtk_knobs.h b/ratatosk_amd/csrc/hip/rtk_knobs.h
--- a/ratatosk_amd/csrc/hip/rtk_knobs.h
+++ b/ratatosk_amd/csrc/hip/rtk_knobs.h
@@ -50,6 +50,7 @@
 inline uint32_t rtk_knob_colours_route() { return rtk_env_eq("RTK_COLOURS_ROUTE", "bits") ? 1u : (rtk_env_eq("RTK_COLOURS_ROUTE", "general") ? 2u : 0u); }
 inline uint32_t rtk_knob_colours_audit() { return rtk_env_is1("RTK_COLOURS_AUDIT") ? (rtk_env_is1("RTK_TEST_COLOURS_FAULT") ? 3u : 1u) : 0u; }
 inline bool rtk_knob_park_eager() { return rtk_env_is1("RTK_PARK_EAGER"); }
+inline bool rtk_knob_trim_store() { return rtk_env_is1("RTK_TRIM_STORE"); }
 inline bool rtk_knob_test_coalesce_fail() { return rtk_env_set("RTK_TEST_COALESCE_FAIL"); }
 
 inline uint64_t rtk_knob_lane_auto_bases() { static const uint64_t v = rtk_env_u64("RTK_LANE_AUTO_BASES", 512ull << 20); return v; }
diff --git a/ratatosk_amd/csrc/hip/rtk_myers.h b/ratatosk_amd/csrc/hip/rtk_myers.h
--- a/ratatosk_amd/csrc/hip/rtk_myers.h
+++ b/ratatosk_amd/csrc/hip/rtk_myers.h
@@ -254,6 +254,7 @@
     int hout_prev = 0; unsigned tc_prev = 0;
     int score = m;
     int best = 0x7fffffff, first = -1, last = -1, cnt = 0, fin = m;
+    uint64_t lastPh = 0, lastMh = 0;
     const int steps = n + W - 1;
     for (int c0 = 0; c0 < steps; c0 += 64) {
         const int cj = c0 + lane;
@@ -275,7 +276,8 @@
             const int hout = rtk_myers_step(nPv, nMv, Eq, hin, bit, Ph, Mh);
             const int col = s - lane;
             const bool active = has_word && col >= 0 && col < n;
-            if (STORE) { if (active) { rtk_tb_put(tb + 4ull * RTK_TB(col, w, n), nPv, nMv, Ph, Mh); } }
+            if (STORE == 1) { if (active) { rtk_tb_put(tb + 4ull * RTK_TB(col, w, n), nPv, nMv, Ph, Mh); } }
+            if (STORE == 2) { lastPh = active ? Ph : lastPh; lastMh = active ? Mh : lastMh; }
             Pv = active ? nPv : Pv; Mv = active ? nMv : Mv;
             hout_prev = active ? hout : hout_prev;
             score += (active && lane == W - 1) ? hout : 0;
@@ -289,6 +291,7 @@
             }
         }
     }
+    if (STORE == 2 && has_word) rtk_tb_put(tb + 4ull * w, Pv, Mv, lastPh, lastMh);
     if (COLUMN) { rtk_last_column_stat(has_word ? Pv : 0ull, has_word ? Mv : 0ull, 64, m, n, at, st); return st; }
     st.final_score = fin; st.best = best; st.first = first; st.last = last; st.cnt = cnt;
     return st;
@@ -349,6 +352,7 @@
     const int bit = (w == W - 1) ? last_bit : 31;
     uint32_t Pv = ~0u, Mv = 0u;
     int hout_prev = 0; uint32_t m1_prev = 0, m2_prev = 0;
+    uint32_t lastPh = 0, lastMh = 0;
     int score = m;
     int vbest = 0x7fffffff, vfirst = -1, vlast = -1, vcnt = 0;
     const int steps = n + W - 1;
@@ -369,12 +373,14 @@
         const int col = s - lane;                                                                                                            \
         if (MASKED) {                                                                                                                        \
             const bool active = has_word && col >= 0 && col < n;                                                                             \
-            if (STORE) { if (active) { RtkTbHalf hv; hv.pv = nPv; hv.mv = nMv; hv.ph = Ph; hv.mh = Mh; tbh[2ull * static_cast<uint64_t>(col)] = hv; } } \
+            if (STORE == 1) { if (active) { RtkTbHalf hv; hv.pv = nPv; hv.mv = nMv; hv.ph = Ph; hv.mh = Mh; tbh[2ull * static_cast<uint64_t>(col)] = hv; } } \
+            if (STORE == 2) { lastPh = active ? Ph : lastPh; lastMh = active ? Mh : lastMh; }                                                \
             Pv = active ? nPv : Pv; Mv = active ? nMv : Mv;                                                                                  \
             hout_prev = active ? hout : hout_prev;                                                                                           \
             score += active ? hout : 0;                                                                                                      \
         } else {                                                                                                                             \
-            if (STORE) { if (has_word) { RtkTbHalf hv; hv.pv = nPv; hv.mv = nMv; hv.ph = Ph; hv.mh = Mh; tbh[2ull * static_cast<uint64_t>(col)] = hv; } } \
+            if (STORE == 1) { if (has_word) { RtkTbHalf hv; hv.pv = nPv; hv.mv = nMv; hv.ph = Ph; hv.mh = Mh; tbh[2ull * static_cast<uint64_t>(col)] = hv; } } \
+            if (STORE == 2) { lastPh = Ph; lastMh = Mh; }                                                                                    \
             Pv = nPv; Mv = nMv; hout_prev = hout; score += hout;                                                                             \
         }                                                                                                                                    \
         m1_prev = m1; m2_prev = m2;                                                                                                          \
@@ -402,6 +408,7 @@
         for (; j < lim; ++j) RTK_STEP32(1)
     }
 #undef RTK_STEP32
+    if (STORE == 2 && has_word) { RtkTbHalf hv; hv.pv = Pv; hv.mv = Mv; hv.ph = lastPh; hv.mh = lastMh; reinterpret_cast<RtkTbHalf*>(tb)[w] = hv; }
     st.final_score = __builtin_amdgcn_readlane(score, W - 1);
     if (TRACK == 2) rtk_last_column_stat(has_word ? Pv : 0u, has_word ? Mv : 0u, 32, m, n, at, st);
     if (TRACK == 1) { st.best = __builtin_amdgcn_readlane(vbest, W - 1); st.first = __builtin_amdgcn_readlane(vfirst, W - 1); st.last = __builtin_amdgcn_readlane(vlast, W - 1); st.cnt = __builtin_amdgcn_readlane(vcnt, W - 1); }
@@ -1049,7 +1056,14 @@
 #ifdef RTK_SIM
     for (int j = 0; j < n; ++j) { const char ch = raw[j]; if (!(ch == 'A' || ch == 'C' || ch == 'G' || ch == 'T')) return false; }
     uint64_t* fin = new uint64_t[2 * W];
-    rtk_myers_pass(sc, rtk_seq(corr, m), rtk_seq(raw, n), 1, iupac, store, fin, fin + W);
+    rtk_myers_pass(sc, rtk_seq(corr, m), rtk_seq(raw, n), 1, iupac, store ? 1 : 0, fin, fin + W);
+    if (store == 2) {
+        uint64_t* const tb = rtk_ld(&sc.tb); uint64_t* const lastc = new uint64_t[4 * W];
+        for (long long w = 0; w < W; ++w) memcpy(lastc + 4 * w, tb + 4ull * RTK_TB(n - 1, w, n), 32);
+        memset(tb, 0xA5, 32ull * static_cast<uint64_t>(W) * static_cast<uint64_t>(n));
+        memcpy(tb, lastc, 32ull * static_cast<uint64_t>(W));
+        delete[] lastc;
+    }
     best = 0x7fffffff; first = -1; last = -1; cnt = 0; atv = n;
     for (int i = 0, v = n; i < m; ++i) {
         v += static_cast<int>((fin[i >> 6] >> (i & 63)) & 1ull) - static_cast<int>((fin[W + (i >> 6)] >> (i & 63)) & 1ull);
@@ -1058,7 +1072,8 @@
     }
     delete[] fin;
 #else
-    const SweepStat st = store ? rtk_myers_fast_any<1, 2>(corr, m, raw, n, 1, iupac, rtk_ld(&sc.tb), at) : rtk_myers_fast_any<0, 2>(corr, m, raw, n, 1, iupac, nullptr, at);
+    const SweepStat st = store == 2 ? rtk_myers_fast_any<2, 2>(corr, m, raw, n, 1, iupac, rtk_ld(&sc.tb), at)
+                       : store ? rtk_myers_fast_any<1, 2>(corr, m, raw, n, 1, iupac, rtk_ld(&sc.tb), at) : rtk_myers_fast_any<0, 2>(corr, m, raw, n, 1, iupac, nullptr, at);
     rtk_sync();
     if (!st.plain) return false;
     best = st.best; first = st.first; last = st.last; cnt = st.cnt; atv = st.at_score;
@@ -1068,7 +1083,7 @@
     r.dist = best;
     if (pseudo && n == best) { r.first = -1; r.last = (colbest == best) ? last : -1; r.nloc = 1 + ((colbest == best) ? cnt : 0); }
     else { r.first = first; r.last = last; r.nloc = cnt; }
-    *out = r;
+    if (out) *out = r;
     if (at_score) *at_score = atv;
     return true;
 }
@@ -1187,6 +1202,21 @@
     int diag = m - 1;
     if (c > 0) { uint64_t l0, l1, l2, l3; rtk_tb_get(tbp + 4ull * RTK_TB(c - 1, w, ncols), l0, l1, l2, l3); diag = cur - hd - (static_cast<int>((l0 >> b) & 1ull) - static_cast<int>((l1 >> b) & 1ull)); }
     return (diag == cur) ? 0 : 3;
+}
+
+RTK_DEV uint8_t rtk_myers_last_move_column(const MyersScratch& sc_, int m_) {
+    const MyersScratch& sc = *rtk_u(&sc_); RTK_ASSUME_LDS(&sc);
+    const int m = rtk_u(m_);
+    const uint64_t* const tbp = rtk_ld(&sc.tb);
+    const int r = m - 1, w = r >> 6, b = r & 63;
+    uint64_t a0, a1, a2, a3; rtk_tb_get(tbp + 4ull * static_cast<uint64_t>(w), a0, a1, a2, a3);
+    const int vd = static_cast<int>((a0 >> b) & 1ull) - static_cast<int>((a1 >> b) & 1ull);
+    if (vd == 1) return 1;
+    if (static_cast<int>((a2 >> b) & 1ull) - static_cast<int>((a3 >> b) & 1ull) == 1) return 2;
+    int hu = 1;
+    if (b > 0) hu = static_cast<int>((a2 >> (b - 1)) & 1ull) - static_cast<int>((a3 >> (b - 1)) & 1ull);
+    else if (w > 0) { uint64_t u0, u1, u2, u3; rtk_tb_get(tbp + 4ull * static_cast<uint64_t>(w - 1), u0, u1, u2, u3); hu = static_cast<int>((u2 >> 63) & 1ull) - static_cast<int>((u3 >> 63) & 1ull); }
+    return (vd + hu == 0) ? 0 : 3;
 }
 
 RTK_FN void rtk_myers_traceback(const MyersScratch& sc_, MySeq q_, MySeq t_, bool iupac_, uint32_t* n_moves_) {
diff --git a/ratatosk_amd/csrc/hip/rtk_pipeline.inc b/ratatosk_amd/csrc/hip/rtk_pipeline.inc
--- a/ratatosk_amd/csrc/hip/rtk_pipeline.inc
+++ b/ratatosk_amd/csrc/hip/rtk_pipeline.inc
@@ -120,6 +120,7 @@
     v.strand2_mode = rtk_knob_strand2_always() ? 1u : (rtk_knob_strand2_audit() ? 2u : 0u);
     v.colours_mode = rtk_knob_colours_route() | (rtk_knob_colours_audit() << 2);
     v.park_eager = rtk_knob_park_eager() ? 1u : 0u;
+    v.trim_store = rtk_knob_trim_store() ? 1u : 0u;
     v.long_read_correct = o->long_read_correct ? 1 : 0; v.max_len_weak_region2 = static_cast<uint32_t>(o->max_len_weak_region2 > 0xFFFFFFFFull ? 0xFFFFFFFFull : o->max_len_weak_region2);
     return v;
 }
diff --git a/ratatosk_amd/csrc/hip/rtk_pipeline_run.inc b/ratatosk_amd/csrc/hip/rtk_pipeline_run.inc
--- a/ratatosk_amd/csrc/hip/rtk_pipeline_run.inc
+++ b/ratatosk_amd/csrc/hip/rtk_pipeline_run.inc
@@ -333,7 +333,8 @@
         for (int i = RTK_RC_FA_LINKED_RUN; i < RTK_RC_STRAND2_RUN; ++i) rtk_atomic_add(bv.counters + RTK_CNT_FA_LINKED + (i - RTK_RC_FA_LINKED_RUN), sc->cnt[i]);
         for (int i = RTK_RC_STRAND2_RUN; i < RTK_RC_PARK_WALKED; ++i) rtk_atomic_add(bv.counters + RTK_CNT_STRAND2 + (i - RTK_RC_STRAND2_RUN), sc->cnt[i]);
         for (int i = RTK_RC_PARK_WALKED; i < RTK_RC_COLOURS_SMALL; ++i) rtk_atomic_add(bv.counters + RTK_CNT_PARK + (i - RTK_RC_PARK_WALKED), sc->cnt[i]);
-        for (int i = RTK_RC_COLOURS_SMALL; i < RTK_RC_N; ++i) rtk_atomic_add(bv.counters + RTK_CNT_COLOURS + (i - RTK_RC_COLOURS_SMALL), sc->cnt[i]);
+        for (int i = RTK_RC_COLOURS_SMALL; i < RTK_RC_PARK_RESWEEPS; ++i) rtk_atomic_add(bv.counters + RTK_CNT_COLOURS + (i - RTK_RC_COLOURS_SMALL), sc->cnt[i]);
+        rtk_atomic_add(bv.counters + RTK_CNT_PARK_RESWEEPS, sc->cnt[RTK_RC_PARK_RESWEEPS]);
         for (int i = 0; i < RTK_H_N; ++i) rtk_atomic_add(bv.counters + RTK_CNT_HIST + i, static_cast<unsigned long long>(RTK_HIST_GET(*sc, i)));
 #ifdef RTK_PROF
         for (int i = 0; i < RTK_LAP_N; ++i) rtk_atomic_add(bv.counters + RTK_CNT_PROF + i, static_cast<unsigned long long>(sc->prof[i]));
@@ -723,7 +724,7 @@
     fprintf(stderr, "[rtk trace] fixAmbiguity linked-allele searches: run %llu, skipped %llu, entries produced %llu, cycles %.3g\n", cnt[RTK_CNT_FA_LINKED + 0], cnt[RTK_CNT_FA_LINKED + 1],
             cnt[RTK_CNT_FA_LINKED + 2], double(cnt[RTK_CNT_FINE + RTK_FINE_FA_LINKED]));
     fprintf(stderr, "[rtk trace] second strand of gap regions: run %llu, skipped %llu (the forward result decides), audit mismatches %llu\n", cnt[RTK_CNT_STRAND2 + 0], cnt[RTK_CNT_STRAND2 + 1], cnt[RTK_CNT_STRAND2 + 2]);
-    fprintf(stderr, "[rtk trace] stored sweeps of the forward trims: walked for a consensus %llu, never walked %llu\n", cnt[RTK_CNT_PARK + 0], cnt[RTK_CNT_PARK + 1]);
+    fprintf(stderr, "[rtk trace] stored sweeps of the forward trims: walked for a consensus %llu (from a second sweep %llu), never walked %llu\n", cnt[RTK_CNT_PARK + 0], cnt[RTK_CNT_PARK_RESWEEPS], cnt[RTK_CNT_PARK + 1]);
     fprintf(stderr, "[rtk trace] colour selections answered by: small %llu, wide %llu, bits %llu, general %llu; audit mismatches %llu; handed on by the register program for room %llu\n", cnt[RTK_CNT_COLOURS + 0], cnt[RTK_CNT_COLOURS + 1], cnt[RTK_CNT_COLOURS + 2],
             cnt[RTK_CNT_COLOURS + 3], cnt[RTK_CNT_COLOURS + 4], cnt[RTK_CNT_COLOURS + 5]);
     fprintf(stderr, "[rtk trace] walks %llu moves %llu reloads %llu scalar steps %llu cycles %.3g tail cycles %.3g\n", cnt[RTK_CNT_WALK_CALLS], cnt[RTK_CNT_WALK_MOVES],
@@ -744,7 +745,7 @@
     st.n_consensus_resumed = cnt[RTK_CNT_ROUTES + 3]; st.n_consensus_swept = cnt[RTK_CNT_ROUTES + 4];
     st.n_fa_linked_run = cnt[RTK_CNT_FA_LINKED + 0]; st.n_fa_linked_skipped = cnt[RTK_CNT_FA_LINKED + 1]; st.n_fa_linked_entries = cnt[RTK_CNT_FA_LINKED + 2];
     st.n_strand2_run = cnt[RTK_CNT_STRAND2 + 0]; st.n_strand2_skipped = cnt[RTK_CNT_STRAND2 + 1]; st.n_strand2_audit_mismatch = cnt[RTK_CNT_STRAND2 + 2];
-    st.n_park_walked = cnt[RTK_CNT_PARK + 0]; st.n_park_deferred = cnt[RTK_CNT_PARK + 1];
+    st.n_park_walked = cnt[RTK_CNT_PARK + 0]; st.n_park_deferred = cnt[RTK_CNT_PARK + 1]; st.n_park_resweeps = cnt[RTK_CNT_PARK_RESWEEPS];
     st.n_colours_small = cnt[RTK_CNT_COLOURS + 0]; st.n_colours_wide = cnt[RTK_CNT_COLOURS + 1]; st.n_colours_bits = cnt[RTK_CNT_COLOURS + 2]; st.n_colours_general = cnt[RTK_CNT_COLOURS + 3];
     st.n_colours_audit_mismatch = cnt[RTK_CNT_COLOURS + 4]; st.n_colours_declined_fit = cnt[RTK_CNT_COLOURS + 5];
     st.ms_stitch = R.t_st.elapsed(); st.ms_total = b->t_all.elapsed();
diff --git a/ratatosk_amd/csrc/hip/rtk_region.h b/ratatosk_amd/csrc/hip/rtk_region.h
--- a/ratatosk_amd/csrc/hip/rtk_region.h
+++ b/ratatosk_amd/csrc/hip/rtk_region.h
@@ -383,7 +383,7 @@
                 emit_minus_k(fw.seq, fw.seq_len, fw.qual, fw.qual_len);
             } else {
                 s.cnt[skippable ? RTK_RC_STRAND2_SKIPPED : RTK_RC_STRAND2_RUN] += 1;
-                rtk_park_walk(c);
+                rtk_park_walk(c, fw.seq, s_fw + pa);
                 auto audit = [&](const char* seq, uint32_t sl, const char* q, uint32_t ql) {
                     if (skippable && !(sl == fw.seq_len && ql == fw.qual_len && rtk_str_equal(seq, fw.seq, sl) && rtk_str_equal(q, fw.qual, ql))) s.cnt[RTK_RC_STRAND2_AUDIT_MISMATCH] += 1;
                 };
diff --git a/ratatosk_amd/csrc/hip/rtk_region_align.h b/ratatosk_amd/csrc/hip/rtk_region_align.h
--- a/ratatosk_amd/csrc/hip/rtk_region_align.h
+++ b/ratatosk_amd/csrc/hip/rtk_region_align.h
@@ -30,14 +30,20 @@
     return r;
 }
 
-RTK_FN void rtk_park_walk(const RCtx& c_) {
-    const RCtx& c = *rtk_u(&c_); RegionScratch& s = rtk_hdr(c);
+RTK_FN void rtk_park_walk(const RCtx& c_, const char* corr_, const char* raw_) {
+    const RCtx& c = *rtk_u(&c_); RegionScratch& s = rtk_hdr(c); const char* corr = rtk_u(corr_); const char* raw = rtk_u(raw_);
     TrimPark& pk = s.loc.park;
     if (!pk.pending) return;
+    const unsigned long long t1 = rtk_clock();
+    if (pk.pending == RTK_PARK_NO_TABLE) {
+        const bool ok = rtk_myers_shw_by_column(s.my, corr, static_cast<int>(pk.len), raw, static_cast<int>(pk.n), true, 1, 0, nullptr, nullptr);
+        s.cnt[RTK_RC_PARK_RESWEEPS] += 1;
+        if (!ok) { pk.pending = 0; pk.nm = 0; s.cnt[RTK_RC_CYC_MYERS] += rtk_clock() - t1; return; }
+        pk.gen = rtk_ld(&s.my.tb_gen);
+    }
 #ifdef RTK_SIM
     assert(pk.gen == s.my.tb_gen);
 #endif
-    const unsigned long long t1 = rtk_clock();
     pk.pending = 0;
     uint32_t& nm = pk.nm; nm = 0;
     rtk_myers_walk(s.my, static_cast<int>(pk.len), static_cast<int>(pk.n), static_cast<int>(pk.n), pk.dist, &nm);
@@ -51,7 +57,8 @@
     const RCtx& c = *rtk_u(&c_); RegionScratch& s = rtk_hdr(c); const char* raw = rtk_u(raw_); const char* corr = rtk_u(corr_);
     const uint32_t n = rtk_u(n_), m = rtk_u(m_); const bool park = rtk_u(park_); MyersResult* out = rtk_u(out_);
     const unsigned long long t0 = rtk_clock();
-    const bool ok = rtk_myers_shw_by_column(s.my, corr, static_cast<int>(m), raw, static_cast<int>(n), true, park ? 1 : 0, 0, out, nullptr);
+    const bool table = rtk_u(c.o.trim_store) != 0u;
+    const bool ok = rtk_myers_shw_by_column(s.my, corr, static_cast<int>(m), raw, static_cast<int>(n), true, park ? (table ? 1 : 2) : 0, 0, out, nullptr);
     s.cnt[RTK_RC_CYC_MYERS] += rtk_clock() - t0;
     if (!ok) return false;
     s.cnt[RTK_RC_ALIGN] += 1; s.cnt[RTK_RC_CELLS] += static_cast<unsigned long long>((m + 63) / 64) * n;
@@ -64,10 +71,10 @@
     if (keep == 0 || keep > s.my.r_cap || keep + n > s.my.mv_cap || !((2LL * 8 + 4) * W * n + 8LL * n < 1024 * 1024)) return true;
     const unsigned long long t1 = rtk_clock();
     TrimPark& pk = s.loc.park;
-    pk.nm = 0; pk.len = keep; pk.dist = out->dist; pk.n = n; pk.gen = rtk_ld(&s.my.tb_gen); pk.pending = 1;
-    pk.last_move = rtk_myers_last_move(s.my, static_cast<int>(keep), static_cast<int>(n), static_cast<int>(n), out->dist);
+    pk.nm = 0; pk.len = keep; pk.dist = out->dist; pk.n = n; pk.gen = rtk_ld(&s.my.tb_gen); pk.pending = table ? RTK_PARK_TABLE : RTK_PARK_NO_TABLE;
+    pk.last_move = table ? rtk_myers_last_move(s.my, static_cast<int>(keep), static_cast<int>(n), static_cast<int>(n), out->dist) : rtk_myers_last_move_column(s.my, static_cast<int>(keep));
     s.cnt[RTK_RC_CYC_MYERS] += rtk_clock() - t1;
-    if (rtk_u(c.o.park_eager) || keep + n > s.str_cap) rtk_park_walk(c);
+    if (rtk_u(c.o.park_eager) || keep + n > s.str_cap) rtk_park_walk(c, corr, raw);
     return true;
 }
 
diff --git a/ratatosk_amd/csrc/hip/rtk_region_types.h b/ratatosk_amd/csrc/hip/rtk_region_types.h
--- a/ratatosk_amd/csrc/hip/rtk_region_types.h
+++ b/ratatosk_amd/csrc/hip/rtk_region_types.h
@@ -129,6 +129,7 @@
 struct ResCorr { char* seq; char* qual; uint32_t seq_len, qual_len; uint64_t* bm; uint32_t old_len; bool is_corrected; uint32_t n_all; int all_set; };
 struct RegionCall { const char* s_read; const char* q_read; uint64_t complete; UMap um1, um2; uint32_t s_len, p1, p2, first_pos, len_weak_region, lw_lo, lw_hi, n_all, n_partial, n_amb, has_end_pt, found_first, lrc; };
 struct TrimPark { uint32_t nm, len; int32_t dist; uint32_t n, last_move, pending, gen; };
+enum { RTK_PARK_TABLE = 1u, RTK_PARK_NO_TABLE = 2u };
 struct DriverLocals { Anchors an[RTK_AN_N]; ResCorr rc[RTK_RES_N]; SideList side[RTK_SIDE_N]; uint32_t len[RTK_LEN_N]; int best[RTK_BEST_N]; MyersSaved saved; RegionCall call; TrimPark park; MyersResult trim; };
 
 struct RegionScratch {
diff --git a/ratatosk_amd/csrc/hip/rtk_seeds.h b/ratatosk_amd/csrc/hip/rtk_seeds.h
--- a/ratatosk_amd/csrc/hip/rtk_seeds.h
+++ b/ratatosk_amd/csrc/hip/rtk_seeds.h
@@ -20,6 +20,7 @@
     U<uint32_t> strand2_mode;
     U<uint32_t> colours_mode;
     U<uint32_t> park_eager;
+    U<uint32_t> trim_store;
 };
 
 struct BatchView {
diff --git a/ratatosk_amd/csrc/hip/rtk_types.h b/ratatosk_amd/csrc/hip/rtk_types.h
--- a/ratatosk_amd/csrc/hip/rtk_types.h
+++ b/ratatosk_amd/csrc/hip/rtk_types.h
@@ -169,7 +169,8 @@
     RTK_CNT_PARK_END = 219,
     RTK_CNT_COLOURS = 219,
     RTK_CNT_COLOURS_END = 225,
-    RTK_CNT_USED_END = RTK_CNT_COLOURS_END,
+    RTK_CNT_PARK_RESWEEPS = 225,
+    RTK_CNT_USED_END = 226,
     RTK_CNT_TOTAL = (RTK_CNT_USED_END + 31) / 32 * 32
 };
 static_assert(RTK_CNT_TOTAL == 256, "counter map: the size of the block changed (it is part of what the kernels and the host agree on)");
@@ -192,12 +193,13 @@
     RTK_RC_FA_LINKED_RUN = 21, RTK_RC_FA_LINKED_SKIPPED = 22, RTK_RC_FA_LINKED_ENTRIES = 23,
     RTK_RC_STRAND2_RUN = 24, RTK_RC_STRAND2_SKIPPED = 25, RTK_RC_STRAND2_AUDIT_MISMATCH = 26,
     RTK_RC_PARK_WALKED = 27, RTK_RC_PARK_DEFERRED = 28,
-    RTK_RC_COLOURS_SMALL = 29, RTK_RC_COLOURS_WIDE = 30, RTK_RC_COLOURS_BITS = 31, RTK_RC_COLOURS_GENERAL = 32, RTK_RC_COLOURS_AUDIT_MISMATCH = 33, RTK_RC_COLOURS_DECLINED_FIT = 34, RTK_RC_N = 35 };
+    RTK_RC_COLOURS_SMALL = 29, RTK_RC_COLOURS_WIDE = 30, RTK_RC_COLOURS_BITS = 31, RTK_RC_COLOURS_GENERAL = 32, RTK_RC_COLOURS_AUDIT_MISMATCH = 33, RTK_RC_COLOURS_DECLINED_FIT = 34,
+    RTK_RC_PARK_RESWEEPS = 35, RTK_RC_N = 36 };
 static_assert(RTK_CNT_ROUTES_END - RTK_CNT_ROUTES == static_cast<int>(RTK_RC_FA_LINKED_RUN) - static_cast<int>(RTK_RC_TRIM_STORED), "counter map: one slot per route counter");
 static_assert(RTK_CNT_FA_LINKED_END - RTK_CNT_FA_LINKED == static_cast<int>(RTK_RC_STRAND2_RUN) - static_cast<int>(RTK_RC_FA_LINKED_RUN), "counter map: one slot per fixAmbiguity counter");
 static_assert(RTK_CNT_STRAND2_END - RTK_CNT_STRAND2 == static_cast<int>(RTK_RC_PARK_WALKED) - static_cast<int>(RTK_RC_STRAND2_RUN), "counter map: one slot per second-strand counter");
 static_assert(RTK_CNT_PARK_END - RTK_CNT_PARK == static_cast<int>(RTK_RC_COLOURS_SMALL) - static_cast<int>(RTK_RC_PARK_WALKED), "counter map: one slot per park counter");
-static_assert(RTK_CNT_COLOURS_END - RTK_CNT_COLOURS == static_cast<int>(RTK_RC_N) - static_cast<int>(RTK_RC_COLOURS_SMALL), "counter map: one slot per colour-route counter");
+static_assert(RTK_CNT_COLOURS_END - RTK_CNT_COLOURS == static_cast<int>(RTK_RC_PARK_RESWEEPS) - static_cast<int>(RTK_RC_COLOURS_SMALL), "counter map: one slot per colour-route counter");
 #define RTK_CM_ROUTE 3u
 #define RTK_CM_ROUTE_BITS 1u
 #define RTK_CM_ROUTE_GENERAL 2u
```

New measurement: 2.302 billion, median of 6. 2.8% higher.
